# thelondonsmiths/Solex_ser_recon_EN

Hardware: AMD Instinct MI355X
Metric: SER frames/sec end-to-end (decode→clahe) + %HBM roofline, 1/2/4/8 MI355X (higher is better)
Workload: dtype u16

## Files before the change

include/shg_hip.h:

```cpp
#ifndef SHG_HIP_H
#define SHG_HIP_H

#include <stddef.h>
#include <stdint.h>

#ifdef __cplusplus
extern "C" {
#endif

#define SHG_ABI_VERSION 16

#define SHG_E_ARG        (-1)
#define SHG_E_WORKSPACE  (-2)
#define SHG_E_UNSUPPORTED (-3)
#define SHG_E_VALUE      (-4)
#define SHG_E_TYPE       (-5)
#define SHG_E_LINALG     (-6)
#define SHG_E_RUNTIME    (-7)
#define SHG_E_QHULL      (-8)
#define SHG_E_ASSERT     (-9)
#define SHG_E_INDEX      (-10)

typedef void* shg_stream_t;

// ... 199 lines not shown
                             int64_t rank_lo, int64_t rank_hi, uint16_t* out_lo, uint16_t* out_hi,
                             shg_stream_t stream);

int shg_crop_pad_u16(const uint16_t* src, int64_t h, int64_t w, int64_t pitch,
                     uint16_t* dst, int64_t nw, int64_t dst_pitch,
                     int64_t sx0, int64_t dx0, int64_t n, int32_t fill, shg_stream_t stream);

size_t shg_clahe_workspace_bytes(int tiles, int bytes_per_px);
size_t shg_clahe_workspace_bytes_for(int64_t h, int64_t w, int tiles, int bytes_per_px);
int shg_clahe(const void* img, int64_t h, int64_t w, int64_t pitch, int bytes_per_px,
              double clip_limit, int tiles, void* dst, int64_t dst_pitch,
              void* workspace, size_t workspace_bytes, shg_stream_t stream);

int shg_hist(const void* img, int64_t h, int64_t w, int64_t pitch, int bytes_per_px,
             uint32_t* hist, shg_stream_t stream);

size_t shg_select_u16_workspace_bytes(int n_ranks);
int shg_select_u16(const uint16_t* img, int64_t h, int64_t w, int64_t pitch, const int64_t* host_ranks,
                   int n_ranks, double* out, void* workspace, size_t workspace_bytes, shg_stream_t stream);

int shg_rescale_u16(const uint16_t* img, int64_t h, int64_t w, int64_t pitch,
                    double lo, double hi, double alpha, uint16_t* dst, int64_t dst_pitch,
                    shg_stream_t stream);
int shg_rescale_u8(const uint8_t* img, int64_t h, int64_t w, int64_t pitch, double lo, double hi,
                   double alpha, uint8_t* dst, int64_t dst_pitch, shg_stream_t stream);

int shg_fill_disc_u16(uint16_t* img, int64_t h, int64_t w, int64_t pitch,
                      int64_t x0, int64_t y0, int64_t r, uint16_t value, int32_t* scratch,
                      shg_stream_t stream);

int shg_downscale_mean_u16(const uint16_t* img, int64_t h, int64_t w, int64_t pitch, int factor,
                           double* dst, shg_stream_t stream);

int shg_box_blur_f64(const double* src, int64_t h, int64_t w, int k, double* dst, double* tmp,
                     shg_stream_t stream);

int shg_box_blur_key_f64(const double* src, int64_t h, int64_t w, int k, double* dst, uint32_t* keys, double* tmp,
                         shg_stream_t stream);
size_t shg_select_keys_workspace_bytes(int n_pairs);
int shg_select_keys_u32(const uint32_t* const* host_keys, int64_t n, const int64_t* host_ranks, const int* host_k,
                        int n_pairs, double* out, void* workspace, size_t workspace_bytes, shg_stream_t stream);

size_t shg_select_workspace_bytes(int n_ranks);
int shg_select_f64(const double* values, int64_t n, const int64_t* host_ranks, int n_ranks, double* out,
                   void* workspace, size_t workspace_bytes, shg_stream_t stream);
int shg_select_multi_f64(const double* const* host_arrays, int64_t n, const int64_t* host_ranks, int n_ranks,
                         double* out, void* workspace, size_t workspace_bytes, shg_stream_t stream);

int shg_flood_stats_f64(const double* image, const double* blurred, int64_t n, double very_bright,
                        double* stats, uint32_t* counts, void* workspace, shg_stream_t stream);
int shg_flood_stats_lerp_f64(const double* image, const double* blurred, int64_t n,
                             const double* order_stats, double gamma, double* stats, uint32_t* counts,
                             void* workspace, shg_stream_t stream);

size_t shg_canny_workspace_bytes(int64_t h, int64_t w);
int shg_canny_masks_f64(const double* blurred, int64_t h, int64_t w, double flood_thresh,
                        const double* host_gauss_weights, int radius, double low, double high,
                        uint8_t* low_mask, uint8_t* high_mask, void* workspace, size_t workspace_bytes,
                        shg_stream_t stream);

size_t shg_edge_components_workspace_bytes(int64_t h, int64_t w);
int shg_edge_components(const uint8_t* low_mask, const uint8_t* high_mask, int64_t h, int64_t w,
                        int32_t* out_idx, int32_t* out_root, int32_t* out_count,
                        void* workspace, size_t workspace_bytes, shg_stream_t stream);

size_t shg_contrast_stats_workspace_bytes(int tiles);
size_t shg_contrast_stats_workspace_bytes_for(int64_t h, int64_t w, int tiles);
int shg_contrast_stats_u16(const uint16_t* frame, int64_t h, int64_t w, int64_t pitch, double clip_limit,
                           int tiles, uint16_t* cl1, int64_t cl1_pitch, const int64_t* ranks_frame2,
                           const int64_t* ranks_cl13, double* out5, void* workspace, size_t workspace_bytes,
                           shg_stream_t stream);
int shg_contrast_products_u16(const uint16_t* frame, int64_t frame_pitch, const uint16_t* cl1, int64_t cl1_pitch,
                              int64_t h, int64_t w, const double* lo_hi6, uint16_t* high_contrast,
                              uint16_t* protus, uint16_t* cc, int64_t dst_pitch, int64_t disc_x0,
                              int64_t disc_y0, int64_t disc_r, shg_stream_t stream);
int shg_contrast_products_vec_fits(const uint16_t* frame, int64_t frame_pitch, const uint16_t* cl1, int64_t cl1_pitch,
                                   int64_t h, int64_t w, const uint16_t* high_contrast, const uint16_t* protus,
                                   const uint16_t* cc, int64_t dst_pitch);

int shg_limb_fused_fits(int64_t sh, int64_t sw, int k);
size_t shg_limb_prepare_workspace_bytes(int64_t sh, int64_t sw, int k);
int shg_limb_prepare(const uint16_t* img, int64_t h, int64_t w, int64_t pitch, int k, const int64_t* host_ranks4, double gamma99,
                     double* packed, const uint32_t** keys_out, void* workspace, size_t workspace_bytes, shg_stream_t stream);
size_t shg_limb_edges_workspace_bytes(int64_t sh, int64_t sw);
int shg_limb_edges(const uint32_t* keys, int64_t sh, int64_t sw, int k, double flood_thresh, const double* host_gauss_weights,
                   int radius, double low, double high, int32_t* comp, void* workspace, size_t workspace_bytes, shg_stream_t stream);


size_t shg_stage_mean_fit_workspace_bytes(int64_t n_frames, int64_t height, int64_t width, int bytes_per_px);
size_t shg_stage_mean_fit_host_bytes(int64_t height, int64_t width);
int shg_stage_mean_fit(const void* stack, int64_t n_frames, int64_t height, int64_t width, int bytes_per_px,
                       int64_t frame_stride_px, const uint64_t* sum_in, const uint16_t* max_in, int64_t n_total,
                       uint16_t* mean_out, uint16_t* max_out, int64_t* host_y12, double* host_p4, double* host_fit,
                       int32_t* host_trace_sharp, uint8_t* host_mask_good, void* workspace, size_t workspace_bytes,
                       void* host_pinned, size_t host_pinned_bytes, shg_stream_t stream);

size_t shg_stage_extract_workspace_bytes(int64_t height, int64_t width, int n_shifts);
int shg_stage_extract(const void* stack, int64_t n_frames, int64_t height, int64_t width, int bytes_per_px,
                      int64_t frame_stride_px, const double* host_fit, const int32_t* host_shifts, int n_shifts,
                      uint16_t* disks, int64_t row_pitch, int64_t plane_stride, int64_t n_cols, int64_t k_offset,
                      int flip_x, uint32_t* minmax_slots, void* workspace, size_t workspace_bytes, void* host_pinned,
                      size_t host_pinned_bytes, shg_stream_t stream);

size_t shg_stage_limb_points_workspace_bytes(int64_t h, int64_t w);
size_t shg_stage_limb_points_host_bytes(int64_t h, int64_t w);
int shg_stage_limb_points(const uint16_t* disk, int64_t h, int64_t w, int64_t pitch, const double* host_gauss_taps,
                          int32_t* host_points, uint8_t* host_flags, int64_t points_cap, int64_t* host_counts2,
                          void* workspace, size_t workspace_bytes, void* host_pinned, size_t host_pinned_bytes,
                          shg_stream_t stream);

int shg_stage_limb_fit(const uint16_t* disk, int64_t h, int64_t w, int64_t pitch, const double* host_gauss_taps,
                       int32_t* host_points, uint8_t* host_flags, int64_t points_cap, int64_t* host_counts3,
                       double* host_geom16, int64_t* host_dims2, double* host_outline200, void* workspace,
                       size_t workspace_bytes, void* host_pinned, size_t host_pinned_bytes, shg_stream_t stream);

size_t shg_stage_process_workspace_bytes(int64_t k, int64_t h, int64_t w, int64_t crop_w, int tiles);
size_t shg_stage_process_host_bytes(int64_t k, int64_t h);
int shg_stage_process_frames(const uint16_t* const* host_frames, int64_t k, int64_t h, int64_t w, int64_t pitch,
                             int transversalium, const double* host_circle3, const double* host_borders4,
                             const double* host_taps, int64_t window, double* host_factors, int64_t crop_w,
                             int64_t sx0, int64_t dx0, int64_t ncopy, double clip_limit, int tiles, int64_t disc_x0,
                             int64_t disc_y0, int64_t disc_r, uint16_t* const* host_detrans, int64_t detrans_pitch,
                             uint16_t* const* host_final, uint16_t* const* host_cl1, uint16_t* const* host_hc,
                             uint16_t* const* host_protus, uint16_t* const* host_cc, int64_t out_pitch, void* workspace,
                             size_t workspace_bytes, void* host_pinned, size_t host_pinned_bytes, shg_stream_t stream);

typedef struct shg_scan_request {
    uint32_t struct_bytes;
    int32_t  start_phase;
    const void* stack;
    int64_t  n_frames, height, width, frame_stride_px;
    int32_t  bytes_per_px;
    int32_t  flip_x;
    const int32_t* host_shifts;
    const uint8_t* host_requested;
    int32_t  n_shifts;
    int32_t  want_fit_image;
    double   ratio_fixe, slant_fix_deg;
    int32_t  transversalium, keep_detrans;
    int64_t  trans_strength;
    const double* host_taps;
    int64_t  taps_window;
    int32_t  crop_square, has_fixed_width;
    int64_t  fixed_width;
    int32_t  disk_display, tiles;
    int64_t  delta_radius;
    double   clip_limit;
    const double* host_gauss_taps;
    uint16_t* mean_out;
    uint16_t* max_out;
    uint16_t* disks;
    int64_t  disk_pitch, disk_plane_stride;
    uint32_t* minmax_slots;
    void*    arena;
    size_t   arena_bytes;
    void*    results;
    size_t   results_bytes;
    void*    workspace;
    size_t   workspace_bytes;
    void*    host_pinned;
    size_t   host_pinned_bytes;
    double*  host_fit;
    int32_t* host_trace_sharp;
    uint8_t* host_mask_good;
    int32_t* host_points;
    uint8_t* host_flags;
    int64_t  points_cap;
    double*  host_outline200;
    double*  host_factors;
} shg_scan_request;

typedef struct shg_scan_result {
    int32_t phase_done;
    int32_t limb_fitted;
    int64_t y1, y2;
    double  p4[4];
    int64_t counts3[3];
    double  geom16[16];
    double  phi, ratio;
    double  h_first[3], h_rest[3];
    double  theta_first, theta_rest;
    double  circle3[3], borders4[4];
    double  circle_out3[3];
    int64_t out_h, out_w, frame_pitch;
    int64_t n_out, prod_w, prod_pitch;
    int64_t window;
    int64_t crop4[4];
    int64_t disc3[3];
    int64_t fit_image_off;
    int64_t frames_off;
    int64_t detrans_off;
    int64_t products_off;
    int64_t results_off;
    size_t  needed_arena_bytes, needed_results_bytes, needed_workspace_bytes;
} shg_scan_result;

size_t shg_scan_workspace_bytes(const shg_scan_request* req);
size_t shg_scan_host_bytes(const shg_scan_request* req);
int shg_scan_file(const shg_scan_request* req, shg_scan_result* res, shg_stream_t stream);
typedef int (*shg_savgol_taps_fn)(int64_t window, double* out);
int shg_host_set_savgol_taps(shg_savgol_taps_fn fn);

typedef struct shg_pool shg_pool;
int shg_pool_create(const shg_stream_t* streams, int n_workers, const int32_t* host_cpus, int n_cpus, shg_pool** out);
int shg_pool_submit(shg_pool* pool, const shg_scan_request* req, shg_scan_result* res, int64_t* ticket);
int shg_pool_submit_after(shg_pool* pool, const shg_scan_request* req, shg_scan_result* res, shg_stream_t after, int64_t* ticket);
int shg_scan_prelaunch(const shg_scan_request* req, shg_stream_t after, int* launched);
int shg_pass_a_prelaunch(const void* stack, int64_t n_frames, int64_t height, int64_t width, int bytes_per_px,
                         int64_t frame_stride_px, void* workspace, size_t workspace_bytes, shg_stream_t after, int* launched);
int shg_pass_a_forget(const void* workspace);
int shg_lane_packets_probe(const void* stack, int64_t n_frames, int64_t height, int64_t width, int bytes_per_px,
                           int64_t frame_stride_px, void* workspace, size_t workspace_bytes, int mode, int launches,
                           shg_stream_t stream, double* ms_per_launch);
int shg_pool_poll(shg_pool* pool, int64_t ticket);
int shg_pool_wait(shg_pool* pool, int64_t ticket, int* scan_status, char* error_buf, size_t error_cap);
int shg_pool_destroy(shg_pool* pool);

int shg_device_cu_count(int* out);
int shg_stream_create(int priority, const uint32_t* host_cu_mask, int n_mask_words, shg_stream_t* out);
int shg_stream_destroy(shg_stream_t stream);
int shg_frame_pass_lane_set(shg_stream_t lane);
shg_stream_t shg_frame_pass_lane_get(void);

int shg_host_bind_lapack(void* dgelsd_ilp64);
int shg_host_lapack_bound(void);
typedef int64_t (*shg_mode_pick_fn)(const int64_t* neg_counts, int64_t n);
int shg_host_set_mode_pick(shg_mode_pick_fn pick);
int shg_host_polyfit3(const double* host_x, const double* host_y, int64_t n, double* host_coef4);
int shg_host_detect_bord(const double* host_row_means, int64_t n, int64_t* lb, int64_t* ub);
int shg_host_line_fit(const int32_t* host_trace_blur, const int32_t* host_trace_sharp, int64_t ih, int64_t y1,
                      int64_t y2, int32_t blur_offset, double* host_p4, double* host_fit, uint8_t* host_mask_good);
int shg_host_column_plan(const double* host_fit, int64_t ih, int64_t iw, const int32_t* host_shifts, int n_shifts,
                         int32_t* host_ind_l, double* host_lw, double* host_rw);
int shg_host_flood_threshold(double total, int64_t h, int64_t w, double mn, double mx, const int64_t* host_counts20,
                             double* thresh_out);
int shg_host_limb_points(const int32_t* host_idx, const int32_t* host_root, int64_t m, int64_t h, int64_t w,
                         uint8_t* host_out_sel, int64_t* n_selected);
int shg_host_bind_blas(void* cblas_dgemm_ilp64, void* cblas_dsyrk_ilp64, void* cblas_dgemv_ilp64, void* dgesv_ilp64,
                       void* dgeev_ilp64);
int shg_host_blas_bound(void);
int shg_host_fit_ellipse(const double* host_points, int64_t n, double* host_center2, double* width, double* height,
                         double* phi);
int shg_host_correction_matrix(double phi, double r, double* host_inv4, double* theta_out);
int shg_host_two_step(const double* host_points, int64_t n, double* host_center2, double* height_out, double* phi_out,
                      double* ratio_out, uint8_t* host_kept, int64_t* n_kept, double* host_outline200);
int shg_host_warp_geometry(double phi, double ratio, int64_t h, int64_t w, double* host_mat3_9, double* host_inv4,
                           double* host_origin2, double* det_out, double* theta_out, int64_t* out_h, int64_t* out_w);
int shg_host_limb_geometry(const double* host_points, int64_t n, int64_t h, int64_t w, double* host_geom16,
                           int64_t* host_dims2, uint8_t* host_kept, int64_t* n_kept, double* host_outline200);
int shg_host_chord_bounds(double cx, double cy, double r, double b0, double b2, int64_t y1, int64_t y2, int64_t w,
                          int32_t* host_xa, int32_t* host_xb);
int shg_host_transversalium_factors(const double* host_ratios, const double* host_interior, int64_t k, int64_t n,
// ... 9 lines not shown
```

solex_ser_recon_en_amd/Solex_recon.py:

```python
import contextlib
import functools
import math
import os
import queue
import sys
import threading

import numpy as np

from . import dist, ops, outputs, timing
from .device import DeviceImage, bind_thread, cpu_plan, default_device, to_device_u16
from .ellipse_to_circle import correct_image, ellipse_to_circle
from .fits_io import write_fits
from . import stages
from .solex_util import (as_uint16_image, clearlog, compute_mean_return_fit, correct_transversalium2_batch, extract_disks,
                         image_process_batch, logme, make_header, output_path, plots_enabled, removeVignette, savgol_taps,
                         savgol_window, write_complete, write_products)
from .video_reader import video_reader


WORKERS = 4


def _worker_count(workers, n_tasks):
# ... 460 lines not shown


def _scan_pool(scan, n_tasks, n_workers, device):
    import torch
    lock = threading.Lock()
    state = {'next': 0, 'errors': []}

    done = threading.Semaphore(0)

    def run(k):
        try:
            work(k)
        except BaseException as e:
            with lock:
                state['errors'].append((n_tasks, e))
        finally:
            done.release()

    def work(k):
        try:
            torch.cuda.set_device(device)
            bind_thread('scan', device)
            ctx = _worker_context(device, k)
            stages.use_buffers(ctx['buffers'])
            stream = ctx['stream']
        except BaseException as e:
            with lock:
                state['errors'].append((state['next'], e))
            return
        with torch.cuda.stream(stream):
            while True:
                with lock:
                    i = state['next']
                    if i >= n_tasks or state['errors']:
                        break
                    state['next'] = i + 1
                try:
                    scan(i)
                except BaseException as e:
                    with lock:
                        state['errors'].append((i, e))
                    break
            stream.synchronize()

    for k in range(n_workers):
        _Service.named('shg-scan-%s-%d' % (device, k)).jobs.put(functools.partial(run, k))
    for _ in range(n_workers):
        done.acquire()
    if state['errors']:
        raise min(state['errors'], key=lambda ie: ie[0])[1]


def _one_call_ok(rdr, options):
    if os.environ.get('SHG_SCAN_CALL', '1') == '0' or timing.enabled:
        return False
    if options.get('_shard_frames') or dist.is_sharded(rdr):
        return False
    if options['de-vignette'] or (options['transversalium'] and options.get('stubborn_transversalium')):
        return False
    return True


def scan_one_call(rdr, options):
    return _OneCall(rdr, options).run().finish()


class _OneCall:

    def __init__(self, rdr, options, pooled=False):
        self.rdr, self.options = rdr, options
        self.basefich0 = basefich0 = os.path.splitext(str(rdr.file))[0]
        options['basefich0'] = basefich0
        self.log = log = basefich0 + '_log.txt'
        clearlog(log, options)
        logme(log, options, 'Pixel shift : ' + str(options['shift']))
        options['shift_requested'] = options['shift']
        options['shift'] = list(dict.fromkeys([options['ellipse_fit_shift'], 0] + options['shift']))
        self.hdr = make_header(rdr)
        logme(log, options, 'Width, Height : ' + str(rdr.Width) + ' ' + str(rdr.Height))
        logme(log, options, 'Number of frames : ' + str(rdr.FrameCount))
        self.shifts = shifts = options['shift']
        self.requested = [sh in options['shift_requested'] for sh in shifts]
        self.plots = plots = plots_enabled(options)
        self.call = stages.ScanCall(rdr.device_stack(), shifts, self.requested, options, savgol_taps, want_plot_data=plots,
                                    want_fit_image=plots, own_buffers=pooled)

    def run(self):
        self.call.run()
        return self

    def submit(self, pool):
        self.call.submit(pool)
        return self

    def done(self):
        return self.call.done()

    def finish(self):
        from .ellipse_to_circle import _log_geometry, _warp_geometry
        rdr, options, hdr, log, basefich0 = self.rdr, self.options, self.hdr, self.log, self.basefich0
        shifts, requested, plots = self.shifts, self.requested, self.plots
        r, error = self.call.wait().collect()
        self.call = None
        _release_stack(rdr)
        phase = r['phase']
        if phase >= 1:
            mean_img = DeviceImage(r['mean'])
            y1, y2 = r['y1'], r['y2']
            if options['save_fit']:
                outputs.submit(write_fits, output_path(basefich0 + '_mean.fits', options), mean_img, hdr)
            logme(log, options, 'Vertical limits y1, y2 : ' + str(y1) + ' ' + str(y2))
            logme(log, options, lambda: 'Spectral line polynomial fit: ' + str(r['p']))
            if plots:
                rows = np.arange(y1, y2)
                good = r['mask_good']
                outputs.submit(outputs.plot_spectral_line, output_path(basefich0 + '_spectral_line_data.png', options), mean_img,
                               r['sharp'].astype(np.int64)[y1:y2][good], rows[good], r['fit'][:, 3], int(rdr.ih), (y2 - y1) // 20 + 1)
        disk_list = []
        if phase >= 2:
            hdr['NAXIS1'] = rdr.iw
            if options['save_fit'] or plots or (phase >= 3 and not r['limb_fitted'] and requested[0] and '_nolog' not in options):
                disk_list = [DeviceImage(r['disks'][i], minmax=r['extrema'][i]) for i in range(len(shifts))]
            if options.get('_keep_raw'):
                options['_raw_disks'] = [DeviceImage(r['disks'][i]) for i in range(len(shifts))]
            for i, disk in enumerate(disk_list):
                if options['save_fit'] and requested[i]:
                    outputs.submit(write_fits, output_path(basefich0 + '_shift=' + str(shifts[i]) + '_raw.fits', options), disk, hdr)
            if options['transversalium']:
                logme(log, options, 'Transversalium correction : ' + str(options['trans_strength']))
            else:
                logme(log, options, 'Transversalium disabled')
            logme(log, options, 'Mirror X : ' + str(options['flip_x']))
            logme(log, options, 'Post-rotation : ' + str(options['img_rotate']) + ' degrees')
            logme(log, options, f'Protus adjustment : {options["delta_radius"]}')
            logme(log, options, f'de-vignette : {options["de-vignette"]}')
        if phase >= 3:
            if r['limb_fitted']:
                options['ratio_fixe'] = r['ratio']
                _log_geometry(options, r['phi'], r['ratio'], r['theta_first'], np.array(r['circle'][:2]), r['circle'][2])
                print('sun borders found:' + str(r['borders']))
                options['slant_fix'] = math.degrees(r['phi'])
            elif requested[0] and '_nolog' not in options:
                ih_, n_ = disk_list[0].shape
                theta, inv_mat, _, _, _, origin, det = _warp_geometry(float(r['phi']), float(r['ratio']), int(ih_), int(n_))
                _log_geometry(options, r['phi'], r['ratio'], theta, (inv_mat @ np.array([-1.0, -1.0]).T).T - origin,
                              -1.0 * np.sqrt(np.abs(r['ratio'] / det)), known=False)
        if error is not None:
            raise error
        names = [basefich0 + '_shift=' + str(shifts[i]) for i in range(len(shifts)) if requested[i]]
        if plots and r['limb_fitted']:
            fix_img = r['frames'][0] if requested[0] else r['fit_image']
            outputs.submit(outputs.plot_ellipse_fit, output_path(basefich0 + '_shift=' + str(shifts[0]) + '_ellipse_fit.png', options),
                           disk_list[0], DeviceImage(fix_img), r['raw_X'], r['X_f'], r['outline'], r['borders'])
        if options['save_fit']:
            for j, basefich in enumerate(names):
                outputs.submit(write_fits, output_path(basefich + '_circular.fits', options), DeviceImage(r['frames'][j]), hdr)
        if options['transversalium']:
            for i, basefich in enumerate(names):
                c = r['factors'][i]
                options['_transversalium_cache'] = c
                if plots:
                    outputs.submit(outputs.plot_transversalium, output_path(basefich + '_transversalium_correction.png', options), c)
                if options['save_fit']:
                    outputs.submit(write_fits, output_path(basefich + '_detransversaliumed.fits', options), DeviceImage(r['detrans'][i]), hdr)
        if '_nolog' in options and not options['save_fit'] and options['img_rotate'] // 90 % 4 == 0:
            return [(DeviceImage(r['cc'][i]), DeviceImage(r['protus'][i])) for i in range(len(names))]
        results = [write_products(r['final'][i], r['cl1'][i], r['hc'][i], r['protus'][i], r['cc'][i], options, hdr, names[i])
                   for i in range(len(names))]
# ... 213 lines not shown
```

solex_ser_recon_en_amd/_lib.py:

```python
import ctypes
import os
from ctypes import c_double, c_int, c_int32, c_int64, c_size_t, c_uint16, c_uint32, c_void_p

import torch

_HERE = os.path.dirname(os.path.abspath(__file__))
LIB_PATH = os.path.join(_HERE, 'csrc', 'libshg_hip.so')

if not os.path.exists(LIB_PATH):
    raise ImportError(
        'libshg_hip.so is missing (%s). Build it with `python -c "import __graft_entry__ as g; g.build()"` or '
        '`make -C solex_ser_recon_en_amd/csrc`. There is no CPU fallback for the SHG hot path.' % LIB_PATH)

lib = ctypes.CDLL(LIB_PATH)

P = c_void_p
PD = ctypes.POINTER(c_double)
PI64 = ctypes.POINTER(c_int64)


class ScanRequest(ctypes.Structure):
    _fields_ = [('struct_bytes', c_uint32), ('start_phase', c_int32),
                ('stack', P), ('n_frames', c_int64), ('height', c_int64), ('width', c_int64), ('frame_stride_px', c_int64),
                ('bytes_per_px', c_int32), ('flip_x', c_int32),
                ('host_shifts', P), ('host_requested', P), ('n_shifts', c_int32), ('want_fit_image', c_int32),
                ('ratio_fixe', c_double), ('slant_fix_deg', c_double),
                ('transversalium', c_int32), ('keep_detrans', c_int32), ('trans_strength', c_int64),
                ('host_taps', P), ('taps_window', c_int64),
                ('crop_square', c_int32), ('has_fixed_width', c_int32), ('fixed_width', c_int64),
                ('disk_display', c_int32), ('tiles', c_int32), ('delta_radius', c_int64), ('clip_limit', c_double),
                ('host_gauss_taps', P),
                ('mean_out', P), ('max_out', P), ('disks', P), ('disk_pitch', c_int64), ('disk_plane_stride', c_int64),
                ('minmax_slots', P), ('arena', P), ('arena_bytes', c_size_t), ('results', P), ('results_bytes', c_size_t), ('workspace', P), ('workspace_bytes', c_size_t),
                ('host_pinned', P), ('host_pinned_bytes', c_size_t),
                ('host_fit', P), ('host_trace_sharp', P), ('host_mask_good', P), ('host_points', P), ('host_flags', P),
                ('points_cap', c_int64), ('host_outline200', P), ('host_factors', P)]


class ScanResult(ctypes.Structure):
    _fields_ = [('phase_done', c_int32), ('limb_fitted', c_int32), ('y1', c_int64), ('y2', c_int64), ('p4', c_double * 4),
                ('counts3', c_int64 * 3), ('geom16', c_double * 16), ('phi', c_double), ('ratio', c_double),
                ('h_first', c_double * 3), ('h_rest', c_double * 3), ('theta_first', c_double), ('theta_rest', c_double),
                ('circle3', c_double * 3), ('borders4', c_double * 4), ('circle_out3', c_double * 3),
                ('out_h', c_int64), ('out_w', c_int64), ('frame_pitch', c_int64),
                ('n_out', c_int64), ('prod_w', c_int64), ('prod_pitch', c_int64), ('window', c_int64),
                ('crop4', c_int64 * 4), ('disc3', c_int64 * 3),
                ('fit_image_off', c_int64), ('frames_off', c_int64), ('detrans_off', c_int64), ('products_off', c_int64),
                ('results_off', c_int64), ('needed_arena_bytes', c_size_t), ('needed_results_bytes', c_size_t), ('needed_workspace_bytes', c_size_t)]


SIGNATURES = {
    'shg_abi_version': (c_int, []),
    'shg_last_error_string': (ctypes.c_char_p, []),
    'shg_profile_enable': (c_int, [c_int]),
    'shg_profile_select': (c_int, [ctypes.c_char_p]),
    'shg_profile_reset': (c_int, []),
    'shg_profile_get': (c_int, [ctypes.c_char_p, ctypes.POINTER(c_double), ctypes.POINTER(c_int64)]),
    'shg_profile_total': (c_int, [ctypes.POINTER(c_double), ctypes.POINTER(c_int64)]),
    'shg_profile_dump': (c_int, [ctypes.c_char_p]),
    'shg_host_timing_enable': (c_int, [c_int]),
    'shg_host_timing_report': (c_int, [ctypes.c_char_p, c_size_t]),
    'shg_stream_read_probe': (c_int, [P, c_int64, c_int, c_int, c_int, c_int64, P, P]),
    'shg_accumulate_workspace_bytes': (c_size_t, [c_int64, c_int64, c_int64, c_int]),
    'shg_accumulate_sum_max': (c_int, [P, c_int64, c_int64, c_int64, c_int, c_int64, P, P, P, c_size_t, P]),
    'shg_frame_pitch_bytes': (c_int64, [c_int64]),
    'shg_upload_frames': (c_int, [P, c_int64, P, c_int64, c_int64, P]),
    'shg_unpack_dib_frames': (c_int, [P, c_int64, c_int64, c_int64, c_int64, c_int, c_int64, c_int, P, P, c_int64, P]),
    'shg_finalize_mean_max': (c_int, [P, P, c_int64, c_int64, c_int64, c_int, P, P, P]),
    'shg_reduce_frame_stats': (c_int, [P, c_int, c_int64, c_int64, P, P, P]),
    'shg_accumulate_mean_max': (c_int, [P, c_int64, c_int64, c_int64, c_int, c_int64, P, P, P, c_size_t, P]),
    'shg_box_blur_u16': (c_int, [P, c_int64, c_int64, c_int, c_int, P, P, P]),
    'shg_row_argmin_u16': (c_int, [P, c_int64, c_int64, c_int64, c_int64, P, P]),
    'shg_row_mean_u16': (c_int, [P, c_int64, c_int64, P, P]),
    'shg_atlas_correlate': (c_int, [P, c_int64, c_double, c_double, c_double, c_double, P, c_int64, c_int64, c_int64, P, c_int64,
                                    P, P, P, c_int64, P, P]),
    'shg_line_core_shift': (c_int, [P, c_int64, c_int64, c_int64, c_int, c_int64, P, c_int, c_int, P, c_int64, c_int64, c_int64, P]),
    'shg_doppler_finish': (c_int, [P, c_int64, c_int64, c_int64, c_double, c_double, c_double, c_int64, c_int64, P, P, P, c_int64,
                                   P, c_int64, c_double, P]),
    'shg_line_profile': (c_int, [P, c_int64, c_int64, c_int64, c_int, c_int64, P, c_int, c_int, c_int, P, c_int64, c_int64, c_int64,
                                 c_int64, P]),
    'shg_line_profile_finish': (c_int, [P, c_int64, c_int64, c_int64, c_int64, c_double, c_double, c_double, c_int64, c_int64, P, P,
                                        P, c_int64, c_int64, P, c_int64, c_int64, c_int, c_double, P]),
    'shg_line_bisector': (c_int, [P, c_int64, c_int64, c_int64, c_int, c_int64, P, c_int, c_int, P, c_int, c_int, P, c_int64, c_int64,
                                  c_int64, c_int64, P]),
    'shg_line_bisector_finish': (c_int, [P, c_int64, c_int, c_int64, c_int64, c_int64, c_double, c_double, c_double, c_int64, c_int64,
                                         P, P, P, c_int64, c_int64, P, c_int64, c_int64, c_int, c_double, P]),
    'shg_line_emission': (c_int, [P, c_int64, c_int64, c_int64, c_int, c_int64, P, c_int, c_int, c_double, c_int, P, c_int64, c_int64,
                                  c_int64, c_int64, P]),
    'shg_line_emission_finish': (c_int, [P, c_int64, c_int64, c_int64, c_int64, c_double, c_double, c_double, c_int64, c_int64, P, P,
                                         P, c_int64, c_int64, P, c_int64, c_int64, c_int, c_double, P]),
    'shg_map_plane_moments': (c_int, [P, c_int64, c_int64, c_int64, P, P, P, P]),
    'shg_map_detrend': (c_int, [P, c_int64, c_int64, c_int64, P, P, c_int64, P, c_int64, c_double, P]),
    'shg_ring_medians_u16_workspace_bytes': (c_size_t, [c_int64]),
    'shg_ring_medians_u16': (c_int, [P, c_int64, c_int64, c_int64, P, c_int64, P, P, P, P, c_size_t, P]),
    'shg_ring_flatten_u16': (c_int, [P, c_int64, c_int64, c_int64, P, P, c_int64, P, c_int64, P]),
    'shg_stack_combine_u16': (c_int, [P, P, P, c_int, c_int, c_double, c_int, P, c_int64, c_int64, c_int64, P, c_int64, P]),
    'shg_shift_ssd_u16': (c_int, [P, c_int64, P, c_int64, c_int64, c_int64, c_int, P, P, P]),
    'shg_patch_ssd_u16': (c_int, [P, c_int64, P, c_int64, c_int64, c_int64, P, c_int64, c_int, c_int, P, P, P]),
    'shg_stack_combine_field_u16': (c_int, [P, P, P, P, c_int64, c_int64, c_int, c_int, c_int, c_double, c_int, P, c_int64, c_int64, c_int64,
                                            P, c_int64, P]),
    'shg_patch_sharpness_u16': (c_int, [P, c_int64, c_int64, c_int64, P, c_int64, c_int, c_int, P, P, P]),
    'shg_stack_combine_weighted_u16': (c_int, [P, P, P, P, P, c_int64, c_int64, c_int, c_int, c_int, c_double, c_int, P, c_int64, c_int64,
                                               c_int64, P, c_int64, P]),
    'shg_wavelet_workspace_bytes': (c_size_t, [c_int64, c_int64, c_int]),
    'shg_wavelet_sharpen_u16': (c_int, [P, c_int64, c_int64, c_int64, c_int, P, P, P, c_int64, P, P, c_size_t, P]),
    'shg_wavelet_noise_u16': (c_int, [P, c_int64, c_int64, c_int64, P, P, P, c_size_t, P]),
    'shg_rl_workspace_bytes': (c_size_t, [c_int64, c_int64]),
    'shg_rl_deconvolve_u16': (c_int, [P, c_int64, c_int64, c_int64, P, c_int, c_int, P, c_int64, P, P, c_size_t, P]),
    'shg_blur_fits_fused': (c_int, [c_int64, c_int]),
    'shg_blur_row_mean_u16': (c_int, [P, c_int64, c_int64, c_int, c_int, P, P]),
    'shg_blur_argmin_u16': (c_int, [P, c_int64, c_int64, c_int, c_int, c_int64, c_int64, P, P, P]),
    'shg_extract_columns': (c_int, [P, c_int64, c_int64, c_int64, c_int, c_int64, P, P, P, c_int, P, c_int64, c_int64,
                                    c_int64, c_int64, c_int, P]),
    'shg_extract_columns_minmax': (c_int, [P, c_int64, c_int64, c_int64, c_int, c_int64, P, P, P, c_int, P, c_int64, c_int64,
                                           c_int64, c_int64, c_int, P, P]),
    'shg_extract_dense_fits': (c_int, [P, c_int]),
    'shg_extract_columns_dense': (c_int, [P, c_int64, c_int64, c_int64, c_int, c_int64, P, P, P, P, P, c_int, P, c_int64, c_int64, c_int64, c_int64,
                                          c_int, P, P]),
    'shg_warp_rows_minmax_u16': (c_int, [P, c_int64, c_int64, c_int64, c_double, c_double, c_double, P, c_int64, c_int64,
                                         c_int64, P, P]),
    'shg_warp_rows_u16': (c_int, [P, c_int64, c_int64, c_int64, c_double, c_double, c_double, P, c_int64, c_int64,
                                  c_int64, P, P]),
    'shg_warp_rows_wide_fits': (c_int, [P, c_int64, c_int64, c_int64, c_double, c_double, c_double, P, c_int64, c_int64, c_int64]),
    'shg_rowpair_logratio_stats': (c_int, [P, c_int64, c_int64, c_int64, c_int64, c_int64, P, P, P, P, P]),
    'shg_rowpair_logratio_stats_mirrored': (c_int, [P, c_int64, c_int64, c_int64, c_int64, c_int64, P, P, P, P, P, P]),
    'shg_line_order_stats_u16': (c_int, [P, c_int64, c_int64, c_int64, c_int, c_int64, c_int64, P, P, P]),
    'shg_scale_rows_u16': (c_int, [P, c_int64, c_int64, c_int64, P, P, P, c_int64, P]),
    'shg_scale_rows_vec_fits': (c_int, [P, c_int64, c_int64, c_int64, P, c_int64]),
    'shg_correlate1d_rows_f64': (c_int, [P, c_int64, c_int64, P, c_int, c_int, P, P]),
    'shg_lin_filter_row_sums': (c_int, [P, c_int64, c_int64, c_int64, P, P, P, P, P, c_int, P, P, P]),
    'shg_lin_filter_apply': (c_int, [P, c_int64, c_int64, c_int64, P, P, P, c_int, c_int, P, P, P, P, c_int, P, c_int64, P]),
    'shg_crop_pad_u16': (c_int, [P, c_int64, c_int64, c_int64, P, c_int64, c_int64, c_int64, c_int64, c_int64,
                                 c_int, P]),
    'shg_clahe_workspace_bytes': (c_size_t, [c_int, c_int]),
    'shg_clahe_workspace_bytes_for': (c_size_t, [c_int64, c_int64, c_int, c_int]),
    'shg_clahe': (c_int, [P, c_int64, c_int64, c_int64, c_int, c_double, c_int, P, c_int64, P, c_size_t, P]),
    'shg_hist': (c_int, [P, c_int64, c_int64, c_int64, c_int, P, P]),
    'shg_select_u16_workspace_bytes': (c_size_t, [c_int]),
    'shg_select_u16': (c_int, [P, c_int64, c_int64, c_int64, ctypes.POINTER(c_int64), c_int, P, P, c_size_t, P]),
    'shg_rescale_u16': (c_int, [P, c_int64, c_int64, c_int64, c_double, c_double, c_double, P, c_int64, P]),
    'shg_rescale_u8': (c_int, [P, c_int64, c_int64, c_int64, c_double, c_double, c_double, P, c_int64, P]),
    'shg_contrast_stats_workspace_bytes': (c_size_t, [c_int]),
    'shg_contrast_stats_workspace_bytes_for': (c_size_t, [c_int64, c_int64, c_int]),
    'shg_contrast_stats_u16': (c_int, [P, c_int64, c_int64, c_int64, c_double, c_int, P, c_int64, P, P, P, P, c_size_t, P]),
    'shg_contrast_products_u16': (c_int, [P, c_int64, P, c_int64, c_int64, c_int64, P, P, P, P, c_int64, c_int64, c_int64, c_int64, P]),
    'shg_contrast_products_vec_fits': (c_int, [P, c_int64, P, c_int64, c_int64, c_int64, P, P, P, c_int64]),
    'shg_fill_disc_u16': (c_int, [P, c_int64, c_int64, c_int64, c_int64, c_int64, c_int64, c_uint16, P, P]),
    'shg_downscale_mean_u16': (c_int, [P, c_int64, c_int64, c_int64, c_int, P, P]),
    'shg_box_blur_f64': (c_int, [P, c_int64, c_int64, c_int, P, P, P]),
    'shg_box_blur_key_f64': (c_int, [P, c_int64, c_int64, c_int, P, P, P, P]),
    'shg_select_keys_workspace_bytes': (c_size_t, [c_int]),
    'shg_select_keys_u32': (c_int, [ctypes.POINTER(c_void_p), c_int64, ctypes.POINTER(c_int64), ctypes.POINTER(c_int), c_int, P, P, c_size_t, P]),
    'shg_select_workspace_bytes': (c_size_t, [c_int]),
    'shg_select_f64': (c_int, [P, c_int64, ctypes.POINTER(c_int64), c_int, P, P, c_size_t, P]),
    'shg_select_multi_f64': (c_int, [ctypes.POINTER(c_void_p), c_int64, ctypes.POINTER(c_int64), c_int, P, P, c_size_t, P]),
    'shg_flood_stats_f64': (c_int, [P, P, c_int64, c_double, P, P, P, P]),
    'shg_flood_stats_lerp_f64': (c_int, [P, P, c_int64, P, c_double, P, P, P, P]),
    'shg_edge_components_workspace_bytes': (c_size_t, [c_int64, c_int64]),
    'shg_edge_components': (c_int, [P, P, c_int64, c_int64, P, P, P, P, c_size_t, P]),
    'shg_canny_workspace_bytes': (c_size_t, [c_int64, c_int64]),
    'shg_canny_masks_f64': (c_int, [P, c_int64, c_int64, c_double, ctypes.POINTER(c_double), c_int, c_double, c_double, P, P, P,
                                    c_size_t, P]),
    'shg_limb_fused_fits': (c_int, [c_int64, c_int64, c_int]),
    'shg_limb_prepare_workspace_bytes': (c_size_t, [c_int64, c_int64, c_int]),
    'shg_limb_prepare': (c_int, [P, c_int64, c_int64, c_int64, c_int, PI64, c_double, P, ctypes.POINTER(c_void_p), P, c_size_t, P]),
    'shg_limb_edges_workspace_bytes': (c_size_t, [c_int64, c_int64]),
    'shg_limb_edges': (c_int, [P, c_int64, c_int64, c_int, c_double, PD, c_int, c_double, c_double, P, P, c_size_t, P]),
    'shg_stage_mean_fit_workspace_bytes': (c_size_t, [c_int64, c_int64, c_int64, c_int]),
    'shg_stage_mean_fit_host_bytes': (c_size_t, [c_int64, c_int64]),
    'shg_stage_mean_fit': (c_int, [P, c_int64, c_int64, c_int64, c_int, c_int64, P, P, c_int64, P, P, P, P, P, P, P, P, c_size_t, P,
                                   c_size_t, P]),
    'shg_stage_extract_workspace_bytes': (c_size_t, [c_int64, c_int64, c_int]),
    'shg_stage_extract': (c_int, [P, c_int64, c_int64, c_int64, c_int, c_int64, P, P, c_int, P, c_int64, c_int64, c_int64, c_int64, c_int,
                                  P, P, c_size_t, P, c_size_t, P]),
    'shg_stage_limb_points_workspace_bytes': (c_size_t, [c_int64, c_int64]),
    'shg_stage_limb_points_host_bytes': (c_size_t, [c_int64, c_int64]),
    'shg_stage_limb_points': (c_int, [P, c_int64, c_int64, c_int64, P, P, P, c_int64, P, P, c_size_t, P, c_size_t, P]),
    'shg_stage_limb_fit': (c_int, [P, c_int64, c_int64, c_int64, P, P, P, c_int64, P, P, P, P, P, c_size_t, P, c_size_t, P]),
    'shg_stage_process_workspace_bytes': (c_size_t, [c_int64, c_int64, c_int64, c_int64, c_int]),
    'shg_stage_process_host_bytes': (c_size_t, [c_int64, c_int64]),
    'shg_stage_process_frames': (c_int, [P, c_int64, c_int64, c_int64, c_int64, c_int, P, P, P, c_int64, P, c_int64, c_int64, c_int64,
                                         c_int64, c_double, c_int, c_int64, c_int64, c_int64, P, c_int64, P, P, P, P, P, c_int64, P, c_size_t,
                                         P, c_size_t, P]),
    'shg_scan_workspace_bytes': (c_size_t, [ctypes.POINTER(ScanRequest)]),
    'shg_scan_host_bytes': (c_size_t, [ctypes.POINTER(ScanRequest)]),
    'shg_scan_file': (c_int, [ctypes.POINTER(ScanRequest), ctypes.POINTER(ScanResult), P]),
    'shg_host_set_savgol_taps': (c_int, [P]),
    'shg_pool_create': (c_int, [P, c_int, P, c_int, ctypes.POINTER(c_void_p)]),
    'shg_pool_submit': (c_int, [P, ctypes.POINTER(ScanRequest), ctypes.POINTER(ScanResult), ctypes.POINTER(c_int64)]),
    'shg_pool_submit_after': (c_int, [P, ctypes.POINTER(ScanRequest), ctypes.POINTER(ScanResult), P, ctypes.POINTER(c_int64)]),
    'shg_scan_prelaunch': (c_int, [ctypes.POINTER(ScanRequest), P, ctypes.POINTER(c_int)]),
    'shg_pass_a_prelaunch': (c_int, [P, c_int64, c_int64, c_int64, c_int, c_int64, P, c_size_t, P, ctypes.POINTER(c_int)]),
    'shg_pass_a_forget': (c_int, [P]),
    'shg_lane_packets_probe': (c_int, [P, c_int64, c_int64, c_int64, c_int, c_int64, P, c_size_t, c_int, c_int, P, ctypes.POINTER(c_double)]),
    'shg_pool_poll': (c_int, [P, c_int64]),
    'shg_pool_wait': (c_int, [P, c_int64, ctypes.POINTER(c_int), ctypes.c_char_p, c_size_t]),
    'shg_pool_destroy': (c_int, [P]),
    'shg_device_cu_count': (c_int, [ctypes.POINTER(c_int)]),
    'shg_stream_create': (c_int, [c_int, P, c_int, ctypes.POINTER(c_void_p)]),
    'shg_stream_destroy': (c_int, [P]),
    'shg_frame_pass_lane_set': (c_int, [P]),
    'shg_frame_pass_lane_get': (c_void_p, []),
    'shg_host_bind_lapack': (c_int, [P]),
    'shg_host_lapack_bound': (c_int, []),
    'shg_host_set_mode_pick': (c_int, [P]),
    'shg_host_polyfit3': (c_int, [P, P, c_int64, P]),
    'shg_host_detect_bord': (c_int, [P, c_int64, PI64, PI64]),
    'shg_host_line_fit': (c_int, [P, P, c_int64, c_int64, c_int64, ctypes.c_int32, P, P, P]),
    'shg_host_column_plan': (c_int, [P, c_int64, c_int64, P, c_int, P, P, P]),
    'shg_host_flood_threshold': (c_int, [c_double, c_int64, c_int64, c_double, c_double, P, PD]),
    'shg_host_limb_points': (c_int, [P, P, c_int64, c_int64, c_int64, P, PI64]),
    'shg_host_bind_blas': (c_int, [P, P, P, P, P]),
    'shg_host_blas_bound': (c_int, []),
    'shg_host_fit_ellipse': (c_int, [P, c_int64, P, PD, PD, PD]),
    'shg_host_correction_matrix': (c_int, [c_double, c_double, P, PD]),
    'shg_host_two_step': (c_int, [P, c_int64, P, PD, PD, PD, P, PI64, P]),
    'shg_host_warp_geometry': (c_int, [c_double, c_double, c_int64, c_int64, P, P, P, PD, PD, PI64, PI64]),
    'shg_host_limb_geometry': (c_int, [P, c_int64, c_int64, c_int64, P, P, P, PI64, P]),
    'shg_host_chord_bounds': (c_int, [c_double, c_double, c_double, c_double, c_double, c_int64, c_int64, c_int64, P, P]),
    'shg_host_transversalium_factors': (c_int, [P, P, c_int64, c_int64, P, c_int64, c_int, P]),
    'shg_host_percentile_plan': (c_int, [c_int64, c_double, PI64, PI64, PD]),
    'shg_host_lerp': (c_double, [c_double, c_double, c_double]),
}

for _name, (_res, _args) in SIGNATURES.items():
    _fn = getattr(lib, _name)
    _fn.restype = _res
    _fn.argtypes = _args

ABI_VERSION = 16
if lib.shg_abi_version() != ABI_VERSION:
    raise ImportError('libshg_hip.so ABI %d != expected %d: rebuild it' % (lib.shg_abi_version(), ABI_VERSION))


def last_error():
    return lib.shg_last_error_string().decode('utf-8', 'replace')


def _host_error(status, what, message=None):
    msg = last_error() if message is None else message
    if status == -4:
        return ValueError(msg)
    if status == -5:
        return TypeError(msg)
    if status == -6:
        import numpy
        return numpy.linalg.LinAlgError(msg)
    if status == -10:
        return IndexError(msg)
    if status == -9:
        return AssertionError(msg)
    if status == -8:
        try:
            from scipy.spatial import QhullError
            return QhullError(msg)
        except ImportError:
            pass
    return RuntimeError('%s: %s' % (what, msg) if status != -7 else msg)


def check(status, what, message=None):
# ... 106 lines not shown
```

solex_ser_recon_en_amd/csrc/extract.hip:

```cpp
#include <stdlib.h>
#include <algorithm>
#include <type_traits>
#include "shg_common.h"

namespace shg {
thread_local bool t_minmax_slots_zeroed = false;
thread_local void* t_zero_with_fold = nullptr;
thread_local size_t t_zero_with_fold_words = 0;
thread_local void* t_prezeroed = nullptr;
}

namespace {

constexpr int TY = 64;
constexpr int TK = 64;
constexpr int TKP = TK + 2;
constexpr int SC_MAX = 4;

struct ExtractArgs {
    const void* stack;
    int n_frames;
    int64_t height, width, fstride;
    const int32_t* ind_l;
    const double *lw, *rw;
    int n_shifts;
    uint16_t* disks;
    int64_t row_pitch, plane_stride, n_cols, k_offset;
    int flip_x, vec_store;
    uint32_t* mm;
};

template <typename T, bool ROT, int BATCH, int SC> __global__ __launch_bounds__(256) void k_extract(const ExtractArgs kargs) {
    const T* __restrict__ stack = static_cast<const T*>(kargs.stack);
    const int n_frames = kargs.n_frames, n_shifts = kargs.n_shifts, flip_x = kargs.flip_x, vec_store = kargs.vec_store;
    const int64_t height = kargs.height, width = kargs.width, fstride = kargs.fstride, row_pitch = kargs.row_pitch, plane_stride = kargs.plane_stride,
                  n_cols = kargs.n_cols, k_offset = kargs.k_offset;
    const int32_t* __restrict__ ind_l = kargs.ind_l;
    const double* __restrict__ lw = kargs.lw;
    const double* __restrict__ rw = kargs.rw;
    uint16_t* __restrict__ disks = kargs.disks;
    uint32_t* __restrict__ mm = kargs.mm;
    __shared__ uint16_t tile[SC][TY][TKP];
    const int64_t ih = ROT ? width : height;
    const int lane = threadIdx.x & 63;
    const int wave = __builtin_amdgcn_readfirstlane(threadIdx.x >> 6);
    const int64_t c0 = (int64_t)blockIdx.x * TK;
    const int64_t y = (int64_t)blockIdx.y * TY + lane;
    const int s0 = blockIdx.z * SC;
    const int ns = min(SC, n_shifts - s0);
    const bool y_ok = y < ih;
    constexpr int scale = sizeof(T) == 1 ? 256 : 1;

    const int64_t yc = y_ok ? y : ih - 1;
    int il[SC];
    const double wl = lw[yc], wr = rw[yc];
    const double kl = wl * 0x1p+52, kr = wr * 0x1p+52;
    const bool fast = __all(fabs(wl) < 0x1p+900 && fabs(wr) < 0x1p+900) != 0;
#pragma unroll
    for (int s = 0; s < SC; ++s) il[s] = ind_l[(int64_t)(s0 + min(s, ns - 1)) * ih + yc];

    uint32_t off[SC], offr[SC];
    const int64_t step = ROT ? width : 1;
#pragma unroll
    for (int s = 0; s < SC; ++s) {
        off[s] = (uint32_t)((ROT ? (int64_t)il[s] * width + (width - 1 - yc) : yc * width + il[s]) * (int64_t)sizeof(T));
        offr[s] = off[s] + (uint32_t)(step * (int64_t)sizeof(T));
    }

    __shared__ uint32_t wred[4][SC][2];
    uint32_t vlo[SC], vhi[SC];
#pragma unroll
    for (int s = 0; s < SC; ++s) { vlo[s] = 0xffffu; vhi[s] = 0u; }

    for (int cb = wave; cb < TK; cb += 4 * BATCH) {
        T lv[BATCH][SC], rv[BATCH][SC];
        bool ok[BATCH];
#pragma unroll
        for (int i = 0; i < BATCH; ++i) {
            const int cc = cb + 4 * i;
            const int64_t col = c0 + cc;
            const int64_t k = (flip_x ? (n_cols - 1 - col) : col) - k_offset;
            ok[i] = cc < TK && col < n_cols && k >= 0 && k < n_frames;
            const char* f = reinterpret_cast<const char*>(stack + (ok[i] ? k : 0) * fstride);
#pragma unroll
            for (int s = 0; s < SC; ++s) {
                lv[i][s] = *reinterpret_cast<const T*>(f + off[s]);
                rv[i][s] = *reinterpret_cast<const T*>(f + offr[s]);
            }
        }
        auto blend = [&](auto fast_form) {
#pragma unroll
            for (int i = 0; i < BATCH; ++i) {
// ... 153 lines not shown
            const T* f = stack + k * fstride;
            for (int d = 0; d < S; ++d) {
                const int il = ind_l[(int64_t)plane_of.v[d] * ih + yc];
                const int64_t off = ROT ? (int64_t)il * width + (width - 1 - yc) : yc * width + il;
                const double l = (double)((int)f[off] * scale);
                const double r = (double)((int)f[off + step] * scale);
                const double val = l * wl + r * wr;
                const uint32_t q = (uint32_t)(uint16_t)(int)val;
                dtile[((size_t)d * TY + lane) * DKP + cc] = (uint16_t)q;
                vlo[d] = q < vlo[d] ? q : vlo[d];
                vhi[d] = q > vhi[d] ? q : vhi[d];
            }
        }
    }
    if (mm) {
#pragma unroll
        for (int d = 0; d < DS_MAX; ++d) {
            if (d < S) {
                uint32_t lo = vlo[d], hi = vhi[d];
#pragma unroll
                for (int e = 32; e >= 1; e >>= 1) {
                    const uint32_t ol = __shfl_xor(lo, e), oh = __shfl_xor(hi, e);
                    lo = ol < lo ? ol : lo;
                    hi = oh > hi ? oh : hi;
                }
                if (lane == 0) { wred[wave][d][0] = lo; wred[wave][d][1] = hi; }
            }
        }
    }
    __syncthreads();
    if (mm && threadIdx.x < S) {
        const int d = threadIdx.x;
        uint32_t lo = wred[0][d][0], hi = wred[0][d][1];
        for (int wv = 1; wv < NW; ++wv) { lo = wred[wv][d][0] < lo ? wred[wv][d][0] : lo; hi = wred[wv][d][1] > hi ? wred[wv][d][1] : hi; }
        if (hi >= lo) {
            const int slot = (int)((blockIdx.x * 5u + blockIdx.y * 3u) & 63u);
            uint32_t* m = mm + ((int64_t)plane_of.v[d] * 64 + slot) * 2;
            atomicMax(&m[0], 0xffffu - lo);
            atomicMax(&m[1], hi);
        }
    }
    constexpr int SEGS = DK / 8, ROWS = 64 * NW / SEGS;
    const int seg = threadIdx.x % SEGS;
    const int64_t col = c0 + seg * 8;
    for (int pr = threadIdx.x / SEGS; pr < S * TY; pr += ROWS) {
        const int d = pr / TY, r = pr % TY;
        const int64_t yy = (int64_t)blockIdx.y * TY + r;
        if (yy >= ih) continue;
        uint16_t* dst = disks + (int64_t)plane_of.v[d] * plane_stride + yy * row_pitch + col;
        const uint16_t* src = &dtile[((size_t)d * TY + r) * DKP + seg * 8];
        if (vec_store && col + 8 <= n_cols) {
            const int64_t ka = (flip_x ? (n_cols - 1 - col) : col) - k_offset;
            const int64_t kb = (flip_x ? (n_cols - 1 - (col + 7)) : (col + 7)) - k_offset;
            if (ka >= 0 && ka < n_frames && kb >= 0 && kb < n_frames) {
                const uint32_t* s32 = reinterpret_cast<const uint32_t*>(src);
                *reinterpret_cast<uint4*>(dst) = make_uint4(s32[0], s32[1], s32[2], s32[3]);
                continue;
            }
        }
        for (int j = 0; j < 8; ++j) {
            const int64_t cj = col + j;
            const int64_t kj = (flip_x ? (n_cols - 1 - cj) : cj) - k_offset;
            if (cj < n_cols && kj >= 0 && kj < n_frames) dst[j] = src[j];
        }
    }
}

constexpr int BAND_MAX_S = DS_MAX;
constexpr int BAND_NW = 8;
struct BandArgs {
    const void* stack;
    int n_frames;
    int64_t height, width, fstride;
    const int32_t* ind_l;
    const int32_t* base_col;
    const double *lw, *rw;
    int S;
    uint16_t* disks;
    int64_t row_pitch, plane_stride, n_cols, k_offset;
    int flip_x, vec_store;
    uint32_t* mm;
    int nx;
    uint8_t plane_of[BAND_MAX_S];
};
typedef unsigned short __attribute__((ext_vector_type(2))) ushort2_t;
typedef unsigned int __attribute__((ext_vector_type(4))) u32x4_t;
__device__ __forceinline__ uint32_t pk_min_u16(uint32_t a, uint32_t b) {
    return __builtin_bit_cast(uint32_t, __builtin_elementwise_min(__builtin_bit_cast(ushort2_t, a), __builtin_bit_cast(ushort2_t, b)));
}
__device__ __forceinline__ uint32_t pk_max_u16(uint32_t a, uint32_t b) {
    return __builtin_bit_cast(uint32_t, __builtin_elementwise_max(__builtin_bit_cast(ushort2_t, a), __builtin_bit_cast(ushort2_t, b)));
}

template <typename T, int G, bool CONSEC>
__global__ __launch_bounds__(64 * BAND_NW) void k_extract_band(const BandArgs a) {
    constexpr int NW = BAND_NW;
    constexpr int DKW = TK / 2 + 1;
    constexpr int FPW = TK / NW;
    constexpr int PAIRS = FPW / 2;
    constexpr int R = CONSEC ? G + 1 : 2 * G;
    static_assert(FPW % 2 == 0 && FPW * R <= 64, "pairs of frames; a wave has at most 64 loads in flight");
    extern __shared__ uint32_t btile[];
    const int g = (int)(blockIdx.x >> 3);
    const int bx = (int)(blockIdx.y * 8u + (blockIdx.x & 7u)), by = (int)blockIdx.z;
    if (bx >= a.nx) return;
    const T* __restrict__ stack = static_cast<const T*>(a.stack);
    const int n_frames = a.n_frames, flip_x = a.flip_x, S = a.S;
    const int64_t width = a.width, ih = a.width, iw = a.height, fstride = a.fstride, n_cols = a.n_cols, k_offset = a.k_offset;
    const int lane = threadIdx.x & 63;
    const int wave = __builtin_amdgcn_readfirstlane(threadIdx.x >> 6);
    const int64_t c0 = (int64_t)bx * TK;
    const int64_t y = (int64_t)by * TY + lane;
    const bool y_ok = y < ih;
    const int64_t yc = y_ok ? y : ih - 1;
    const int g0 = g * G, ns = min(G, S - g0);
    constexpr int scale = sizeof(T) == 1 ? 256 : 1;
    const double wl = a.lw[yc], wr = a.rw[yc];
    constexpr int HI = sizeof(T) == 1 ? 0x43B00000 : 0x43300000;
    const double kl = wl * (sizeof(T) == 1 ? 0x1p+60 : 0x1p+52), kr = wr * (sizeof(T) == 1 ? 0x1p+60 : 0x1p+52);
    const bool fast = __all(fabs(wl) < 0x1p+900 && fabs(wr) < 0x1p+900) != 0;
    const uint32_t rowb = (uint32_t)(width * (int64_t)sizeof(T));
    const uint32_t colb = (uint32_t)((width - 1 - yc) * (int64_t)sizeof(T));
    uint32_t voff[R];
    bool plain = true;
    if (CONSEC) {
        const int base = a.base_col[yc];
        plain = base >= 0 && (int64_t)base + S <= iw - 1;
        voff[0] = (uint32_t)((plain ? base : 0) + g0) * rowb + colb;
#pragma unroll
        for (int d = 1; d < R; ++d) voff[d] = voff[0] + (uint32_t)min(d, ns) * rowb;
    } else {
#pragma unroll
        for (int d = 0; d < G; ++d) {
            voff[2 * d] = (uint32_t)a.ind_l[(int64_t)(g0 + min(d, ns - 1)) * ih + yc] * rowb + colb;
            voff[2 * d + 1] = voff[2 * d] + rowb;
        }
    }

    const int ncols32 = (int)n_cols;
    uint32_t f_lo, f_hi;
    {
        const int i = lane < FPW ? lane : 0;
        const int col = (int)c0 + 2 * (wave + NW * (i >> 1)) + (i & 1);
        const int k = (flip_x ? (ncols32 - 1 - col) : col) - (int)k_offset;
        const bool ok = col < ncols32 && (unsigned)k < (unsigned)n_frames;
        const uint64_t f = (uint64_t)(uint32_t)(ok ? k : 0) * (uint64_t)(fstride * (int64_t)sizeof(T));
        f_lo = (uint32_t)f;
        f_hi = (uint32_t)(f >> 32);
    }
    uint32_t v[FPW][R];
#pragma unroll
    for (int i = 0; i < FPW; ++i) {
        const char* f = reinterpret_cast<const char*>(stack) + (((uint64_t)(uint32_t)__builtin_amdgcn_readlane((int)f_hi, i) << 32) |
                                                                (uint32_t)__builtin_amdgcn_readlane((int)f_lo, i));
#pragma unroll
        for (int d = 0; d < R; ++d) v[i][d] = (uint32_t)*reinterpret_cast<const T*>(f + voff[d]);
    }

    uint32_t* const my = btile + lane * DKW + wave;
    auto blend = [&](auto fast_form) {
#pragma unroll
        for (int p = 0; p < PAIRS; ++p) {
            uint32_t qv[2][G];
#pragma unroll
            for (int h = 0; h < 2; ++h) {
                const int i = 2 * p + h;
#pragma unroll
                for (int d = 0; d < G; ++d) {
                    const uint32_t xl = v[i][CONSEC ? d : 2 * d], xr = v[i][CONSEC ? d + 1 : 2 * d + 1];
                    double val;
                    if (decltype(fast_form)::value)
                        val = __builtin_fma(__hiloint2double(HI, (int)xl), wl, -kl) + __builtin_fma(__hiloint2double(HI, (int)xr), wr, -kr);
                    else
                        val = (double)(int)(xl * scale) * wl + (double)(int)(xr * scale) * wr;
                    qv[h][d] = (uint32_t)(int)val;
                }
            }
#pragma unroll
            for (int d = 0; d < G; ++d) my[d * TY * DKW + NW * p] = __builtin_amdgcn_perm(qv[1][d], qv[0][d], 0x05040100u);
        }
    };
    if (fast) blend(std::true_type{});
    else blend(std::false_type{});

    if (CONSEC && y_ok && !plain) {
        uint16_t* t16 = reinterpret_cast<uint16_t*>(btile);
        for (int i = 0; i < FPW; ++i) {
            const int cc = 2 * (wave + NW * (i >> 1)) + (i & 1);
            const int64_t col = c0 + cc;
            const int64_t k = (flip_x ? (n_cols - 1 - col) : col) - k_offset;
            if (!(col < n_cols && k >= 0 && k < n_frames)) continue;
            const T* f = stack + k * fstride;
            for (int d = 0; d < ns; ++d) {
                const int il = a.ind_l[(int64_t)a.plane_of[g0 + d] * ih + yc];
                const int64_t off = (int64_t)il * width + (width - 1 - yc);
                const double l = (double)((int)f[off] * scale);
                const double r = (double)((int)f[off + width] * scale);
                t16[((size_t)(d * TY + lane) * DKW) * 2 + cc] = (uint16_t)(uint32_t)(int)(l * wl + r * wr);
            }
        }
    }
    __syncthreads();

    constexpr int SEGS = TK / 8;
    const int seg = lane % SEGS;
    const int64_t col = c0 + seg * 8;
    const int64_t ka = (flip_x ? (n_cols - 1 - col) : col) - k_offset;
    const int64_t kb = (flip_x ? (n_cols - 1 - (col + 7)) : (col + 7)) - k_offset;
    const bool whole = a.vec_store && col + 8 <= n_cols && ka >= 0 && ka < n_frames && kb >= 0 && kb < n_frames;
    const int rows_here = (int)min((int64_t)TY, ih - (int64_t)by * TY);
    for (int d = wave; d < ns; d += NW) {
        const int plane = CONSEC ? a.plane_of[g0 + d] : g0 + d;
        uint16_t* dst0 = a.disks + (int64_t)plane * a.plane_stride + ((int64_t)by * TY) * a.row_pitch + col;
        uint32_t lo = 0xffffffffu, hi = 0u;
        if (whole) {
#pragma unroll 4
            for (int r = lane / SEGS; r < rows_here; r += 64 / SEGS) {
                const uint32_t* s32 = &btile[(d * TY + r) * DKW + seg * 4];
                const u32x4_t o = {s32[0], s32[1], s32[2], s32[3]};
                __builtin_nontemporal_store(o, reinterpret_cast<u32x4_t*>(dst0 + r * a.row_pitch));
                lo = pk_min_u16(pk_min_u16(lo, o.x), pk_min_u16(pk_min_u16(o.y, o.z), o.w));
                hi = pk_max_u16(pk_max_u16(hi, o.x), pk_max_u16(pk_max_u16(o.y, o.z), o.w));
            }
        } else {
            for (int r = lane / SEGS; r < rows_here; r += 64 / SEGS) {
                const uint16_t* src = reinterpret_cast<const uint16_t*>(&btile[(d * TY + r) * DKW + seg * 4]);
                uint16_t* dst = dst0 + r * a.row_pitch;
                for (int j = 0; j < 8; ++j) {
                    const int64_t cj = col + j;
                    const int64_t kj = (flip_x ? (n_cols - 1 - cj) : cj) - k_offset;
                    if (cj < n_cols && kj >= 0 && kj < n_frames) {
                        dst[j] = src[j];
                        lo = pk_min_u16(lo, src[j] * 0x10001u);
                        hi = pk_max_u16(hi, src[j] * 0x10001u);
                    }
                }
            }
        }
        if (a.mm) {
            lo = shg::wave_fold_u32(lo, [](uint32_t x, uint32_t y) { return pk_min_u16(x, y); });
            hi = shg::wave_fold_u32(hi, [](uint32_t x, uint32_t y) { return pk_max_u16(x, y); });
            const uint32_t l16 = min(lo & 0xffffu, lo >> 16), h16 = max(hi & 0xffffu, hi >> 16);
            if (lane == 0 && h16 >= l16) {
                const int slot = (int)((bx * 5u + by * 3u) & 63u);
                uint32_t* m = a.mm + ((int64_t)plane * 64 + slot) * 2;
                atomicMax(&m[0], 0xffffu - l16);
                atomicMax(&m[1], h16);
            }
        }
    }
}

template <bool CONSEC>
int launch_band(const BandArgs& ba, int bytes_per_px, int64_t ih, hipStream_t st) {
    const int S = ba.S;
    int G;
    if (CONSEC) {
        const int ng7 = (S + 6) / 7;
        G = std::max(4, (S + ng7 - 1) / ng7);
    } else {
        G = S <= 2 ? 2 : 4;
    }
    const int ng = (S + G - 1) / G;
    const dim3 grid(8u * (unsigned)ng, ((unsigned)ba.nx + 7u) / 8u, (unsigned)((ih + TY - 1) / TY));
    int status = SHG_E_UNSUPPORTED;
#define SHG_BAND(T, GV)                                                                                                                   \
    if (G == GV && bytes_per_px == (int)sizeof(T)) {                                                                                      \
        constexpr size_t lds = (size_t)GV * TY * (TK / 2 + 1) * 4;                                                                        \
        static const bool ok_ = lds <= 64 * 1024 || hipFuncSetAttribute(reinterpret_cast<const void*>(k_extract_band<T, GV, CONSEC>),    \
                                                                        hipFuncAttributeMaxDynamicSharedMemorySize, (int)lds) == hipSuccess; \
        if (!ok_) (void)hipGetLastError();                                                                                                \
        status = shg::launch_timed("extract", k_extract_band<T, GV, CONSEC>, grid, dim3(64 * BAND_NW), lds, st, nullptr, "k_extract_band", ba); \
    }
    if constexpr (CONSEC) {
        SHG_BAND(uint16_t, 4) SHG_BAND(uint16_t, 5) SHG_BAND(uint16_t, 6) SHG_BAND(uint16_t, 7)
        SHG_BAND(uint8_t, 4) SHG_BAND(uint8_t, 5) SHG_BAND(uint8_t, 6) SHG_BAND(uint8_t, 7)
    } else {
        SHG_BAND(uint16_t, 2) SHG_BAND(uint16_t, 4) SHG_BAND(uint8_t, 2) SHG_BAND(uint8_t, 4)
    }
#undef SHG_BAND
    return status;
}

struct FoldMinmaxArgs {
    const uint32_t* slots;
    uint32_t* out;
    int n_planes;
    uint32_t* zero;
    size_t zero_words;
};

__global__ __launch_bounds__(64) void k_fold_minmax(const FoldMinmaxArgs kargs) {
    const uint32_t* __restrict__ slots = kargs.slots;
    uint32_t* __restrict__ out = kargs.out;
    if ((int)blockIdx.x >= kargs.n_planes) {
        uint32_t* __restrict__ z = kargs.zero;
        const size_t stride = (size_t)(gridDim.x - kargs.n_planes) * 64;
        for (size_t i = (size_t)(blockIdx.x - kargs.n_planes) * 64 + threadIdx.x; i < kargs.zero_words; i += stride) z[i] = 0;
        return;
    }
    uint32_t a = slots[((int64_t)blockIdx.x * 64 + threadIdx.x) * 2], b = slots[((int64_t)blockIdx.x * 64 + threadIdx.x) * 2 + 1];
    a = shg::wave_fold_u32(a, [](uint32_t x, uint32_t y) { return x > y ? x : y; });
    b = shg::wave_fold_u32(b, [](uint32_t x, uint32_t y) { return x > y ? x : y; });
    if (threadIdx.x == 0) { out[blockIdx.x * 2] = 0xffffu - a; out[blockIdx.x * 2 + 1] = b; }
}

int launch_fold(uint32_t* minmax_slots, int n_shifts, hipStream_t st) {
    FoldMinmaxArgs fa{minmax_slots, minmax_slots + (int64_t)n_shifts * 64 * 2, n_shifts, nullptr, 0};
    unsigned extra = 0;
    if (shg::t_zero_with_fold && shg::t_zero_with_fold_words > 0) {
        fa.zero = static_cast<uint32_t*>(shg::t_zero_with_fold);
        fa.zero_words = shg::t_zero_with_fold_words;
        extra = (unsigned)std::min<size_t>((fa.zero_words + 1023) / 1024, 64);
    }
    const int e = shg::launch(k_fold_minmax, dim3((unsigned)n_shifts + extra), dim3(64), 0, st, fa, "k_fold_minmax");
    if (e == 0 && extra) shg::t_prezeroed = shg::t_zero_with_fold;
    shg::t_zero_with_fold = nullptr;
    shg::t_zero_with_fold_words = 0;
    return e;
}

}

extern "C" int shg_extract_columns(const void* stack, int64_t n_frames, int64_t height, int64_t width,
                                   int bytes_per_px, int64_t frame_stride_px, const int32_t* ind_l, const double* lw, const double* rw,
                                   int n_shifts, uint16_t* disks, int64_t row_pitch, int64_t plane_stride,
                                   int64_t n_cols, int64_t k_offset, int flip_x, shg_stream_t stream) {
    return shg_extract_columns_minmax(stack, n_frames, height, width, bytes_per_px, frame_stride_px, ind_l, lw, rw, n_shifts, disks,
                                      row_pitch, plane_stride, n_cols, k_offset, flip_x, nullptr, stream);
}

extern "C" int shg_extract_columns_minmax(const void* stack, int64_t n_frames, int64_t height, int64_t width,
                                          int bytes_per_px, int64_t frame_stride_px, const int32_t* ind_l, const double* lw, const double* rw,
                                          int n_shifts, uint16_t* disks, int64_t row_pitch, int64_t plane_stride,
                                          int64_t n_cols, int64_t k_offset, int flip_x, uint32_t* minmax_slots, shg_stream_t stream) {
    const bool slots_zeroed = shg::t_minmax_slots_zeroed;
    shg::t_minmax_slots_zeroed = false;
    SHG_REQUIRE(stack && ind_l && lw && rw && disks, SHG_E_ARG, "shg_extract_columns: null pointer");
    SHG_REQUIRE(n_frames > 0 && height > 0 && width > 0 && n_shifts > 0, SHG_E_ARG, "shg_extract_columns: empty input");
    SHG_REQUIRE(bytes_per_px == 1 || bytes_per_px == 2, SHG_E_ARG, "shg_extract_columns: bytes_per_px must be 1 or 2");
    SHG_REQUIRE(n_frames < (1ll << 31), SHG_E_UNSUPPORTED, "shg_extract_columns: too many frames");
    SHG_REQUIRE(n_cols >= n_frames && k_offset >= 0 && k_offset + n_frames <= n_cols, SHG_E_ARG,
                "shg_extract_columns: frames [%lld, %lld) do not fit %lld columns", (long long)k_offset,
                (long long)(k_offset + n_frames), (long long)n_cols);
    SHG_REQUIRE(row_pitch >= n_cols, SHG_E_ARG, "shg_extract_columns: row_pitch < n_cols");
    SHG_REQUIRE((height < width ? height : width) >= 2, SHG_E_ARG, "shg_extract_columns: spectral axis needs >= 2 pixels");
    SHG_REQUIRE(frame_stride_px == 0 || frame_stride_px >= height * width, SHG_E_ARG, "shg_extract_columns: frame stride smaller than a frame");
    SHG_REQUIRE(height * width * bytes_per_px < (1ll << 32), SHG_E_UNSUPPORTED, "shg_extract_columns: a frame of %lld x %lld samples is larger than 4 GiB",
                (long long)height, (long long)width);
    const int64_t fstride = frame_stride_px > 0 ? frame_stride_px : height * width;
    const bool rot = width > height;
    const int64_t ih = rot ? width : height;
    const int vec_store = ((reinterpret_cast<uintptr_t>(disks) & 15) == 0) && (row_pitch % 8 == 0) && (plane_stride % 8 == 0);
    static const int sc_env = [] { const char* e = getenv("SHG_EXT_SC"); return e ? atoi(e) : 0; }();
    const int sc = n_shifts <= 2 ? 2 : (sc_env == 2 ? 2 : SC_MAX);
    dim3 grid((unsigned)((n_cols + TK - 1) / TK), (unsigned)((ih + TY - 1) / TY), (unsigned)((n_shifts + sc - 1) / sc));
    hipStream_t st = shg::as_stream(stream);
    const int n = (int)n_frames;
    const ExtractArgs xa{stack, n, height, width, fstride, ind_l, lw, rw, n_shifts, disks, row_pitch, plane_stride, n_cols, k_offset, flip_x, vec_store, minmax_slots};
    int launch_status = 0;
#define EXT_LAUNCH_BS(T, ROT, B, SCV) launch_status = shg::launch_timed("extract", k_extract<T, ROT, B, SCV>, grid, dim3(256), 0, st, nullptr, "k_extract", xa)
#define EXT_LAUNCH_B(T, ROT, B) do { if (sc == 2) EXT_LAUNCH_BS(T, ROT, B, 2); else EXT_LAUNCH_BS(T, ROT, B, 4); } while (0)
#define EXT_LAUNCH(T, ROT)                                                 \
    switch (batch) {                                                       \
        case 1: EXT_LAUNCH_B(T, ROT, 1); break;                            \
        case 2: EXT_LAUNCH_B(T, ROT, 2); break;                            \
        case 8: EXT_LAUNCH_B(T, ROT, 8); break;                            \
        case 16: EXT_LAUNCH_B(T, ROT, 16); break;                          \
        default: EXT_LAUNCH_B(T, ROT, 4); break;                           \
    }
    static const int batch_env = [] { const char* e = getenv("SHG_EXT_BATCH"); return e ? atoi(e) : 0; }();
    const int batch2 = 4;
    const int batch = batch_env > 0 ? batch_env : (n_shifts > SC_MAX ? 8 : (n_shifts <= 2 ? batch2 : 4));
    if (minmax_slots && !slots_zeroed) {
        if (hipError_t e = hipMemsetAsync(minmax_slots, 0, (size_t)n_shifts * 64 * 2 * sizeof(uint32_t), st)) {
            shg::set_error("shg_extract_columns: memset: %s", hipGetErrorString(e));
            return (int)e;
        }
    }
    const bool general_only = [] { const char* e = getenv("SHG_EXT_GENERAL"); return e && atoi(e) != 0; }();
    if (rot && !general_only) {
        BandArgs ba{stack, n, height, width, fstride, ind_l, nullptr, lw, rw, n_shifts, disks, row_pitch, plane_stride, n_cols, k_offset, flip_x, vec_store,
                    minmax_slots, (int)((n_cols + TK - 1) / TK), {}};
        launch_status = launch_band<false>(ba, bytes_per_px, ih, st);
        if (launch_status) return launch_status;
        if (minmax_slots) return launch_fold(minmax_slots, n_shifts, st);
        return 0;
    }
    if (bytes_per_px == 2) {
        if (rot) EXT_LAUNCH(uint16_t, true) else EXT_LAUNCH(uint16_t, false)
    } else {
        if (rot) EXT_LAUNCH(uint8_t, true) else EXT_LAUNCH(uint8_t, false)
    }
#undef EXT_LAUNCH_B
#undef EXT_LAUNCH_BS
#undef EXT_LAUNCH
    if (launch_status) return launch_status;
    if (minmax_slots) return launch_fold(minmax_slots, n_shifts, st);
    return 0;
}

extern "C" int shg_extract_dense_fits(const int32_t* host_shifts, int n_shifts) {
    if (!host_shifts || n_shifts < 3 || n_shifts > DS_MAX) return 0;
    int lo = host_shifts[0], hi = host_shifts[0];
    for (int i = 1; i < n_shifts; ++i) { lo = host_shifts[i] < lo ? host_shifts[i] : lo; hi = host_shifts[i] > hi ? host_shifts[i] : hi; }
    if ((int64_t)hi - lo != n_shifts - 1) return 0;
    bool seen[DS_MAX] = {};
    for (int i = 0; i < n_shifts; ++i) {
        if (seen[host_shifts[i] - lo]) return 0;
        seen[host_shifts[i] - lo] = true;
    }
    return 1;
}

extern "C" int shg_extract_columns_dense(const void* stack, int64_t n_frames, int64_t height, int64_t width, int bytes_per_px,
                                         int64_t frame_stride_px, const int32_t* ind_l, const int32_t* base_col, const double* lw,
                                         const double* rw, const int32_t* host_shifts, int n_shifts, uint16_t* disks, int64_t row_pitch,
                                         int64_t plane_stride, int64_t n_cols, int64_t k_offset, int flip_x, uint32_t* minmax_slots,
                                         shg_stream_t stream) {
    const bool slots_zeroed = shg::t_minmax_slots_zeroed;
    shg::t_minmax_slots_zeroed = false;
    SHG_REQUIRE(stack && ind_l && base_col && lw && rw && host_shifts && disks, SHG_E_ARG, "shg_extract_columns_dense: null pointer");
    SHG_REQUIRE(n_frames > 0 && height > 0 && width > 0, SHG_E_ARG, "shg_extract_columns_dense: empty input");
    SHG_REQUIRE(shg_extract_dense_fits(host_shifts, n_shifts), SHG_E_UNSUPPORTED, "shg_extract_columns_dense: the shifts are not 3..%d consecutive integers", DS_MAX);
    SHG_REQUIRE(bytes_per_px == 1 || bytes_per_px == 2, SHG_E_ARG, "shg_extract_columns_dense: bytes_per_px must be 1 or 2");
    SHG_REQUIRE(n_frames < (1ll << 31), SHG_E_UNSUPPORTED, "shg_extract_columns_dense: too many frames");
    SHG_REQUIRE(n_cols >= n_frames && k_offset >= 0 && k_offset + n_frames <= n_cols, SHG_E_ARG, "shg_extract_columns_dense: frames do not fit the columns");
    SHG_REQUIRE(row_pitch >= n_cols, SHG_E_ARG, "shg_extract_columns_dense: row_pitch < n_cols");
    SHG_REQUIRE((height < width ? height : width) > n_shifts, SHG_E_UNSUPPORTED, "shg_extract_columns_dense: the spectral axis must be wider than the shift range");
    SHG_REQUIRE(frame_stride_px == 0 || frame_stride_px >= height * width, SHG_E_ARG, "shg_extract_columns_dense: frame stride smaller than a frame");
    const int64_t fstride = frame_stride_px > 0 ? frame_stride_px : height * width;
    const bool rot = width > height;
    const int64_t ih = rot ? width : height;
    const int vec_store = ((reinterpret_cast<uintptr_t>(disks) & 15) == 0) && (row_pitch % 8 == 0) && (plane_stride % 8 == 0);
    int lo = host_shifts[0];
    for (int i = 1; i < n_shifts; ++i) lo = host_shifts[i] < lo ? host_shifts[i] : lo;
    PlaneOfOffset po = {};
    for (int i = 0; i < n_shifts; ++i) po.v[host_shifts[i] - lo] = i;
    hipStream_t st = shg::as_stream(stream);
    if (minmax_slots && !slots_zeroed) {
        if (hipError_t e = hipMemsetAsync(minmax_slots, 0, (size_t)n_shifts * 64 * 2 * sizeof(uint32_t), st)) {
            shg::set_error("shg_extract_columns_dense: memset: %s", hipGetErrorString(e));
            return (int)e;
        }
    }
    const int n = (int)n_frames;
    if (rot) {
        BandArgs ba{stack, n, height, width, fstride, ind_l, base_col, lw, rw, n_shifts, disks, row_pitch, plane_stride, n_cols, k_offset, flip_x, vec_store,
                    minmax_slots, (int)((n_cols + TK - 1) / TK), {}};
        for (int i = 0; i < n_shifts; ++i) ba.plane_of[host_shifts[i] - lo] = (uint8_t)i;
        const int launch_status = launch_band<true>(ba, bytes_per_px, ih, st);
        if (launch_status) return launch_status;
        if (minmax_slots) return launch_fold(minmax_slots, n_shifts, st);
        return 0;
    }
    static const int shape = [] { const char* e = getenv("SHG_EXT_DENSE_SHAPE"); return e ? atoi(e) : 0; }();
#define SHG_DENSE(T, ROT, B, NW, DKV)                                                                                                               \
    do {                                                                                                                                            \
        static const bool ok_ = hipFuncSetAttribute(reinterpret_cast<const void*>(k_extract_dense<T, ROT, B, NW, DKV>),                            \
                                                    hipFuncAttributeMaxDynamicSharedMemorySize, 160 * 1024) == hipSuccess;                         \
        if (!ok_) (void)hipGetLastError();                                                                                                          \
        const size_t lds = (size_t)n_shifts * TY * (DKV + 2) * sizeof(uint16_t);                                                                    \
        dim3 grid((unsigned)((n_cols + DKV - 1) / DKV), (unsigned)((ih + TY - 1) / TY));                                                            \
        launch_status = shg::launch_timed("extract", k_extract_dense<T, ROT, B, NW, DKV>, grid, dim3(64 * NW), lds, st, nullptr, "k_extract_dense",      \
                                          static_cast<const T*>(stack), n, height, width, fstride, ind_l, base_col, lw, rw,                       \
                                          n_shifts, po, disks, row_pitch, plane_stride, n_cols, k_offset, flip_x, vec_store, minmax_slots);       \
    } while (0)
#define SHG_DENSE_S(T, ROT)                                                                  \
    do {                                                                                     \
        switch (shape) {                                                                     \
            case 1: SHG_DENSE(T, ROT, 4, 8, 32); break;                                      \
            case 2: SHG_DENSE(T, ROT, 2, 16, 32); break;                                     \
            case 3: SHG_DENSE(T, ROT, 4, 4, 16); break;                                      \
            case 4: SHG_DENSE(T, ROT, 2, 8, 16); break;                                      \
            case 5: SHG_DENSE(T, ROT, 2, 4, 8); break;                                       \
            case 6: SHG_DENSE(T, ROT, 4, 4, 32); break;                                      \
            default: SHG_DENSE(T, ROT, 4, 4, 16); break;                                     \
        }                                                                                    \
    } while (0)
    int launch_status = 0;
    if (bytes_per_px == 2) { if (rot) SHG_DENSE_S(uint16_t, true); else SHG_DENSE_S(uint16_t, false); }
    else { if (rot) SHG_DENSE_S(uint8_t, true); else SHG_DENSE_S(uint8_t, false); }
#undef SHG_DENSE_S
#undef SHG_DENSE
    if (launch_status) return launch_status;
    if (minmax_slots) return launch_fold(minmax_slots, n_shifts, st);
    return 0;
}
```

solex_ser_recon_en_amd/csrc/limb_fused.hip:

```cpp
#include <math.h>
#include <stdlib.h>
#include <algorithm>
#include "shg_common.h"
#include "limb_math.h"

namespace {

using namespace shg::limb;
using shg::f64_key;
using shg::key_f64;

#if defined(__HIP_DEVICE_COMPILE__) && !defined(__gfx950__)
#error "limb_fused.hip: published() relies on how gfx950 performs agent-scope atomics; use an acq_rel agent-scope fetch_add elsewhere"
#endif
__device__ __forceinline__ void published() {
    asm volatile("s_waitcnt vmcnt(0)" ::: "memory");
    __syncthreads();
}
__device__ __forceinline__ bool count_done(uint32_t* done, uint32_t total, int fence) {
    const uint32_t before = fence ? __hip_atomic_fetch_add(done, 1u, __ATOMIC_ACQ_REL, __HIP_MEMORY_SCOPE_AGENT)
                                  : __hip_atomic_fetch_add(done, 1u, __ATOMIC_RELAXED, __HIP_MEMORY_SCOPE_AGENT);
    return before == total - 1;
}
inline int limb_fence() {
// ... 1 lines not shown
    return v && v[0] == '1';
}


constexpr int TH = 16, TW = 64;
constexpr int KMAX = 16;

struct PrepLayout {
    int bits0, bits1;
    size_t hist0, hist1, coarse0, coarse1, acc, counts, done, zero_words;
    size_t keys5, keysk, total_words;
};

__host__ __device__ inline int bit_length(uint64_t v) {
    int b = 0;
    while (v) { ++b; v >>= 1; }
    return b;
}

PrepLayout prep_layout(int64_t sh, int64_t sw, int k) {
    PrepLayout L;
    const int kk = k > 5 ? k : 5;
    const int total_bits = bit_length((uint64_t)kk * kk * 16ull * 65535ull);
    L.bits1 = total_bits / 2;
    L.bits0 = total_bits - L.bits1;
    size_t off = 0;
    L.hist0 = off; off += (size_t)2 << L.bits0;
    L.hist1 = off; off += (size_t)4 << L.bits1;
    L.coarse0 = off; off += 2 * 256;
    L.coarse1 = off; off += 4 * 256;
    L.acc = off; off += 2 * ACC_WORDS;
    L.counts = off; off += HIST_BINS;
    L.done = off; off += 4;
    L.zero_words = off;
    off = (off + 63) / 64 * 64;
    const size_t n = (size_t)sh * (size_t)sw;
    L.keysk = off; off += (n + 63) / 64 * 64;
    L.keys5 = off; off += (n + 63) / 64 * 64;
    L.total_words = off;
    return L;
}

__device__ __forceinline__ void flush_hist(const uint32_t* lh, int bits, uint32_t* coarse_lds, uint32_t* __restrict__ fine,
                                           uint32_t* __restrict__ coarse, int tid, int nthreads) {
    for (int e = tid; e < 256; e += nthreads) coarse_lds[e] = 0;
    __syncthreads();
    const int shift = bits - 8;
    for (int e = tid; e < (1 << bits); e += nthreads) {
        const uint32_t c = lh[e];
        if (c) {
            atomicAdd(&fine[e], c);
            atomicAdd(&coarse_lds[e >> shift], c);
        }
    }
    __syncthreads();
    for (int e = tid; e < 256; e += nthreads)
        if (coarse_lds[e]) atomicAdd(&coarse[e], coarse_lds[e]);
}

__device__ __forceinline__ int refl101(int i, int n) {
    if (i < 0) i = -i;
    if (i >= n) i = 2 * n - 2 - i;
    return (i >= 0 && i < n) ? i : (int)shg::reflect101(i, n);
}

constexpr int BT = 16;
constexpr int NT1 = 1024;
struct ZeroWordsArgs {
    uint32_t* dst;
    size_t n_words;
};
__global__ __launch_bounds__(256) void k_zero_words(const ZeroWordsArgs kargs) {
    uint32_t* __restrict__ dst = kargs.dst;
    for (size_t i = (size_t)blockIdx.x * 256 + threadIdx.x; i < kargs.n_words; i += (size_t)gridDim.x * 256) dst[i] = 0;
}

struct LimbBlurArgs {
    const uint16_t* img;
    int h, w;
    int64_t pitch;
    int sh, sw, k, vec4;
    uint32_t *keysk, *keys5;
    unsigned long long* acc;
};
__global__ __launch_bounds__(256) void k_limb_blur(const LimbBlurArgs kargs) {
    const uint16_t* __restrict__ img = kargs.img;
    const int h = kargs.h, w = kargs.w, sh = kargs.sh, sw = kargs.sw, k = kargs.k, vec4 = kargs.vec4;
    const int64_t pitch = kargs.pitch;
    uint32_t* __restrict__ keysk = kargs.keysk;
    uint32_t* __restrict__ keys5 = kargs.keys5;
    unsigned long long* __restrict__ acc = kargs.acc;
    __shared__ uint32_t S[(BT + KMAX) * (BT + KMAX)];
    __shared__ uint32_t H[(BT + KMAX) * BT];
    __shared__ unsigned long long wsum[4];
    __shared__ uint32_t wmin[4];
    const int hl = max(k / 2, 2), hr = max(k - 1 - k / 2, 2);
    const int RH = BT + hl + hr, RW = RH;
    const int x0 = blockIdx.x * BT, y0 = blockIdx.y * BT;
    const int tid = threadIdx.x;
    uint32_t my_min = 0xffffffffu;
    unsigned long long own = 0;
    for (int e = tid; e < RH * RW; e += 256) {
        const int r = e / RW, c = e - r * RW;
        const int sy = refl101(y0 - hl + r, sh), sx = refl101(x0 - hl + c, sw);
        uint32_t s = 0;
        if (vec4 && sx * 4 + 4 <= w && sy * 4 + 4 <= h) {
            uint2 q[4];
#pragma unroll
            for (int j = 0; j < 4; ++j) q[j] = *reinterpret_cast<const uint2*>(img + (int64_t)(sy * 4 + j) * pitch + sx * 4);
#pragma unroll
            for (int j = 0; j < 4; ++j) s += (q[j].x & 0xffffu) + (q[j].x >> 16) + (q[j].y & 0xffffu) + (q[j].y >> 16);
        } else {
            for (int j = 0; j < 4; ++j) {
                const int y = sy * 4 + j;
                if (y >= h) break;
                for (int i = 0; i < 4; ++i) {
                    const int x = sx * 4 + i;
                    if (x < w) s += img[(int64_t)y * pitch + x];
                }
            }
        }
        S[e] = s;
        const int oy = y0 - hl + r, ox = x0 - hl + c;
        if (r >= hl && r < hl + BT && c >= hl && c < hl + BT && oy < sh && ox < sw) own += s;
    }
    own = shg::wave_sum((uint64_t)own);
    if ((tid & 63) == 0) wsum[tid >> 6] = own;
    const int n_arrays = k == 5 ? 1 : 2;
    for (int a = 0; a < n_arrays; ++a) {
        const int kw = a == 0 ? k : 5;
        uint32_t* keys = a == 0 ? keysk : keys5;
        __syncthreads();
        const int c_off = hl - kw / 2, r_lo = hl - kw / 2, r_n = BT + kw - 1;
        for (int e = tid; e < r_n * BT; e += 256) {
            const int r = r_lo + e / BT, x = e % BT;
            uint32_t s = 0;
            for (int j = 0; j < kw; ++j) s += S[r * RW + x + c_off + j];
            H[r * BT + x] = s;
        }
        __syncthreads();
        const int y = tid / BT, x = tid % BT;
        if (y0 + y < sh && x0 + x < sw) {
            uint32_t s = 0;
            for (int j = 0; j < kw; ++j) s += H[(r_lo + y + j) * BT + x];
            keys[(int64_t)(y0 + y) * sw + x0 + x] = s;
            if (a == 0) my_min = s;
        }
    }
    my_min = shg::wave_fold_u32(my_min, [](uint32_t x, uint32_t y) { return x < y ? x : y; });
    if ((tid & 63) == 0) wmin[tid >> 6] = my_min;
    __syncthreads();
    if (tid == 0) {
        const int slot = (blockIdx.y * gridDim.x + blockIdx.x) % FLOOD_SLOTS;
        const unsigned long long t = wsum[0] + wsum[1] + wsum[2] + wsum[3];
        if (t) atomicAdd(&acc[acc_sum(slot)], t);
        const uint32_t m = min(min(wmin[0], wmin[1]), min(wmin[2], wmin[3]));
        if (m != 0xffffffffu) atomicMax(&acc[ACC_SMALLEST + slot], ~f64_key(((double)m * kUnit) * (1.0 / ((double)k * (double)k))));
    }
}

__device__ __forceinline__ void wave_pick(const uint32_t* __restrict__ fine, const uint32_t* __restrict__ coarse, int bits, int64_t rank,
                                          int& digit, int64_t& below) {
    const int lane = threadIdx.x & 63;
    const int per = 1 << (bits - 8);
    int64_t c[4], local = 0;
#pragma unroll
    for (int j = 0; j < 4; ++j) {
        c[j] = __hip_atomic_load(&coarse[lane * 4 + j], __ATOMIC_RELAXED, __HIP_MEMORY_SCOPE_AGENT);
        local += c[j];
    }
    int64_t incl = shg::wave_scan((int64_t)local);
    int64_t excl = incl - local;
    int chunk = -1;
    int64_t base = 0;
    if (excl <= rank && rank < incl) {
#pragma unroll
        for (int j = 0; j < 4; ++j) {
            if (chunk < 0 && rank < excl + c[j]) { chunk = lane * 4 + j; base = excl; }
            excl += c[j];
        }
    }
    const unsigned long long owner = __ballot(chunk >= 0);
    const int src = owner ? __ffsll((long long)owner) - 1 : 0;
    chunk = __shfl(chunk, src);
    base = __shfl(base, src);
    const int64_t f = lane < per ? (int64_t)__hip_atomic_load(&fine[chunk * per + lane], __ATOMIC_RELAXED, __HIP_MEMORY_SCOPE_AGENT) : 0;
    int64_t fi = shg::wave_scan((int64_t)f);
    const int64_t fe = base + fi - f;
    const bool mine = lane < per && fe <= rank && rank < fe + f;
    const unsigned long long who = __ballot(mine);
    const int src2 = who ? __ffsll((long long)who) - 1 : 0;
    digit = chunk * per + src2;
    below = __shfl(fe, src2);
}

struct Ranks4 { int64_t rank[4]; int array[4]; double scale[4]; };

struct LimbSelect0Args {
    const uint32_t *keysk, *keys5;
    int64_t n;
    int bits0, bits1;
    uint32_t *hist0, *coarse0;
};
__global__ __launch_bounds__(256) void k_limb_select0(const LimbSelect0Args kargs) {
    const uint32_t* __restrict__ keysk = kargs.keysk;
    const uint32_t* __restrict__ keys5 = kargs.keys5;
    const int64_t n = kargs.n;
    const int bits0 = kargs.bits0, bits1 = kargs.bits1;
    uint32_t* __restrict__ hist0 = kargs.hist0;
    uint32_t* __restrict__ coarse0 = kargs.coarse0;
    extern __shared__ uint32_t lds[];
    __shared__ uint32_t lc[256];
    const int a = blockIdx.y;
    const uint32_t* __restrict__ v = a ? keys5 : keysk;
    for (int e = threadIdx.x; e < (1 << bits0); e += 256) lds[e] = 0;
    __syncthreads();
    const int64_t stride = (int64_t)gridDim.x * 256;
    for (int64_t base = (int64_t)blockIdx.x * 256 + threadIdx.x; base < n; base += 4 * stride) {
        uint32_t kk[4];
        bool ok[4];
#pragma unroll
        for (int u = 0; u < 4; ++u) { const int64_t i = base + u * stride; ok[u] = i < n; kk[u] = v[ok[u] ? i : 0]; }
#pragma unroll
        for (int u = 0; u < 4; ++u)
            if (ok[u]) atomicAdd(&lds[kk[u] >> bits1], 1u);
    }
    __syncthreads();
    flush_hist(lds, bits0, lc, hist0 + ((size_t)a << bits0), coarse0 + a * 256, threadIdx.x, 256);
}

struct LimbSelect1Args {
    const uint32_t *keysk, *keys5;
    int64_t n;
    Ranks4 p;
    int bits0, bits1;
    const uint32_t *hist0, *coarse0;
    uint32_t *hist1, *coarse1;
    double gamma;
    uint32_t* done;
// ... 292 lines not shown
        if ((top || left) && x > 0 && (mask[up - 1] & 1)) uf_union<AgentLoad>(L, i, up - 1);
        if (top && (mask[up] & 1)) uf_union<AgentLoad>(L, i, up);
        if ((top || right) && x < w - 1 && (mask[up + 1] & 1)) uf_union<AgentLoad>(L, i, up + 1);
    }
}

struct LimbEmitArgs {
    const uint8_t* mask;
    const int* L;
    int h, w;
    const int* row_counts;
    int tiles_x, n;
    int* comp;
};
__global__ __launch_bounds__(256) void k_limb_emit(const LimbEmitArgs kargs) {
    const uint8_t* __restrict__ mask = kargs.mask;
    const int* __restrict__ L = kargs.L;
    const int h = kargs.h, w = kargs.w, tiles_x = kargs.tiles_x, n = kargs.n;
    const int* __restrict__ row_counts = kargs.row_counts;
    int* __restrict__ comp = kargs.comp;
    __shared__ int wave_cnt[4];
    __shared__ int base;
    __shared__ int part[4];
    const int y = blockIdx.x;
    const int lane = threadIdx.x & 63, wave = threadIdx.x >> 6;
    int before = 0;
    for (int e = threadIdx.x; e < y * tiles_x; e += 256) before += row_counts[e];
    before = shg::wave_sum(before);
    if (lane == 0) part[wave] = before;
    __syncthreads();
    if (threadIdx.x == 0) base = part[0] + part[1] + part[2] + part[3];
    __syncthreads();
    for (int xb = 0; xb < w; xb += 256) {
        const int x = xb + threadIdx.x;
        int root = -1, hi = 0;
        if (x < w) {
            const int i = y * w + x;
            const int l = L[i];
            if (l >= 0) {
                root = uf_find<AgentLoad>(L, l);
                hi = (mask[i] >> 1) & 1;
            }
        }
        const unsigned long long m = __ballot(root >= 0);
        if (lane == 0) wave_cnt[wave] = __popcll(m);
        __syncthreads();
        int off = base;
        for (int i = 0; i < wave; ++i) off += wave_cnt[i];
        if (root >= 0) {
            const int pos = off + __popcll(m & ((1ull << lane) - 1ull));
            comp[1 + pos] = y * w + x;
            comp[1 + n + pos] = root | (hi << 30);
        }
        __syncthreads();
        if (threadIdx.x == 0) base += wave_cnt[0] + wave_cnt[1] + wave_cnt[2] + wave_cnt[3];
        __syncthreads();
    }
    if (y == h - 1 && threadIdx.x == 0) comp[0] = base;
}

size_t canny_tile_lds(int R) {
    const int FW = TW + 4 + 2 * R, FH = TH + 4 + 2 * R, VW = FW, VH = TH + 4, SW = TW + 4, MW = TW + 2, MH = TH + 2;
    return (size_t)(((VH + 7) & ~7) + VH * VW + VH * SW + 3 * MH * MW) * 8 + (size_t)TH * TW * 4 + (size_t)FH * FW;
}

}

extern "C" int shg_limb_fused_fits(int64_t sh, int64_t sw, int k) {
    return sh > 2 && sw > 2 && sh * sw < (1ll << 30) && k >= 1 && k <= KMAX;
}

size_t shg::limb_prepare_zero_words(int64_t h, int64_t w) {
    const int64_t sh = (h + 3) / 4, sw = (w + 3) / 4;
    const int k = (int)((double)sh * 0.01);
    if (!shg_limb_fused_fits(sh, sw, k)) return 0;
    return prep_layout(sh, sw, k).zero_words;
}

extern "C" size_t shg_limb_prepare_workspace_bytes(int64_t sh, int64_t sw, int k) {
    if (!shg_limb_fused_fits(sh, sw, k)) return 0;
    return prep_layout(sh, sw, k).total_words * 4;
}

extern "C" int shg_limb_prepare(const uint16_t* img, int64_t h, int64_t w, int64_t pitch, int k, const int64_t* host_ranks4, double gamma99,
                                double* packed, const uint32_t** keys_out, void* workspace, size_t workspace_bytes, shg_stream_t stream) {
    SHG_REQUIRE(img && host_ranks4 && packed && keys_out && workspace, SHG_E_ARG, "shg_limb_prepare: null pointer");
    SHG_REQUIRE(h > 0 && w > 0 && pitch >= w, SHG_E_ARG, "shg_limb_prepare: bad image size");
    const int64_t sh = (h + 3) / 4, sw = (w + 3) / 4, n = sh * sw;
    SHG_REQUIRE(shg_limb_fused_fits(sh, sw, k), SHG_E_UNSUPPORTED, "shg_limb_prepare: a %d x %d window on %lld x %lld is outside the fused path", k, k,
                (long long)sh, (long long)sw);
    SHG_REQUIRE(gamma99 >= 0.0 && gamma99 <= 1.0, SHG_E_ARG, "shg_limb_prepare: gamma %g outside [0, 1]", gamma99);
    const PrepLayout lay = prep_layout(sh, sw, k);
    SHG_REQUIRE(workspace_bytes >= lay.total_words * 4, SHG_E_WORKSPACE, "shg_limb_prepare: workspace too small");
    SHG_REQUIRE((reinterpret_cast<uintptr_t>(workspace) & 7) == 0, SHG_E_ARG, "shg_limb_prepare: workspace not 8-byte aligned");
    for (int i = 0; i < 4; ++i) SHG_REQUIRE(host_ranks4[i] >= 0 && host_ranks4[i] < n, SHG_E_ARG, "shg_limb_prepare: rank outside the image");
    hipStream_t st = shg::as_stream(stream);
    uint32_t* ws = static_cast<uint32_t*>(workspace);
    uint32_t *hist0 = ws + lay.hist0, *hist1 = ws + lay.hist1, *coarse0 = ws + lay.coarse0, *coarse1 = ws + lay.coarse1;
    uint32_t *counts = ws + lay.counts, *done = ws + lay.done;
    unsigned long long* acc = reinterpret_cast<unsigned long long*>(ws + lay.acc);
    uint32_t *keysk = ws + lay.keysk, *keys5 = k == 5 ? keysk : ws + lay.keys5;
    double* out4 = reinterpret_cast<double*>(acc + ACC_ORDER_STATS);
    SHG_PROF("limb_prepare", st);
    if (shg::t_prezeroed == workspace) {
        shg::t_prezeroed = nullptr;
    } else if (int e = shg::launch(k_zero_words, dim3((unsigned)std::min<size_t>((lay.zero_words + 255) / 256, 64)), dim3(256), 0, st, ZeroWordsArgs{ws, lay.zero_words}, "k_zero_words")) {
        return e;
    }
    Ranks4 p;
    const double scale_k = 1.0 / ((double)k * (double)k), scale_5 = 1.0 / 25.0;
    for (int i = 0; i < 4; ++i) { p.rank[i] = host_ranks4[i]; p.array[i] = (i < 2 && k != 5) ? 1 : 0; p.scale[i] = (i < 2) ? scale_5 : scale_k; }
    dim3 grid1((unsigned)((sw + BT - 1) / BT), (unsigned)((sh + BT - 1) / BT));
    const int vec4 = (reinterpret_cast<uintptr_t>(img) & 7) == 0 && pitch % 4 == 0;
    if (int e = shg::launch(k_limb_blur, grid1, dim3(256), 0, st, LimbBlurArgs{img, (int)h, (int)w, pitch, (int)sh, (int)sw, k, vec4, keysk, keys5, acc}, "k_limb_blur")) return e;
    static const bool lds_ok = [] {
        return hipFuncSetAttribute(reinterpret_cast<const void*>(k_limb_select0), hipFuncAttributeMaxDynamicSharedMemorySize, 128 * 1024) == hipSuccess &&
               hipFuncSetAttribute(reinterpret_cast<const void*>(k_limb_select1), hipFuncAttributeMaxDynamicSharedMemorySize, 128 * 1024) == hipSuccess;
    }();
    if (!lds_ok) (void)hipGetLastError();
    int64_t blocks = (n + 2047) / 2048;
    if (blocks > 256) blocks = 256;
    if (int e = shg::launch(k_limb_select0, dim3((unsigned)blocks, k == 5 ? 1u : 2u), dim3(256), ((size_t)1 << lay.bits0) * 4, st,
                           LimbSelect0Args{keysk, keys5, n, lay.bits0, lay.bits1, hist0, coarse0}, "k_limb_select0"))
        return e;
    if (int e = shg::launch(k_limb_select1, dim3((unsigned)blocks, 4u), dim3(256), ((size_t)1 << lay.bits1) * 4, st,
                           LimbSelect1Args{keysk, keys5, n, p, lay.bits0, lay.bits1, hist0, coarse0, hist1, coarse1, gamma99, done, acc, out4, limb_fence()}, "k_limb_select1"))
        return e;
    *keys_out = keysk;
    return shg::launch(k_limb_flood_hist, dim3((unsigned)blocks), dim3(256), 0, st, LimbFloodHistArgs{keysk, n, scale_k, acc, out4, counts, done + 1, packed, limb_fence()}, "k_limb_flood_hist");
}

extern "C" size_t shg_limb_edges_workspace_bytes(int64_t sh, int64_t sw) {
    if (sh <= 0 || sw <= 0) return 0;
    const size_t n = (size_t)sh * (size_t)sw, tiles_x = (size_t)((sw + TW - 1) / TW);
    return ((n + 255) / 256 * 256) + n * 4 + (size_t)sh * tiles_x * 4 + 256;
}

extern "C" int shg_limb_edges(const uint32_t* keys, int64_t sh, int64_t sw, int k, double flood_thresh, const double* host_gauss_weights,
                              int radius, double low, double high, int32_t* comp, void* workspace, size_t workspace_bytes, shg_stream_t stream) {
    SHG_REQUIRE(keys && host_gauss_weights && comp && workspace, SHG_E_ARG, "shg_limb_edges: null pointer");
    SHG_REQUIRE(sh > 2 && sw > 2 && sh * sw < (1ll << 30) && k >= 1, SHG_E_ARG, "shg_limb_edges: bad image size");
    SHG_REQUIRE(radius >= 0 && radius <= MAXR, SHG_E_UNSUPPORTED, "shg_limb_edges: Gaussian radius %d > %d", radius, MAXR);
    SHG_REQUIRE(workspace_bytes >= shg_limb_edges_workspace_bytes(sh, sw), SHG_E_WORKSPACE, "shg_limb_edges: workspace too small");
    GaussW g;
    g.radius = radius;
    for (int i = 0; i < 2 * radius + 1; ++i) g.w[i] = host_gauss_weights[i];
    const size_t n = (size_t)sh * (size_t)sw;
    const int tiles_x = (int)((sw + TW - 1) / TW);
    uint8_t* mask = static_cast<uint8_t*>(workspace);
    int* L = reinterpret_cast<int*>(mask + (n + 255) / 256 * 256);
    int* row_counts = L + n;
    hipStream_t st = shg::as_stream(stream);
    SHG_PROF("limb_edges", st);
    dim3 grid((unsigned)tiles_x, (unsigned)((sh + TH - 1) / TH));
    static const bool lds_ok = hipFuncSetAttribute(reinterpret_cast<const void*>(k_limb_canny_tile), hipFuncAttributeMaxDynamicSharedMemorySize, 160 * 1024) == hipSuccess;
    if (!lds_ok) (void)hipGetLastError();
    if (int e = shg::launch(k_limb_canny_tile, grid, dim3(NT1), canny_tile_lds(radius), st,
                           LimbCannyArgs{keys, (int)sh, (int)sw, 1.0 / ((double)k * (double)k), flood_thresh, g, low, high, mask, L, row_counts, tiles_x}, "k_limb_canny_tile"))
        return e;
    {
        const int64_t tops = ((sh + TH - 1) / TH) * sw, sides = 2 * (int64_t)tiles_x * sh;
        if (int e = shg::launch(k_limb_border_merge, dim3((unsigned)((std::max(tops, sides) + 255) / 256), 2u), dim3(256), 0, st, LimbBorderArgs{mask, (int)sh, (int)sw, L}, "k_limb_border_merge"))
            return e;
    }
    return shg::launch(k_limb_emit, dim3((unsigned)sh), dim3(256), 0, st, LimbEmitArgs{mask, L, (int)sh, (int)sw, row_counts, tiles_x, (int)n, comp}, "k_limb_emit");
}
```

solex_ser_recon_en_amd/csrc/scan.hip:

```cpp
#include <math.h>
#include <string.h>
#include <atomic>
#include <vector>
#include "shg_common.h"

namespace {

constexpr size_t kAlign = 256;
inline size_t up(size_t b) { return (b + kAlign - 1) / kAlign * kAlign; }
inline int64_t round64(int64_t v) { return (v + 63) / 64 * 64; }
inline int64_t floor_div(int64_t a, int64_t b) { int64_t q = a / b; return (a % b != 0 && ((a < 0) != (b < 0))) ? q - 1 : q; }

const double kRadToDeg = 180.0 / 3.141592653589793238462643383279502884;
const double kDegToRad = 3.141592653589793238462643383279502884 / 180.0;

std::atomic<shg_savgol_taps_fn> g_taps_fn{nullptr};

#define SCAN_TRY(expr)                  \
    do {                                \
        if (int e_ = (expr)) return e_; \
    } while (0)

struct Regions {
    size_t mean_ws, extract_ws, limb_ws, mean_pin, extract_pin, limb_pin, process_pin;
// ... 93 lines not shown
    }
    memcpy(rs->disc3, pl->disc, sizeof(rs->disc3));
    return 0;
}

}

extern "C" int shg_host_set_savgol_taps(shg_savgol_taps_fn fn) {
    g_taps_fn.store(fn);
    return 0;
}

extern "C" size_t shg_scan_workspace_bytes(const shg_scan_request* rq) {
    if (!rq || rq->height <= 0 || rq->width <= 0 || rq->n_frames <= 0 || rq->n_shifts <= 0 || !rq->host_requested) return 0;
    const Regions r = regions(rq);
    return r.mean_ws + r.extract_ws + r.limb_ws + kAlign;
}

extern "C" size_t shg_scan_host_bytes(const shg_scan_request* rq) {
    if (!rq || rq->height <= 0 || rq->width <= 0 || rq->n_frames <= 0 || rq->n_shifts <= 0 || !rq->host_requested) return 0;
    const Regions r = regions(rq);
    return r.mean_pin + r.extract_pin + r.limb_pin + r.process_pin + kAlign;
}

extern "C" int shg_scan_prelaunch(const shg_scan_request* rq, shg_stream_t after, int* launched) {
    SHG_REQUIRE(rq && launched, SHG_E_ARG, "shg_scan_prelaunch: null pointer");
    *launched = 0;
    if (rq->struct_bytes != sizeof(shg_scan_request) || rq->start_phase != 0 || !rq->stack || !rq->workspace || rq->n_frames <= 0 ||
        rq->height <= 0 || rq->width <= 0 || rq->n_shifts <= 0 || (rq->bytes_per_px != 1 && rq->bytes_per_px != 2))
        return 0;
    const Regions rg = regions(rq);
    const size_t acc = shg_accumulate_workspace_bytes(rq->n_frames, rq->height, rq->width, rq->bytes_per_px);
    if (rq->workspace_bytes < rg.mean_ws || acc == 0 || acc > rg.mean_ws) return 0;
    return shg_pass_a_prelaunch(rq->stack, rq->n_frames, rq->height, rq->width, rq->bytes_per_px, rq->frame_stride_px, rq->workspace, acc, after,
                                launched);
}

extern "C" int shg_scan_file(const shg_scan_request* rq, shg_scan_result* rs, shg_stream_t stream) {
    SHG_HOST_TIME("scan_file");
    SHG_REQUIRE(rq && rs, SHG_E_ARG, "shg_scan_file: null pointer");
    SHG_REQUIRE(rq->struct_bytes == sizeof(shg_scan_request), SHG_E_ARG, "shg_scan_file: the caller's shg_scan_request has %u bytes, the library's %zu",
                rq->struct_bytes, sizeof(shg_scan_request));
    SHG_REQUIRE(rq->stack && rq->host_shifts && rq->host_requested && rq->mean_out && rq->max_out && rq->disks && rq->minmax_slots &&
                rq->workspace && rq->host_pinned && rq->host_fit, SHG_E_ARG, "shg_scan_file: null pointer in the request");
    SHG_REQUIRE(rq->n_frames > 0 && rq->height > 0 && rq->width > 0 && rq->n_shifts > 0, SHG_E_ARG, "shg_scan_file: empty input");
    SHG_REQUIRE(rq->disk_pitch >= rq->n_frames && rq->disk_plane_stride > 0, SHG_E_ARG, "shg_scan_file: bad disk layout");
    SHG_REQUIRE(rq->start_phase == 0 || rq->start_phase == 3, SHG_E_ARG, "shg_scan_file: start_phase must be 0 or 3");
    const int64_t ih = slit_rows(rq), n_cols = rq->n_frames;
    const int S = rq->n_shifts;
    const int64_t k = n_requested(rq);
    const bool limb = fits_limb(rq);
    SHG_REQUIRE(!limb || (rq->host_gauss_taps && rq->host_points && rq->host_flags && rq->points_cap > 0), SHG_E_ARG,
                "shg_scan_file: the limb fit needs host_gauss_taps, host_points, host_flags");
    const Regions rg = regions(rq);
    char* ws = static_cast<char*>(rq->workspace);
    char* pin = static_cast<char*>(rq->host_pinned);
    const size_t ws_fixed = rg.mean_ws + rg.extract_ws + rg.limb_ws;
    SHG_REQUIRE(rq->workspace_bytes >= ws_fixed, SHG_E_WORKSPACE, "shg_scan_file: workspace %zu < %zu bytes", rq->workspace_bytes, ws_fixed);
    SHG_REQUIRE(rq->host_pinned_bytes >= rg.mean_pin + rg.extract_pin + rg.limb_pin + rg.process_pin, SHG_E_WORKSPACE,
                "shg_scan_file: pinned staging area %zu < %zu bytes", rq->host_pinned_bytes, rg.mean_pin + rg.extract_pin + rg.limb_pin + rg.process_pin);
    char* mean_ws = ws;
    char* extract_ws = mean_ws + rg.mean_ws;
    char* limb_ws = extract_ws + rg.extract_ws;
    char* process_ws = limb_ws + rg.limb_ws;
    char* mean_pin = pin;
    char* extract_pin = mean_pin + rg.mean_pin;
    char* limb_pin = extract_pin + rg.extract_pin;
    char* process_pin = limb_pin + rg.limb_pin;

    if (rq->start_phase == 0) {
        memset(rs, 0, sizeof(*rs));
        rs->fit_image_off = rs->frames_off = rs->detrans_off = rs->products_off = rs->results_off = -1;
        int64_t y12[2];
        SCAN_TRY(shg_stage_mean_fit(rq->stack, rq->n_frames, rq->height, rq->width, rq->bytes_per_px, rq->frame_stride_px, nullptr, nullptr,
                                    rq->n_frames, rq->mean_out, rq->max_out, y12, rs->p4, rq->host_fit, rq->host_trace_sharp, rq->host_mask_good,
                                    mean_ws, rg.mean_ws, mean_pin, rg.mean_pin, stream));
        rs->y1 = y12[0];
        rs->y2 = y12[1];
        rs->phase_done = 1;
        if (limb) {
            shg::t_zero_with_fold = limb_ws;
            shg::t_zero_with_fold_words = shg::limb_prepare_zero_words(ih, n_cols);
        }
        const int extract_status = shg_stage_extract(rq->stack, rq->n_frames, rq->height, rq->width, rq->bytes_per_px, rq->frame_stride_px, rq->host_fit,
                                                     rq->host_shifts, S, rq->disks, rq->disk_pitch, rq->disk_plane_stride, n_cols, 0, rq->flip_x,
                                                     rq->minmax_slots, extract_ws, rg.extract_ws, extract_pin, rg.extract_pin, stream);
        shg::t_zero_with_fold = nullptr;
        shg::t_zero_with_fold_words = 0;
        if (extract_status) { shg::t_prezeroed = nullptr; return extract_status; }
        rs->phase_done = 2;
        bool later_disks = false;
        for (int i = 1; i < S; ++i) later_disks = later_disks || rq->host_requested[i];
        double mat3[9], inv[4], origin[2], det;
        if (limb) {
            int64_t dims[2];
            const int limb_status = shg_stage_limb_fit(rq->disks, ih, n_cols, rq->disk_pitch, rq->host_gauss_taps, rq->host_points, rq->host_flags, rq->points_cap,
                                                       rs->counts3, rs->geom16, dims, rq->host_outline200, limb_ws, rg.limb_ws, limb_pin, rg.limb_pin, stream);
            shg::t_prezeroed = nullptr;
            if (limb_status) return limb_status;
            const double* g = rs->geom16;
            rs->limb_fitted = 1;
            rs->phi = g[3];
            rs->ratio = g[4];
            memcpy(rs->circle3, g + 5, 3 * sizeof(double));
            memcpy(rs->borders4, g + 8, 4 * sizeof(double));
            memcpy(rs->h_first, g + 12, 3 * sizeof(double));
            rs->theta_first = g[15];
            rs->out_h = dims[0];
            rs->out_w = dims[1];
            memcpy(rs->h_rest, rs->h_first, sizeof(rs->h_rest));
            rs->theta_rest = rs->theta_first;
            if (later_disks) {
                const double phi_again = (rs->phi * kRadToDeg) * kDegToRad;
                int64_t oh, ow;
                SCAN_TRY(shg_host_warp_geometry(phi_again, rs->ratio, ih, n_cols, mat3, inv, origin, &det, &rs->theta_rest, &oh, &ow));
                SHG_REQUIRE(oh == rs->out_h && ow == rs->out_w, SHG_E_VALUE, "process_frames: the frames must share one shape and row pitch");
                memcpy(rs->h_rest, mat3, 3 * sizeof(double));
            }
        } else {
            rs->ratio = isnan(rq->ratio_fixe) ? 1.0 : rq->ratio_fixe;
            rs->phi = isnan(rq->slant_fix_deg) ? 0.0 : rq->slant_fix_deg * kDegToRad;
            SCAN_TRY(shg_host_warp_geometry(rs->phi, rs->ratio, ih, n_cols, mat3, inv, origin, &det, &rs->theta_first, &rs->out_h, &rs->out_w));
            memcpy(rs->h_first, mat3, 3 * sizeof(double));
            memcpy(rs->h_rest, mat3, 3 * sizeof(double));
            rs->theta_rest = rs->theta_first;
            rs->circle3[0] = rs->circle3[1] = rs->circle3[2] = -1;
            shg::t_prezeroed = nullptr;
        }
        rs->phase_done = 3;
    } else {
        SHG_REQUIRE(rs->phase_done == 3, SHG_E_ARG, "shg_scan_file: nothing to resume (phase_done = %d)", rs->phase_done);
    }

    Plan pl;
    SCAN_TRY(make_plan(rq, rs, &pl));
    const int64_t out_h = rs->out_h, out_w = rs->out_w;
    SHG_REQUIRE(out_h > 0 && out_w > 0, SHG_E_VALUE, "correct_image: empty output (%lld x %lld)", (long long)out_h, (long long)out_w);
    const int64_t frame_pitch = round64(out_w);
    const int64_t prod_w = pl.crop_w > 0 ? pl.crop_w : out_w, prod_pitch = round64(prod_w);
    const bool fit_image = rq->want_fit_image && !rq->host_requested[0];
    const bool detrans = rq->transversalium && rq->keep_detrans && k > 0;
    const size_t frame_bytes = up((size_t)out_h * frame_pitch * 2), prod_bytes = up((size_t)out_h * prod_pitch * 2);
    size_t off = 0;
    rs->fit_image_off = fit_image ? (int64_t)off : -1;
    off += fit_image ? frame_bytes : 0;
    rs->frames_off = k > 0 ? (int64_t)off : -1;
    off += (size_t)k * frame_bytes;
    rs->detrans_off = detrans ? (int64_t)off : -1;
    off += detrans ? (size_t)k * frame_bytes : 0;
    rs->products_off = k > 0 ? (int64_t)off : -1;
    off += (size_t)k * 3 * prod_bytes;
    rs->results_off = k > 0 ? 0 : -1;
    rs->needed_results_bytes = (size_t)k * 2 * prod_bytes;
    rs->frame_pitch = frame_pitch;
    rs->n_out = k;
    rs->prod_w = prod_w;
    rs->prod_pitch = prod_pitch;
    rs->needed_arena_bytes = off;
    const size_t process_ws_bytes = k > 0 ? up(shg_stage_process_workspace_bytes(k, out_h, out_w, pl.crop_w, rq->tiles)) : 0;
    rs->needed_workspace_bytes = ws_fixed + process_ws_bytes;
    if (rq->arena_bytes < rs->needed_arena_bytes || (off > 0 && !rq->arena) || rq->results_bytes < rs->needed_results_bytes ||
        (k > 0 && !rq->results) || rq->workspace_bytes < rs->needed_workspace_bytes) {
        shg::set_error("shg_scan_file: the corrected images are %lld x %lld: arena %zu of %zu bytes, results %zu of %zu bytes, workspace %zu of "
                       "%zu bytes -- grow them and call again with start_phase = 3", (long long)out_h, (long long)out_w, rq->arena_bytes,
                       rs->needed_arena_bytes, rq->results_bytes, rs->needed_results_bytes, rq->workspace_bytes, rs->needed_workspace_bytes);
        return SHG_E_WORKSPACE;
    }
    SHG_REQUIRE(((reinterpret_cast<uintptr_t>(rq->arena) | reinterpret_cast<uintptr_t>(rq->results)) & 255) == 0, SHG_E_ARG,
                "shg_scan_file: arenas not 256-byte aligned");
    char* arena = static_cast<char*>(rq->arena);
    char* results = static_cast<char*>(rq->results);
    const uint32_t* extrema = rq->minmax_slots + (size_t)S * 128;
    std::vector<const uint16_t*> w_src;
    std::vector<uint16_t*> w_dst;
    std::vector<const uint32_t*> w_mm;
    std::vector<double> w_h;
    auto add_warp = [&](int i, uint16_t* dst) {
        const double* hr = i == 0 ? rs->h_first : rs->h_rest;
        w_src.push_back(rq->disks + (size_t)i * rq->disk_plane_stride);
        w_dst.push_back(dst);
// ... 32 lines not shown
```

solex_ser_recon_en_amd/csrc/shg_common.h:

```cpp
#pragma once
#if defined(__HIPCC__)
#include <hip/hip_runtime.h>
#include <hip/hip_ext.h>
#endif
#include <stdint.h>
#include <stdio.h>
#include <string.h>
#include <type_traits>

#if defined(__HIPCC__)
#define SHG_HD __host__ __device__ __forceinline__
#else
#define SHG_HD inline
#endif

namespace shg {

SHG_HD uint64_t f64_key(double v) {
#if defined(__HIP_DEVICE_COMPILE__)
    const uint64_t b = (uint64_t)__double_as_longlong(v);
#else
    uint64_t b;
    memcpy(&b, &v, sizeof b);
#endif
    return (b >> 63) ? ~b : (b | 0x8000000000000000ull);
}
SHG_HD double key_f64(uint64_t k) {
    const uint64_t b = (k >> 63) ? (k & 0x7fffffffffffffffull) : ~k;
#if defined(__HIP_DEVICE_COMPILE__)
    return __longlong_as_double((long long)b);
#else
    double v;
    memcpy(&v, &b, sizeof v);
    return v;
#endif
}

SHG_HD double np_lerp(double a, double b, double gamma) {
    const double diff = b - a;
    return gamma >= 0.5 ? b - diff * (1 - gamma) : a + diff * gamma;
}

}

#if defined(__HIPCC__)
#include "../../include/shg_hip.h"

namespace shg {

void set_error(const char* fmt, ...);

inline int check_launch(const char* what) {
    hipError_t e = hipGetLastError();
    if (e != hipSuccess) {
        set_error("%s: %s", what, hipGetErrorString(e));
        return (int)e;
    }
    return 0;
}


template <typename A>
struct same_type { using type = A; };
template <typename A>
inline int launch(void (*k)(A), dim3 grid, dim3 block, size_t lds, hipStream_t st, const typename same_type<A>::type& a, const char* what) {
    hipLaunchKernelGGL(k, grid, block, lds, st, a);
    return check_launch(what);
}

struct TimedEvents { hipEvent_t start = nullptr, stop = nullptr; bool sampled = false; };
int timed_begin(const char* tag, bool want_done, TimedEvents* ev);
void timed_end(const char* tag, hipStream_t st, const TimedEvents& ev, bool launched, hipEvent_t* done);
void event_release(hipEvent_t e);
template <typename... P>
inline int launch_timed(const char* tag, void (*k)(P...), dim3 grid, dim3 block, size_t lds, hipStream_t st, hipEvent_t* done, const char* what,
                        typename same_type<P>::type... a) {
    TimedEvents ev;
    if (int e = timed_begin(tag, done != nullptr, &ev)) return e;
    int r;
    if (ev.start || ev.stop) {
        void* args[] = {static_cast<void*>(&a)...};
        const hipError_t le = hipExtLaunchKernel(reinterpret_cast<const void*>(k), grid, block, args, lds, st, ev.start, ev.stop, 0);
        r = check_launch(what);
        if (r == 0 && le != hipSuccess) { set_error("%s: %s", what, hipGetErrorString(le)); r = (int)le; }
    } else {
        hipLaunchKernelGGL(k, grid, block, lds, st, a...);
        r = check_launch(what);
    }
    timed_end(tag, st, ev, r == 0, done);
    return r;
}

#define SHG_REQUIRE(cond, code, ...)            \
    do {                                        \
        if (!(cond)) {                          \
            shg::set_error(__VA_ARGS__);        \
            return (code);                      \
        }                                       \
    } while (0)

inline hipStream_t as_stream(shg_stream_t s) { return reinterpret_cast<hipStream_t>(s); }

typedef int (*lane_launch_fn)(hipStream_t st, void* arg, hipEvent_t* done);
int on_frame_pass_lane(hipStream_t st, lane_launch_fn launch, void* arg);

extern thread_local bool t_minmax_slots_zeroed;
extern thread_local void* t_zero_with_fold;
extern thread_local size_t t_zero_with_fold_words;
extern thread_local void* t_prezeroed;
size_t limb_prepare_zero_words(int64_t h, int64_t w);
int prelaunch_on_lane(hipStream_t after, lane_launch_fn launch, void* arg, hipEvent_t* done);

struct ProfScope {
    ProfScope(const char* tag, hipStream_t st);
    ~ProfScope();
    int slot;
    hipStream_t stream;
    unsigned generation;
};
#define SHG_PROF(tag, st) shg::ProfScope shg_prof_scope_(tag, st)

struct HostScope {
    explicit HostScope(const char* tag);
    ~HostScope();
    const char* tag;
    double t0;
};
#define SHG_HOST_CAT2(a, b) a##b
#define SHG_HOST_CAT(a, b) SHG_HOST_CAT2(a, b)
#define SHG_HOST_TIME(tag) shg::HostScope SHG_HOST_CAT(shg_host_scope_, __LINE__)(tag)

constexpr int kMaxBatch = 32;
template <int N>
struct PtrBatchN {
    const void* p[N];
    template <typename T>
    __device__ __forceinline__ T* at(int i) const { return static_cast<T*>(const_cast<void*>(p[i])); }
};
using PtrBatch = PtrBatchN<kMaxBatch>;
template <int N, typename T>
inline PtrBatchN<N> make_batch_n(T* const* host_ptrs, int first, int count) {
    PtrBatchN<N> b = {};
    for (int i = 0; i < count && i < N; ++i) b.p[i] = host_ptrs[first + i];
    return b;
}
template <typename T>
inline PtrBatch make_batch(T* const* host_ptrs, int first, int count) { return make_batch_n<kMaxBatch>(host_ptrs, first, count); }

int rowpair_stats_batch(const uint16_t* const* host_imgs, int64_t k, int64_t h, int64_t w, int64_t pitch, int64_t y1, int64_t y2,
                        const int32_t* xa, const int32_t* xb, const double* row_factor, double* out, double* out_mirror, shg_stream_t stream);
int scale_rows_batch(const uint16_t* const* host_imgs, int64_t k, int64_t h, int64_t w, int64_t pitch, const double* c,
                     const double* row_factor, uint16_t* const* host_dsts, int64_t dst_pitch, shg_stream_t stream);
int crop_pad_batch(const uint16_t* const* host_srcs, int64_t k, int64_t h, int64_t w, int64_t pitch, uint16_t* const* host_dsts, int64_t nw,
                   int64_t dst_pitch, int64_t sx0, int64_t dx0, int64_t n, int32_t fill, shg_stream_t stream);
int contrast_products_batch(const uint16_t* const* host_frames, int64_t frame_pitch, const uint16_t* const* host_cl1, int64_t cl1_pitch,
                            int64_t k, int64_t h, int64_t w, const double* host_lo_hi6, uint16_t* const* host_hc, uint16_t* const* host_protus,
                            uint16_t* const* host_cc, int64_t dst_pitch, int64_t disc_x0, int64_t disc_y0, int64_t disc_r, shg_stream_t stream,
                            const double* stats5 = nullptr, double g_bright = 0.0, double g_dark = 0.0, double* mirror5 = nullptr);
int warp_rows_batch(const uint16_t* const* host_srcs, int64_t k, int64_t h, int64_t w, int64_t src_pitch, const double* host_h3,
                    uint16_t* const* host_dsts, int64_t out_h, int64_t out_w, int64_t dst_pitch, const uint32_t* const* host_minmax2,
                    shg_stream_t stream);
struct FrameSource {
    const uint16_t* const* host_raw;
    int64_t raw_pitch;
    const double* factors;
    int64_t sx0, dx0, ncopy;
};
bool contrast_stats_batches(int64_t h, int64_t w, int tiles, double clip_limit);
int contrast_stats_batch(const uint16_t* const* host_frames, int64_t k, int64_t h, int64_t w, int64_t pitch, double clip_limit, int tiles,
                         uint16_t* const* host_cl1, int64_t cl1_pitch, const int64_t* ranks_frame2, const int64_t* ranks_cl13, double* out5,
                         void* workspace, size_t workspace_bytes, shg_stream_t stream, const FrameSource* from = nullptr);

constexpr int kWave = 64;
constexpr int kCUs = 256;

__device__ __forceinline__ int lane_id() { return threadIdx.x & (kWave - 1); }

template <typename Op>
__device__ __forceinline__ uint32_t wave_fold_u32(uint32_t v, Op op) {
    v = op(v, (uint32_t)__builtin_amdgcn_update_dpp((int)v, (int)v, 0xB1, 0xf, 0xf, false));
    v = op(v, (uint32_t)__builtin_amdgcn_update_dpp((int)v, (int)v, 0x4E, 0xf, 0xf, false));
    v = op(v, (uint32_t)__builtin_amdgcn_update_dpp((int)v, (int)v, 0x141, 0xf, 0xf, false));
    v = op(v, (uint32_t)__builtin_amdgcn_update_dpp((int)v, (int)v, 0x140, 0xf, 0xf, false));
    const uint32_t r0 = (uint32_t)__builtin_amdgcn_readlane((int)v, 0), r1 = (uint32_t)__builtin_amdgcn_readlane((int)v, 16),
                   r2 = (uint32_t)__builtin_amdgcn_readlane((int)v, 32), r3 = (uint32_t)__builtin_amdgcn_readlane((int)v, 48);
    return op(op(r0, r1), op(r2, r3));
}

template <typename Op>
__device__ __forceinline__ uint64_t wave_fold_u64(uint64_t v, Op op) {
    auto step = [&](auto ctrl) {
        const int lo = __builtin_amdgcn_update_dpp((int)(uint32_t)v, (int)(uint32_t)v, decltype(ctrl)::value, 0xf, 0xf, false);
// ... 81 lines not shown
```

solex_ser_recon_en_amd/csrc/stages.hip:

```cpp
#include <math.h>
#include <stdlib.h>
#include <string.h>
#include <algorithm>
#include <vector>
#include "shg_common.h"

namespace {

constexpr size_t kAlign = 256;
inline size_t up(size_t b) { return (b + kAlign - 1) / kAlign * kAlign; }

struct Arena {
    char* base;
    size_t cap, off;
    Arena(void* p, size_t bytes) : base(static_cast<char*>(p)), cap(bytes), off(0) {}
    template <typename T>
    T* take(size_t count) {
        const size_t b = up(count * sizeof(T));
        if (!base || off + b > cap) return nullptr;
        T* p = reinterpret_cast<T*>(base + off);
        off += b;
        return p;
    }
};
// ... 87 lines not shown
extern "C" size_t shg_stage_mean_fit_host_bytes(int64_t height, int64_t width) {
    if (height <= 0 || width <= 0) return 0;
    const size_t ih = (size_t)slit_rows(height, width);
    return up(ih * 8) + up(2 * ih * 4);
}

extern "C" int shg_stage_mean_fit(const void* stack, int64_t n_frames, int64_t height, int64_t width, int bytes_per_px,
                                  int64_t frame_stride_px, const uint64_t* sum_in, const uint16_t* max_in, int64_t n_total,
                                  uint16_t* mean_out, uint16_t* max_out, int64_t* host_y12, double* host_p4, double* host_fit,
                                  int32_t* host_trace_sharp, uint8_t* host_mask_good, void* workspace, size_t workspace_bytes,
                                  void* host_pinned, size_t host_pinned_bytes, shg_stream_t stream) {
    SHG_HOST_TIME("stage mean_fit");
    SHG_REQUIRE(mean_out && max_out && host_y12 && host_p4 && host_fit && workspace && host_pinned, SHG_E_ARG,
                "shg_stage_mean_fit: null pointer");
    SHG_REQUIRE((sum_in == nullptr) == (max_in == nullptr), SHG_E_ARG, "shg_stage_mean_fit: sum_in and max_in go together");
    SHG_REQUIRE(sum_in || stack, SHG_E_ARG, "shg_stage_mean_fit: neither a stack nor its sums");
    SHG_REQUIRE(height > 0 && width > 0 && n_total > 0, SHG_E_ARG, "shg_stage_mean_fit: empty input");
    const int64_t ih = slit_rows(height, width), iw = spectral_cols(height, width);
    const size_t hw = (size_t)height * (size_t)width;
    hipStream_t st = shg::as_stream(stream);
    Arena dev(workspace, workspace_bytes), pin(host_pinned, host_pinned_bytes);
    const size_t acc_bytes = sum_in ? 0 : shg_accumulate_workspace_bytes(n_frames, height, width, bytes_per_px);
    char* acc_ws = dev.take<char>(acc_bytes ? acc_bytes : 1);
    uint64_t* sum = dev.take<uint64_t>(hw);
    uint16_t* mx = dev.take<uint16_t>(hw);
    uint16_t* blur = dev.take<uint16_t>(hw);
    uint32_t* tmp = dev.take<uint32_t>(hw);
    double* row_means = dev.take<double>((size_t)ih);
    int32_t* traces = dev.take<int32_t>(2 * (size_t)ih);
    double* h_means = pin.take<double>((size_t)ih);
    int32_t* h_traces = pin.take<int32_t>(2 * (size_t)ih);
    SHG_REQUIRE(acc_ws && sum && mx && blur && tmp && row_means && traces, SHG_E_WORKSPACE, "shg_stage_mean_fit: workspace too small");
    SHG_REQUIRE(h_means && h_traces, SHG_E_WORKSPACE, "shg_stage_mean_fit: pinned staging area too small");
    Staging stg;
    STAGE_TRY(map_staging(host_pinned, &stg, "shg_stage_mean_fit"));
    row_means = stg.on_device(h_means);
    traces = stg.on_device(h_traces);

    if (!sum_in) {
        SHG_REQUIRE(n_total == n_frames, SHG_E_ARG, "shg_stage_mean_fit: n_total %lld != %lld frames of the stack", (long long)n_total, (long long)n_frames);
        STAGE_TRY(shg_accumulate_mean_max(stack, n_frames, height, width, bytes_per_px, frame_stride_px, mean_out, max_out, acc_ws, acc_bytes, stream));
    } else {
        STAGE_TRY(shg_finalize_mean_max(sum_in, max_in, n_total, height, width, bytes_per_px, mean_out, max_out, stream));
    }
    if (shg_blur_fits_fused(iw, 5)) {
        STAGE_TRY(shg_blur_row_mean_u16(max_out, ih, iw, 5, 5, row_means, stream));
    } else {
        STAGE_TRY(shg_box_blur_u16(max_out, ih, iw, 5, 5, blur, tmp, stream));
        STAGE_TRY(shg_row_mean_u16(blur, ih, iw, row_means, stream));
    }
    STAGE_SYNC(st, "shg_stage_mean_fit");
    int64_t y1, y2;
    STAGE_TRY(shg_host_detect_bord(h_means, ih, &y1, &y2));
    const int64_t clip = (int64_t)((double)(y2 - y1) * 0.05);
    y1 = std::min(ih - 1, y1 + clip);
    y2 = std::max<int64_t>(0, y2 - clip);
    host_y12[0] = y1;
    host_y12[1] = y2;
    const int blur_w = 25, blur_h = (int)((double)(y2 - y1) * 0.01);
    const int64_t lo = blur_w / 2, hi = iw + (-(blur_w + 1) / 2);
    if (blur_h > 0 && shg_blur_fits_fused(iw, blur_h)) {
        STAGE_TRY(shg_blur_argmin_u16(mean_out, ih, iw, blur_w, blur_h, lo, hi, traces, traces + ih, stream));
    } else {
        STAGE_TRY(shg_box_blur_u16(mean_out, ih, iw, blur_w, blur_h, blur, tmp, stream));
        STAGE_TRY(shg_row_argmin_u16(blur, ih, iw, lo, hi, traces, stream));
        STAGE_TRY(shg_row_argmin_u16(mean_out, ih, iw, 0, iw, traces + ih, stream));
    }
    STAGE_SYNC(st, "shg_stage_mean_fit");
    if (host_trace_sharp) memcpy(host_trace_sharp, h_traces + ih, (size_t)ih * 4);
    return shg_host_line_fit(h_traces, h_traces + ih, ih, y1, y2, (int32_t)lo, host_p4, host_fit, host_mask_good);
}

extern "C" size_t shg_stage_extract_workspace_bytes(int64_t height, int64_t width, int n_shifts) {
    if (height <= 0 || width <= 0 || n_shifts <= 0) return 0;
    const size_t ih = (size_t)slit_rows(height, width);
    return up((size_t)n_shifts * ih * 4) + up(2 * ih * 8) + up(ih * 4);
}

extern "C" int shg_stage_extract(const void* stack, int64_t n_frames, int64_t height, int64_t width, int bytes_per_px,
                                 int64_t frame_stride_px, const double* host_fit, const int32_t* host_shifts, int n_shifts,
                                 uint16_t* disks, int64_t row_pitch, int64_t plane_stride, int64_t n_cols, int64_t k_offset,
                                 int flip_x, uint32_t* minmax_slots, void* workspace, size_t workspace_bytes, void* host_pinned,
                                 size_t host_pinned_bytes, shg_stream_t stream) {
    SHG_HOST_TIME("stage extract");
    SHG_REQUIRE(stack && host_fit && host_shifts && disks && workspace && host_pinned, SHG_E_ARG, "shg_stage_extract: null pointer");
    SHG_REQUIRE(height > 0 && width > 0 && n_shifts > 0, SHG_E_ARG, "shg_stage_extract: empty input");
    const int64_t ih = slit_rows(height, width), iw = spectral_cols(height, width);
    Arena dev(workspace, workspace_bytes), pin(host_pinned, host_pinned_bytes);
    int32_t* ind_l = dev.take<int32_t>((size_t)n_shifts * ih);
    double* w2 = dev.take<double>(2 * (size_t)ih);
    int32_t* base = dev.take<int32_t>((size_t)ih);
    int32_t* h_ind = pin.take<int32_t>((size_t)n_shifts * ih);
    double* h_w2 = pin.take<double>(2 * (size_t)ih);
    int32_t* h_base = pin.take<int32_t>((size_t)ih);
    SHG_REQUIRE(ind_l && w2 && base, SHG_E_WORKSPACE, "shg_stage_extract: workspace too small");
    SHG_REQUIRE(h_ind && h_w2 && h_base, SHG_E_WORKSPACE, "shg_stage_extract: pinned staging area too small");
    STAGE_TRY(shg_host_column_plan(host_fit, ih, iw, host_shifts, n_shifts, h_ind, h_w2, h_w2 + ih));
    const int dense_mode = [] { const char* v = getenv("SHG_EXT_DENSE"); return v ? atoi(v) : 1; }();
    const bool dense = dense_mode > 0 && iw > n_shifts && shg_extract_dense_fits(host_shifts, n_shifts);
    if (dense) {
        int lo = host_shifts[0];
        for (int i = 1; i < n_shifts; ++i) lo = std::min(lo, (int)host_shifts[i]);
        for (int64_t y = 0; y < ih; ++y) {
            const double v = host_fit[y * 4] + 1.0 * (double)lo;
            h_base[y] = (v == v && v > -1e9 && v < 1e9) ? (int32_t)(int64_t)v : INT32_MIN;
        }
    }
    hipStream_t st = shg::as_stream(stream);
    Staging stg;
    STAGE_TRY(map_staging(host_pinned, &stg, "shg_stage_extract"));
    const char* end = dense ? reinterpret_cast<const char*>(h_base + ih) : reinterpret_cast<const char*>(h_w2 + 2 * ih);
    if (minmax_slots) {
        const size_t n_words = ((size_t)(end - reinterpret_cast<const char*>(h_ind)) + 3) / 4, zero_words = (size_t)n_shifts * 130;
        const unsigned blocks = (unsigned)std::min<size_t>((std::max(n_words, zero_words) + 255) / 256, 64);
        STAGE_TRY(shg::launch(k_words_zero, dim3(blocks), dim3(256), 0, st,
                             WordsArgs{reinterpret_cast<uint32_t*>(ind_l), reinterpret_cast<const uint32_t*>(stg.on_device(h_ind)), n_words, minmax_slots, zero_words}, "k_words_zero"));
        shg::t_minmax_slots_zeroed = true;
    } else {
        STAGE_TRY(move_words(ind_l, stg.on_device(h_ind), (size_t)(end - reinterpret_cast<const char*>(h_ind)), st));
    }
    if (dense)
        return shg_extract_columns_dense(stack, n_frames, height, width, bytes_per_px, frame_stride_px, ind_l, base, w2, w2 + ih, host_shifts, n_shifts,
                                         disks, row_pitch, plane_stride, n_cols, k_offset, flip_x, minmax_slots, stream);
    return shg_extract_columns_minmax(stack, n_frames, height, width, bytes_per_px, frame_stride_px, ind_l, w2, w2 + ih, n_shifts, disks,
                                      row_pitch, plane_stride, n_cols, k_offset, flip_x, minmax_slots, stream);
}

namespace {
constexpr int kFactor = 4;
inline int64_t small_dim(int64_t v) { return (v + kFactor - 1) / kFactor; }

inline bool limb_fused(int64_t sh, int64_t sw, int k) {
    const char* v = getenv("SHG_LIMB_FUSED");
    return !(v && v[0] == '0') && k > 0 && shg_limb_fused_fits(sh, sw, k);
}

int64_t keep_strong_components(int32_t* idx, int32_t* root, int64_t m, int64_t n) {
    thread_local std::vector<uint8_t> strong;
    if ((int64_t)strong.size() < n) strong.assign((size_t)n, 0);
    for (int64_t i = 0; i < m; ++i)
        if (root[i] & (1 << 30)) strong[(size_t)(root[i] & 0x3fffffff)] = 1;
    int64_t kept = 0;
    for (int64_t i = 0; i < m; ++i) {
        const int32_t r = root[i] & 0x3fffffff;
        if (strong[(size_t)r]) { idx[kept] = idx[i]; root[kept] = r; ++kept; }
    }
    for (int64_t i = 0; i < kept; ++i) strong[(size_t)root[i]] = 0;
    return kept;
}
struct LimbImage { const uint16_t* disk; int64_t h, w, pitch, sh, sw, n; int k; };

struct FusedLimb {
    size_t prep_bytes, edge_bytes;
    char *prep_ws = nullptr, *edge_ws = nullptr;
    const uint32_t* keys = nullptr;
    FusedLimb(const LimbImage& im) : prep_bytes(shg_limb_prepare_workspace_bytes(im.sh, im.sw, im.k)), edge_bytes(shg_limb_edges_workspace_bytes(im.sh, im.sw)) {}
    size_t bytes() const { return up(prep_bytes) + up(edge_bytes) + kAlign; }
    bool carve(Arena& dev) {
        prep_ws = dev.take<char>(prep_bytes);
        edge_ws = dev.take<char>(edge_bytes);
        return prep_ws && edge_ws;
    }
    int prepare(const LimbImage& im, const int64_t* ranks, double gamma99, double* packed_dev, shg_stream_t stream) {
        return shg_limb_prepare(im.disk, im.h, im.w, im.pitch, im.k, ranks, gamma99, packed_dev, &keys, prep_ws, prep_bytes, stream);
    }
    int edges(const LimbImage& im, double thresh3, const double* taps, int radius, double low, double high, int32_t* comp_dev, shg_stream_t stream) {
        return shg_limb_edges(keys, im.sh, im.sw, im.k, thresh3, taps, radius, low, high, comp_dev, edge_ws, edge_bytes, stream);
    }
    int64_t kept(int32_t* h_comp, int64_t n) const { return keep_strong_components(h_comp + 1, h_comp + 1 + n, h_comp[0], n); }
};

struct SeparateLimb {
    size_t n, sel_bytes, canny_bytes, cc_bytes;
    double *small = nullptr, *blurred = nullptr, *blur5 = nullptr, *tmp = nullptr, *packed = nullptr;
    char *sel_ws = nullptr, *flood_ws = nullptr, *canny_ws = nullptr, *cc_ws = nullptr;
    uint32_t *keys_k = nullptr, *keys_5 = nullptr;
    uint8_t *low_mask = nullptr, *high_mask = nullptr;
    int32_t* comp = nullptr;
    SeparateLimb(const LimbImage& im)
        : n((size_t)im.n), sel_bytes(std::max(shg_select_workspace_bytes(4), shg_select_keys_workspace_bytes(4))),
          canny_bytes(shg_canny_workspace_bytes(im.sh, im.sw)), cc_bytes(shg_edge_components_workspace_bytes(im.sh, im.sw)) {}
    template <typename Take>
    void layout(Take take) {
        take(small, n); take(blurred, n); take(blur5, n); take(tmp, n);
        take(sel_ws, sel_bytes);
        take(keys_k, n); take(keys_5, n);
        take(packed, 32);
        take(flood_ws, 256);
        take(low_mask, n); take(high_mask, n);
        take(canny_ws, canny_bytes); take(cc_ws, cc_bytes);
        take(comp, 2 * n + 1);
    }
    size_t bytes() {
        size_t total = 0;
        layout([&](auto*& p, size_t count) { total += up(count * sizeof(*p)); });
        return total + 3 * kAlign + kAlign;
    }
    bool carve(Arena& dev) {
        bool ok = true;
        layout([&](auto*& p, size_t count) { p = dev.take<std::remove_reference_t<decltype(*p)>>(count); ok = ok && p; });
        return ok;
    }
    int prepare(const LimbImage& im, const int64_t* ranks, double gamma99, double* packed_dev, shg_stream_t stream) {
        const int64_t sh = im.sh, sw = im.sw;
        const int k = im.k;
        STAGE_TRY(shg_downscale_mean_u16(im.disk, im.h, im.w, im.pitch, kFactor, small, stream));
        if (k <= 63) {
            STAGE_TRY(shg_box_blur_key_f64(small, sh, sw, k, blurred, keys_k, tmp, stream));
            if (k == 5) {
                blur5 = blurred;
                keys_5 = keys_k;
            } else {
                STAGE_TRY(shg_box_blur_key_f64(small, sh, sw, 5, blur5, keys_5, tmp, stream));
            }
            const uint32_t* karr[4] = {keys_5, keys_5, keys_k, keys_k};
            const int kk[4] = {5, 5, k, k};
            STAGE_TRY(shg_select_keys_u32(karr, im.n, ranks, kk, 4, packed, sel_ws, sel_bytes, stream));
        } else {
            STAGE_TRY(shg_box_blur_f64(small, sh, sw, k, blurred, tmp, stream));
            STAGE_TRY(shg_box_blur_f64(small, sh, sw, 5, blur5, tmp, stream));
            const double* arrays[4] = {blur5, blur5, blurred, blurred};
            STAGE_TRY(shg_select_multi_f64(arrays, im.n, ranks, 4, packed, sel_ws, sel_bytes, stream));
        }
        STAGE_TRY(shg_flood_stats_lerp_f64(small, blurred, im.n, packed + 2, gamma99, packed + 4, reinterpret_cast<uint32_t*>(packed + 8), flood_ws, stream));
        return move_words(packed_dev, packed, 8 * 8 + 20 * 4, shg::as_stream(stream));
    }
    int edges(const LimbImage& im, double thresh3, const double* taps, int radius, double low, double high, int32_t* comp_dev, shg_stream_t stream) {
        STAGE_TRY(shg_canny_masks_f64(blurred, im.sh, im.sw, thresh3, taps, radius, low, high, low_mask, high_mask, canny_ws, canny_bytes, stream));
        STAGE_TRY(shg_edge_components(low_mask, high_mask, im.sh, im.sw, comp + 1, comp + 1 + im.n, comp, cc_ws, cc_bytes, stream));
        k_edge_list<<<16, 256, 0, shg::as_stream(stream)>>>(comp, im.n, comp_dev);
        return shg::check_launch("k_edge_list");
    }
    int64_t kept(int32_t* h_comp, int64_t) const { return h_comp[0]; }
};

inline LimbImage limb_image(const uint16_t* disk, int64_t h, int64_t w, int64_t pitch) {
    const int64_t sh = small_dim(h), sw = small_dim(w);
    return LimbImage{disk, h, w, pitch, sh, sw, sh * sw, (int)((double)sh * 0.01)};
}

template <typename Chain>
int limb_points_with(Chain chain, const LimbImage& im, const double* host_gauss_taps, int32_t* host_points, uint8_t* host_flags, int64_t points_cap,
                     int64_t* host_counts2, void* workspace, size_t workspace_bytes, void* host_pinned, size_t host_pinned_bytes, shg_stream_t stream) {
    const int64_t sh = im.sh, sw = im.sw, n = im.n;
    hipStream_t st = shg::as_stream(stream);
    Arena dev(workspace, workspace_bytes), pin(host_pinned, host_pinned_bytes);
    const bool carved = chain.carve(dev);
    double* h_packed = pin.take<double>(32);
    int32_t* h_comp = pin.take<int32_t>(2 * (size_t)n + 1);
    SHG_REQUIRE(carved, SHG_E_WORKSPACE, "shg_stage_limb_points: workspace too small");
    SHG_REQUIRE(h_packed && h_comp, SHG_E_WORKSPACE, "shg_stage_limb_points: pinned staging area too small");
    Staging stg;
    STAGE_TRY(map_staging(host_pinned, &stg, "shg_stage_limb_points"));
    int64_t ranks[4];
    double gamma99;
    ranks[0] = (n & 1) ? n / 2 : n / 2 - 1;
    ranks[1] = n / 2;
    STAGE_TRY(shg_host_percentile_plan(n, 99.0, &ranks[2], &ranks[3], &gamma99));
    STAGE_TRY(chain.prepare(im, ranks, gamma99, stg.on_device(h_packed), stream));
    STAGE_SYNC(st, "shg_stage_limb_points");
    const double median5 = (n & 1) ? h_packed[0] : (h_packed[0] + h_packed[1]) / 2;
    const double low = median5 / 10, high = low * 1.5;
    int64_t counts64[20];
    const uint32_t* hc = reinterpret_cast<const uint32_t*>(h_packed + 8);
    for (int i = 0; i < 20; ++i) counts64[i] = hc[i];
    double thresh3;
    STAGE_TRY(shg_host_flood_threshold(h_packed[4], sh, sw, h_packed[5], h_packed[6], counts64, &thresh3));

    int64_t m = 0;
    const double* taps = host_gauss_taps;
    for (int rung = 0;; ++rung) {
        if (rung == 4) { shg::set_error("ellipse fit: could not find any edges of the solar disk"); return SHG_E_RUNTIME; }
        const double sigma = 2.0 - 0.5 * rung;
        const int radius = (int)(4.0 * sigma + 0.5);
        STAGE_TRY(chain.edges(im, thresh3, taps, radius, low, high, stg.on_device(h_comp), stream));
        STAGE_SYNC(st, "shg_stage_limb_points");
        SHG_REQUIRE(h_comp[0] >= 0 && h_comp[0] <= n, SHG_E_RUNTIME, "shg_stage_limb_points: %lld edge pixels in an image of %lld", (long long)h_comp[0], (long long)n);
        m = chain.kept(h_comp, n);
        if (m > 0) break;
        taps += 2 * radius + 1;
    }
    const int32_t* idx = h_comp + 1;
    const int32_t* root = h_comp + 1 + n;
    SHG_REQUIRE(points_cap >= m, SHG_E_WORKSPACE, "shg_stage_limb_points: %lld edge pixels, room for %lld", (long long)m, (long long)points_cap);
    int64_t n_sel = 0;
    STAGE_TRY(shg_host_limb_points(idx, root, m, sh, sw, host_flags, &n_sel));
    for (int64_t i = 0; i < m; ++i) {
        host_points[2 * i] = idx[i] / (int32_t)sw;
        host_points[2 * i + 1] = idx[i] % (int32_t)sw;
    }
    host_counts2[0] = m;
    host_counts2[1] = n_sel;
    return 0;
}
}

extern "C" size_t shg_stage_limb_points_workspace_bytes(int64_t h, int64_t w) {
    if (h <= 0 || w <= 0) return 0;
    const LimbImage im = limb_image(nullptr, h, w, w);
    return limb_fused(im.sh, im.sw, im.k) ? FusedLimb(im).bytes() : SeparateLimb(im).bytes();
}

extern "C" size_t shg_stage_limb_points_host_bytes(int64_t h, int64_t w) {
    if (h <= 0 || w <= 0) return 0;
    const size_t n = (size_t)small_dim(h) * (size_t)small_dim(w);
    return up(32 * 8) + up((2 * n + 1) * 4);
}

extern "C" int shg_stage_limb_points(const uint16_t* disk, int64_t h, int64_t w, int64_t pitch, const double* host_gauss_taps,
                                     int32_t* host_points, uint8_t* host_flags, int64_t points_cap, int64_t* host_counts2,
                                     void* workspace, size_t workspace_bytes, void* host_pinned, size_t host_pinned_bytes,
                                     shg_stream_t stream) {
    SHG_REQUIRE(disk && host_gauss_taps && host_points && host_flags && host_counts2 && workspace && host_pinned, SHG_E_ARG,
                "shg_stage_limb_points: null pointer");
    SHG_REQUIRE(h > 0 && w > 0 && pitch >= w, SHG_E_ARG, "shg_stage_limb_points: bad image size");
    const LimbImage im = limb_image(disk, h, w, pitch);
    if (im.k <= 0) {
        shg::set_error("ellipse fit: the scan needs at least 400 slit rows (cv2.blur kernel int(0.01 * h/4) = 0)");
        return SHG_E_RUNTIME;
    }
    if (limb_fused(im.sh, im.sw, im.k))
        return limb_points_with(FusedLimb(im), im, host_gauss_taps, host_points, host_flags, points_cap, host_counts2, workspace, workspace_bytes,
                                host_pinned, host_pinned_bytes, stream);
    return limb_points_with(SeparateLimb(im), im, host_gauss_taps, host_points, host_flags, points_cap, host_counts2, workspace, workspace_bytes,
                            host_pinned, host_pinned_bytes, stream);
}

extern "C" int shg_stage_limb_fit(const uint16_t* disk, int64_t h, int64_t w, int64_t pitch, const double* host_gauss_taps,
                                  int32_t* host_points, uint8_t* host_flags, int64_t points_cap, int64_t* host_counts3,
                                  double* host_geom16, int64_t* host_dims2, double* host_outline200, void* workspace,
                                  size_t workspace_bytes, void* host_pinned, size_t host_pinned_bytes, shg_stream_t stream) {
    SHG_HOST_TIME("stage limb_fit");
    SHG_REQUIRE(host_counts3 && host_geom16 && host_dims2, SHG_E_ARG, "shg_stage_limb_fit: null pointer");
    STAGE_TRY(shg_stage_limb_points(disk, h, w, pitch, host_gauss_taps, host_points, host_flags, points_cap, host_counts3, workspace,
                                    workspace_bytes, host_pinned, host_pinned_bytes, stream));
    const int64_t m = host_counts3[0], n_sel = host_counts3[1];
    std::vector<double> X((size_t)std::max<int64_t>(n_sel, 1) * 2);
    std::vector<uint8_t> kept((size_t)std::max<int64_t>(n_sel, 1));
    for (int64_t i = 0, j = 0; i < m; ++i)
        if (host_flags[i]) {
            X[2 * j] = (double)host_points[2 * i] * kFactor;
            X[2 * j + 1] = (double)host_points[2 * i + 1] * kFactor;
            ++j;
        }
    STAGE_TRY(shg_host_limb_geometry(X.data(), n_sel, h, w, host_geom16, host_dims2, kept.data(), &host_counts3[2], host_outline200));
    for (int64_t i = 0, j = 0; i < m; ++i)
        if (host_flags[i]) { if (kept[j]) host_flags[i] |= 2; ++j; }
    return 0;
}

extern "C" size_t shg_stage_process_workspace_bytes(int64_t k, int64_t h, int64_t w, int64_t crop_w, int tiles) {
    if (k <= 0 || h <= 0 || w <= 0) return 0;
    const size_t pitch = ((size_t)std::max(w, crop_w) + 63) / 64 * 64;
    return 2 * up((size_t)h * 4) + 2 * up((size_t)k * h * 8) + up((size_t)k * h * 8) + up(4096 * 8) +
           (size_t)k * up((size_t)h * pitch * 2) + (size_t)k * up(shg_contrast_stats_workspace_bytes_for(h, crop_w > 0 ? crop_w : w, tiles)) + up((size_t)k * 5 * 8) + kAlign;
}

extern "C" size_t shg_stage_process_host_bytes(int64_t k, int64_t h) {
    if (k <= 0 || h <= 0) return 0;
    return 2 * up((size_t)h * 4) + 2 * up((size_t)k * h * 8) + up((size_t)k * h * 8) + up((size_t)k * 5 * 8) + up(4096 * 8);
}

extern "C" int shg_stage_process_frames(const uint16_t* const* host_frames, int64_t k, int64_t h, int64_t w, int64_t pitch,
                                        int transversalium, const double* host_circle3, const double* host_borders4,
                                        const double* host_taps, int64_t window, double* host_factors,
                                        int64_t crop_w, int64_t sx0, int64_t dx0, int64_t ncopy,
                                        double clip_limit, int tiles, int64_t disc_x0, int64_t disc_y0, int64_t disc_r,
                                        uint16_t* const* host_detrans, int64_t detrans_pitch,
                                        uint16_t* const* host_final, uint16_t* const* host_cl1, uint16_t* const* host_hc,
                                        uint16_t* const* host_protus, uint16_t* const* host_cc, int64_t out_pitch,
                                        void* workspace, size_t workspace_bytes, void* host_pinned, size_t host_pinned_bytes,
                                        shg_stream_t stream) {
    SHG_HOST_TIME("stage process_frames");
    SHG_REQUIRE(host_frames && host_final && host_cl1 && host_hc && host_protus && host_cc && workspace && host_pinned, SHG_E_ARG,
                "shg_stage_process_frames: null pointer");
    SHG_REQUIRE(k > 0 && h > 0 && w > 0 && pitch >= w, SHG_E_ARG, "shg_stage_process_frames: bad image size");
    const int64_t out_w = crop_w > 0 ? crop_w : w;
    SHG_REQUIRE(out_pitch >= out_w, SHG_E_ARG, "shg_stage_process_frames: out_pitch < output width");
    hipStream_t st = shg::as_stream(stream);
    Arena dev(workspace, workspace_bytes), pin(host_pinned, host_pinned_bytes);
    int32_t* xa = dev.take<int32_t>((size_t)h);
    int32_t* xb = dev.take<int32_t>((size_t)h);
    double* taps_d = dev.take<double>(4096);
    double* stats = dev.take<double>((size_t)k * h);
    double* interior = dev.take<double>((size_t)k * h);
    double* factors = dev.take<double>((size_t)k * h);
    const size_t tpitch = ((size_t)w + 63) / 64 * 64;
    std::vector<uint16_t*> scaled((size_t)k, nullptr);
    const char* fuse_env = getenv("SHG_FUSE_SCALE");
    const bool fuse_on = !(fuse_env && fuse_env[0] == '0');
    const bool fuse = fuse_on && !host_detrans && shg::contrast_stats_batches(h, crop_w > 0 ? crop_w : w, tiles, clip_limit) && pitch >= w;
    const bool need_tmp = transversalium && crop_w > 0 && !host_detrans && !fuse;
    if (need_tmp)
        for (int64_t i = 0; i < k; ++i) scaled[i] = dev.take<uint16_t>((size_t)h * tpitch);
    const size_t cs_each = up(shg_contrast_stats_workspace_bytes_for(h, out_w, tiles));
    SHG_REQUIRE(cs_each != 0, SHG_E_ARG, "shg_stage_process_frames: unsupported tile count %d", tiles);
    const size_t cs_bytes = (size_t)k * cs_each;
    char* cs_ws = dev.take<char>(cs_bytes);
    double* out5 = dev.take<double>((size_t)k * 5);
    int32_t* h_xa = pin.take<int32_t>((size_t)h);
    int32_t* h_xb = pin.take<int32_t>((size_t)h);
    double* h_taps = pin.take<double>(4096);
    double* h_stats = pin.take<double>((size_t)k * h);
    double* h_interior = pin.take<double>((size_t)k * h);
    double* h_factors = pin.take<double>((size_t)k * h);
    double* h_out5 = pin.take<double>((size_t)k * 5);
    SHG_REQUIRE(xa && xb && stats && interior && factors && taps_d && cs_ws && out5 && (!need_tmp || scaled[k - 1]), SHG_E_WORKSPACE,
                "shg_stage_process_frames: workspace too small");
    SHG_REQUIRE(h_xa && h_xb && h_stats && h_interior && h_factors && h_out5 && h_taps, SHG_E_WORKSPACE, "shg_stage_process_frames: pinned staging area too small");
    Staging stg;
    STAGE_TRY(map_staging(host_pinned, &stg, "shg_stage_process_frames"));

    std::vector<const uint16_t*> cur((size_t)k);
    int64_t cur_pitch = pitch;
    for (int64_t i = 0; i < k; ++i) cur[i] = host_frames[i];
    if (transversalium) {
        SHG_REQUIRE(host_circle3 && host_borders4 && host_taps, SHG_E_ARG, "shg_stage_process_frames: transversalium needs circle, borders, taps");
        const double cx = host_circle3[0], cy = host_circle3[1], r = host_circle3[2];
// ... 98 lines not shown
```

solex_ser_recon_en_amd/stages.py:

```python
import ctypes
import os
import threading

import numpy as np
import torch

from . import _lib, ops
from ._lib import lib

_local = threading.local()


def use_buffers(store):
    _local.buffers = store


def _scratch(name, nbytes, device=None, pinned=False):
    store = _local.__dict__.setdefault('buffers', {})
    key = (name, str(device), pinned)
    buf = store.get(key)
    if buf is None or buf.numel() < nbytes:
        size = max(int(nbytes), 1)
        if pinned:
            buf = torch.empty(size, dtype=torch.uint8).pin_memory()
# ... 217 lines not shown
    def __init__(self, buf):
        self.words = buf.view(torch.uint16)

    def plane(self, off, h, pitch, w):
        return torch.as_strided(self.words, (h, w), (pitch, 1), off // 2)


class _LazyImages:
    __slots__ = ('planes', 'off', 'step', 'count', 'geom')

    def __init__(self, planes, off, step, count, h, pitch, w):
        self.planes, self.off, self.step, self.count, self.geom = planes, off, step, count, (h, pitch, w)

    def __len__(self):
        return self.count

    def __getitem__(self, j):
        if not 0 <= j < self.count:
            raise IndexError(j)
        return self.planes.plane(self.off + j * self.step, *self.geom)


def _host_buffers(name, specs):
    store = _local.__dict__.setdefault('host', {})
    out = []
    for tag, shape, dtype in specs:
        key = (name, tag)
        buf = store.get(key)
        if buf is None or buf.shape != tuple(shape) or buf.dtype != np.dtype(dtype):
            buf = store[key] = np.empty(shape, dtype=dtype)
        out.append(buf)
    return out


_pinned_free = []
_pinned_lock = threading.Lock()


PINNED_SLAB = 12


def _lease_pinned(nbytes):
    with _pinned_lock:
        for i, buf in enumerate(_pinned_free):
            if buf.numel() >= nbytes:
                return _pinned_free.pop(i)
        each = (max(int(nbytes), 1) + 4095) // 4096 * 4096
        slab = torch.empty(each * PINNED_SLAB, dtype=torch.uint8).pin_memory()
        parts = [slab[i * each:(i + 1) * each] for i in range(PINNED_SLAB)]
        _pinned_free.extend(parts[1:])
        return parts[0]


def _return_pinned(buf):
    with _pinned_lock:
        if len(_pinned_free) < 64:
            _pinned_free.append(buf)


_host_free = {}


def _lease_host(specs):
    with _pinned_lock:
        free = _host_free.get(specs)
        if free:
            return free.pop()
    return [np.empty(shape, dtype=dt) for _, shape, dt in specs]


def _return_host(specs, bufs):
    with _pinned_lock:
        free = _host_free.setdefault(specs, [])
        if len(free) < 32:
            free.append(bufs)


def _even256(nbytes):
    return (max(int(nbytes), 256) + 255) // 256 * 256


class ScanCall:

    def __init__(self, stack, shifts, requested, options, taps_for, want_plot_data=False, want_fit_image=False, own_buffers=False):
        n, h, w, bpp = ops.stack_geometry(stack)
        dev = stack.device
        ih, iw = (w, h) if w > h else (h, w)
        self.stack, self.dev, self.n, self.ih, self.plot = stack, dev, n, ih, want_plot_data
        self.sh = sh = np.ascontiguousarray(shifts, dtype=np.int32)
        self.rqd = rqd = np.ascontiguousarray(requested, dtype=np.uint8)
        self.s, self.k = s, k = int(sh.size), int(rqd.sum())
        ratio_fixe, slant_fix = options['ratio_fixe'], options['slant_fix']
        self.limb = limb = ratio_fixe is None and slant_fix is None
        self.trans = trans = bool(options['transversalium'])
        keep_detrans = bool(options['save_fit'] and trans)
        fit_image = bool(want_fit_image and not rqd[0])
        self.own = own_buffers

        self.pitch = pitch = (n + 63) // 64 * 64
        self.images = images = torch.empty((2, ih, iw), dtype=torch.uint16, device=dev)
        self.disks = disks = torch.empty((s, ih, pitch), dtype=torch.uint16, device=dev)
        self.mm_store = mm_store = torch.empty(s * 130, dtype=torch.int32, device=dev)
        self.cap = cap = (-(-ih // 4)) * (-(-n // 4)) if limb else 1
        self.specs = specs = (('fit', (ih, 4), 'f8'), ('sharp', (ih,), 'i4'), ('mask', (ih,), 'u1'), ('points', (cap, 2), 'i4'),
                              ('flags', (cap,), 'u1'), ('outline', (100, 2), 'f8'), ('factors', (max(k, 1), ih), 'f8'))
        self.bufs = bufs = _lease_host(specs) if own_buffers else _host_buffers('scan', specs)
        self.fit, self.sharp, self.mask, self.points, self.flags, self.outline, self.factors = bufs
        self.gauss = gauss = _canny_ladder_taps()
        ts = int(options['trans_strength'])
        self.taps = taps = taps_for(ts) if trans and ts > 3 and ts % 2 == 1 else None

        self.rq = rq = _lib.ScanRequest()
        rq.struct_bytes = ctypes.sizeof(_lib.ScanRequest)
        rq.stack, rq.n_frames, rq.height, rq.width, rq.frame_stride_px, rq.bytes_per_px = stack.data_ptr(), n, h, w, ops.frame_stride(stack), bpp
        rq.flip_x = int(bool(options['flip_x']))
        rq.host_shifts, rq.host_requested, rq.n_shifts, rq.want_fit_image = _p(sh), _p(rqd), s, int(fit_image)
        rq.ratio_fixe = _NAN if ratio_fixe is None else float(ratio_fixe)
        rq.slant_fix_deg = _NAN if slant_fix is None else float(slant_fix)
        rq.transversalium, rq.keep_detrans, rq.trans_strength = int(trans), int(keep_detrans), ts
        rq.host_taps, rq.taps_window = (None, 0) if taps is None else (_p(taps), ts)
        rq.crop_square = int(bool(options['crop_width_square']))
        rq.has_fixed_width = int(options['fixed_width'] is not None)
        rq.fixed_width = 0 if options['fixed_width'] is None else int(options['fixed_width'])
        rq.disk_display, rq.tiles, rq.delta_radius, rq.clip_limit = int(bool(options['disk_display'])), 2, int(options['delta_radius']), 0.8
        rq.host_gauss_taps = _p(gauss)
        rq.mean_out, rq.max_out = images[0].data_ptr(), images[1].data_ptr()
        rq.disks, rq.disk_pitch, rq.disk_plane_stride, rq.minmax_slots = disks.data_ptr(), pitch, ih * pitch, mm_store.data_ptr()
        rq.host_fit = _p(self.fit)
        rq.host_trace_sharp, rq.host_mask_good = (_p(self.sharp), _p(self.mask)) if want_plot_data else (None, None)
        rq.host_points, rq.host_flags, rq.points_cap = (_p(self.points), _p(self.flags), cap) if limb else (None, None, 0)
        rq.host_outline200 = _p(self.outline) if (limb and want_plot_data) else None
        rq.host_factors = _p(self.factors) if (trans and k) else None

        self.key = key = (s, k, ih, n, bpp, bool(options['crop_width_square']), options['fixed_width'], keep_detrans, fit_image, limb)
        hint = _arena_hint.get(key)
        if hint is None:
            guess_w = (int(n * FIRST_GUESS_SCALE) + 127) // 64 * 64
            prod_w = max(guess_w, ih if options['crop_width_square'] else 0, rq.fixed_width)
            hint = ((k * (1 + keep_detrans) + fit_image) * ih * guess_w * 2 + k * 3 * ih * prod_w * 2 + (1 << 16), k * 2 * ih * prod_w * 2 + 4096,
                    lib.shg_scan_workspace_bytes(ctypes.byref(rq)) + (lib.shg_stage_process_workspace_bytes(k, ih, guess_w, prod_w, 2) if k else 0) + 4096)
        self.hint = hint
        pin_bytes = _sizes('scan_pin', lambda *a: lib.shg_scan_host_bytes(ctypes.byref(rq)), s, k, n, h, w, bpp, limb)
        self.pin = _lease_pinned(pin_bytes) if own_buffers else _scratch('scan', pin_bytes, pinned=True)
        self.rs = _lib.ScanResult()
        self.status = None
        self.message = None
        self.pool = self.ticket = None
        self._buffers()

    def _buffers(self):
        rq, hint, dev = self.rq, self.hint, self.dev
        self.arena = arena = torch.empty(_even256(hint[0]), dtype=torch.uint8, device=dev)
        self.results = results = torch.empty(_even256(hint[1]), dtype=torch.uint8, device=dev)
        self.ws = ws = torch.empty(_even256(hint[2]), dtype=torch.uint8, device=dev) if self.own else _scratch('scan', hint[2], dev)
        rq.arena, rq.arena_bytes, rq.results, rq.results_bytes = arena.data_ptr(), arena.numel(), results.data_ptr(), results.numel()
        rq.workspace, rq.workspace_bytes = ws.data_ptr(), ws.numel()
        rq.host_pinned, rq.host_pinned_bytes = self.pin.data_ptr(), self.pin.numel()

    def _needs_resume(self):
        rs = self.rs
        if self.status == -2 and rs.phase_done == 3 and self.rq.start_phase == 0:
            self.hint = (rs.needed_arena_bytes + 4096, rs.needed_results_bytes + 4096, rs.needed_workspace_bytes + 4096)
            self.rq.start_phase = 3
            self._buffers()
            return True
        return False

    def run(self):
        stream = ops._stream()
        while True:
            self.status = lib.shg_scan_file(ctypes.byref(self.rq), ctypes.byref(self.rs), stream)
            self.message = _lib.last_error() if self.status else None
            if not self._needs_resume():
                return self

    def submit(self, pool):
        self.pool = pool
        ticket = ctypes.c_int64()
        after = torch.cuda.current_stream(self.stack.device).cuda_stream
        _lib.check(lib.shg_pool_submit_after(pool, ctypes.byref(self.rq), ctypes.byref(self.rs), after, ctypes.byref(ticket)),
                   'shg_pool_submit')
        self.ticket = ticket.value
        return self

    def done(self):
        return self.ticket is None or lib.shg_pool_poll(self.pool, self.ticket) != 0

    def wait(self):
        while self.ticket is not None:
            status = ctypes.c_int()
            buf = ctypes.create_string_buffer(512)
            _lib.check(lib.shg_pool_wait(self.pool, self.ticket, ctypes.byref(status), buf, len(buf)), 'shg_pool_wait')
            self.ticket = None
            self.status = status.value
            self.message = buf.value.decode('utf-8', 'replace') if self.status else None
            if self._needs_resume():
                self.submit(self.pool)
        return self

    def collect(self):
        rs, rq = self.rs, self.rq
        s, k, n = self.s, self.k, self.n
        phase = int(rs.phase_done)
        if (phase >= 3 and _arena_hint.get(self.key) is None) or rq.start_phase == 3:
            _arena_hint[self.key] = (int(rs.needed_arena_bytes * 1.03) + 4096, int(rs.needed_results_bytes * 1.03) + 4096,
                                     int(rs.needed_workspace_bytes * 1.03) + 4096)
        error = None
        if self.status != 0:
            error = _lib.take_callback_error(rs.window)
            if error is None:
                try:
                    _lib.check(self.status, 'shg_scan_file', self.message)
                except Exception as e:
                    error = e
        out = {'phase': phase, 'mean': self.images[0], 'max': self.images[1], 'limb_fitted': bool(rs.limb_fitted)}
# ... 42 lines not shown
```

Measured before the change: 6.053 million.

## Produce limb-fit 4x4 block sums inside extract kernel and skip unread fit-plane store

The band extraction kernel now uses spare waves to compute 4x4 block sums of the fit plane from its shared tile and writes them into a limb workspace area. The limb blur kernel gains a sums-based variant that reads these precomputed sums instead of re-reading the full disk image. When the raw fit plane is not needed for saving or plots, its store to global memory is skipped entirely. This removes a full-resolution reread and, in some cases, a write, at the cost of extra thread-local hint plumbing and a new ABI field.

Result: no change. 6.042 million (-0.2%).

```diff
diff --git a/include/shg_hip.h b/include/shg_hip.h
--- a/include/shg_hip.h
+++ b/include/shg_hip.h
@@ -305,6 +305,9 @@
 size_t shg_limb_prepare_workspace_bytes(int64_t sh, int64_t sw, int k);
 int shg_limb_prepare(const uint16_t* img, int64_t h, int64_t w, int64_t pitch, int k, const int64_t* host_ranks4, double gamma99,
                      double* packed, const uint32_t** keys_out, void* workspace, size_t workspace_bytes, shg_stream_t stream);
+int shg_limb_prepare_sums(const uint32_t* sums, int64_t sh, int64_t sw, int64_t sums_pitch, int k, const int64_t* host_ranks4,
+                          double gamma99, double* packed, const uint32_t** keys_out, void* workspace, size_t workspace_bytes,
+                          shg_stream_t stream);
 size_t shg_limb_edges_workspace_bytes(int64_t sh, int64_t sw);
 int shg_limb_edges(const uint32_t* keys, int64_t sh, int64_t sw, int k, double flood_thresh, const double* host_gauss_weights,
                    int radius, double low, double high, int32_t* comp, void* workspace, size_t workspace_bytes, shg_stream_t stream);
@@ -324,6 +327,12 @@
                       uint16_t* disks, int64_t row_pitch, int64_t plane_stride, int64_t n_cols, int64_t k_offset,
                       int flip_x, uint32_t* minmax_slots, void* workspace, size_t workspace_bytes, void* host_pinned,
                       size_t host_pinned_bytes, shg_stream_t stream);
+int shg_stage_extract_sums(const void* stack, int64_t n_frames, int64_t height, int64_t width, int bytes_per_px,
+                           int64_t frame_stride_px, const double* host_fit, const int32_t* host_shifts, int n_shifts,
+                           uint16_t* disks, int64_t row_pitch, int64_t plane_stride, int64_t n_cols, int64_t k_offset,
+                           int flip_x, uint32_t* minmax_slots, uint32_t* block_sums, int64_t sums_pitch, int sums_plane,
+                           int skip_plane_store, int* sums_written, void* workspace, size_t workspace_bytes, void* host_pinned,
+                           size_t host_pinned_bytes, shg_stream_t stream);
 
 size_t shg_stage_limb_points_workspace_bytes(int64_t h, int64_t w);
 size_t shg_stage_limb_points_host_bytes(int64_t h, int64_t w);
@@ -336,6 +345,11 @@
                        int32_t* host_points, uint8_t* host_flags, int64_t points_cap, int64_t* host_counts3,
                        double* host_geom16, int64_t* host_dims2, double* host_outline200, void* workspace,
                        size_t workspace_bytes, void* host_pinned, size_t host_pinned_bytes, shg_stream_t stream);
+int shg_stage_limb_fit_sums(const uint16_t* disk, int64_t h, int64_t w, int64_t pitch, const uint32_t* block_sums,
+                            int64_t sums_pitch, const double* host_gauss_taps, int32_t* host_points, uint8_t* host_flags,
+                            int64_t points_cap, int64_t* host_counts3, double* host_geom16, int64_t* host_dims2,
+                            double* host_outline200, void* workspace, size_t workspace_bytes, void* host_pinned,
+                            size_t host_pinned_bytes, shg_stream_t stream);
 
 size_t shg_stage_process_workspace_bytes(int64_t k, int64_t h, int64_t w, int64_t crop_w, int tiles);
 size_t shg_stage_process_host_bytes(int64_t k, int64_t h);
@@ -391,6 +405,7 @@
     int64_t  points_cap;
     double*  host_outline200;
     double*  host_factors;
+    int32_t  fit_disk_unread;
 } shg_scan_request;
 
 typedef struct shg_scan_result {
diff --git a/solex_ser_recon_en_amd/Solex_recon.py b/solex_ser_recon_en_amd/Solex_recon.py
--- a/solex_ser_recon_en_amd/Solex_recon.py
+++ b/solex_ser_recon_en_amd/Solex_recon.py
@@ -566,8 +566,9 @@
         self.shifts = shifts = options['shift']
         self.requested = [sh in options['shift_requested'] for sh in shifts]
         self.plots = plots = plots_enabled(options)
+        self.raw_read = raw_read = bool(options['save_fit'] or plots or options.get('_keep_raw'))
         self.call = stages.ScanCall(rdr.device_stack(), shifts, self.requested, options, savgol_taps, want_plot_data=plots,
-                                    want_fit_image=plots, own_buffers=pooled)
+                                    want_fit_image=plots, own_buffers=pooled, fit_disk_unread=not raw_read)
 
     def run(self):
         self.call.run()
diff --git a/solex_ser_recon_en_amd/_lib.py b/solex_ser_recon_en_amd/_lib.py
--- a/solex_ser_recon_en_amd/_lib.py
+++ b/solex_ser_recon_en_amd/_lib.py
@@ -34,7 +34,7 @@
                 ('minmax_slots', P), ('arena', P), ('arena_bytes', c_size_t), ('results', P), ('results_bytes', c_size_t), ('workspace', P), ('workspace_bytes', c_size_t),
                 ('host_pinned', P), ('host_pinned_bytes', c_size_t),
                 ('host_fit', P), ('host_trace_sharp', P), ('host_mask_good', P), ('host_points', P), ('host_flags', P),
-                ('points_cap', c_int64), ('host_outline200', P), ('host_factors', P)]
+                ('points_cap', c_int64), ('host_outline200', P), ('host_factors', P), ('fit_disk_unread', c_int32)]
 
 
 class ScanResult(ctypes.Structure):
@@ -164,6 +164,7 @@
     'shg_limb_fused_fits': (c_int, [c_int64, c_int64, c_int]),
     'shg_limb_prepare_workspace_bytes': (c_size_t, [c_int64, c_int64, c_int]),
     'shg_limb_prepare': (c_int, [P, c_int64, c_int64, c_int64, c_int, PI64, c_double, P, ctypes.POINTER(c_void_p), P, c_size_t, P]),
+    'shg_limb_prepare_sums': (c_int, [P, c_int64, c_int64, c_int64, c_int, PI64, c_double, P, ctypes.POINTER(c_void_p), P, c_size_t, P]),
     'shg_limb_edges_workspace_bytes': (c_size_t, [c_int64, c_int64]),
     'shg_limb_edges': (c_int, [P, c_int64, c_int64, c_int, c_double, PD, c_int, c_double, c_double, P, P, c_size_t, P]),
     'shg_stage_mean_fit_workspace_bytes': (c_size_t, [c_int64, c_int64, c_int64, c_int]),
@@ -173,10 +174,13 @@
     'shg_stage_extract_workspace_bytes': (c_size_t, [c_int64, c_int64, c_int]),
     'shg_stage_extract': (c_int, [P, c_int64, c_int64, c_int64, c_int, c_int64, P, P, c_int, P, c_int64, c_int64, c_int64, c_int64, c_int,
                                   P, P, c_size_t, P, c_size_t, P]),
+    'shg_stage_extract_sums': (c_int, [P, c_int64, c_int64, c_int64, c_int, c_int64, P, P, c_int, P, c_int64, c_int64, c_int64, c_int64, c_int,
+                                       P, P, c_int64, c_int, c_int, ctypes.POINTER(c_int), P, c_size_t, P, c_size_t, P]),
     'shg_stage_limb_points_workspace_bytes': (c_size_t, [c_int64, c_int64]),
     'shg_stage_limb_points_host_bytes': (c_size_t, [c_int64, c_int64]),
     'shg_stage_limb_points': (c_int, [P, c_int64, c_int64, c_int64, P, P, P, c_int64, P, P, c_size_t, P, c_size_t, P]),
     'shg_stage_limb_fit': (c_int, [P, c_int64, c_int64, c_int64, P, P, P, c_int64, P, P, P, P, P, c_size_t, P, c_size_t, P]),
+    'shg_stage_limb_fit_sums': (c_int, [P, c_int64, c_int64, c_int64, P, c_int64, P, P, P, c_int64, P, P, P, P, P, c_size_t, P, c_size_t, P]),
     'shg_stage_process_workspace_bytes': (c_size_t, [c_int64, c_int64, c_int64, c_int64, c_int]),
     'shg_stage_process_host_bytes': (c_size_t, [c_int64, c_int64]),
     'shg_stage_process_frames': (c_int, [P, c_int64, c_int64, c_int64, c_int64, c_int, P, P, P, c_int64, P, c_int64, c_int64, c_int64,
diff --git a/solex_ser_recon_en_amd/csrc/extract.hip b/solex_ser_recon_en_amd/csrc/extract.hip
--- a/solex_ser_recon_en_amd/csrc/extract.hip
+++ b/solex_ser_recon_en_amd/csrc/extract.hip
@@ -8,6 +8,7 @@
 thread_local void* t_zero_with_fold = nullptr;
 thread_local size_t t_zero_with_fold_words = 0;
 thread_local void* t_prezeroed = nullptr;
+thread_local BlockSumsHint t_block_sums;
 }
 
 namespace {
@@ -327,6 +328,10 @@
     uint32_t* mm;
     int nx;
     uint8_t plane_of[BAND_MAX_S];
+    uint32_t* block_sums;
+    int64_t sums_pitch;
+    int sums_d;
+    uint32_t no_store;
 };
 typedef unsigned short __attribute__((ext_vector_type(2))) ushort2_t;
 typedef unsigned int __attribute__((ext_vector_type(4))) u32x4_t;
@@ -454,8 +459,33 @@
     const int64_t kb = (flip_x ? (n_cols - 1 - (col + 7)) : (col + 7)) - k_offset;
     const bool whole = a.vec_store && col + 8 <= n_cols && ka >= 0 && ka < n_frames && kb >= 0 && kb < n_frames;
     const int rows_here = (int)min((int64_t)TY, ih - (int64_t)by * TY);
+    if (a.block_sums && wave >= ns) {
+        const int ds = a.sums_d - g0;
+        if (ds >= 0 && ds < ns) {
+            const int sh = (int)((ih + 3) >> 2), sw = (ncols32 + 3) >> 2;
+            const int cols_here = min(TK, ncols32 - (int)c0);
+            for (int e = (wave - ns) * 64 + lane; e < (TY / 4) * (TK / 4); e += (NW - ns) * 64) {
+                const int by4 = e / (TK / 4), bx4 = e % (TK / 4);
+                const int sy = by * (TY / 4) + by4, sx = bx * (TK / 4) + bx4;
+                if (sy >= sh || sx >= sw) continue;
+                uint32_t s = 0;
+#pragma unroll
+                for (int j = 0; j < 4; ++j) {
+                    const int r = 4 * by4 + j;
+                    const uint32_t* s32 = &btile[(ds * TY + r) * DKW + 2 * bx4];
+                    const uint32_t p0 = s32[0], p1 = s32[1];
+                    const int c = 4 * bx4;
+                    uint32_t t = (c < cols_here ? p0 & 0xffffu : 0u) + (c + 1 < cols_here ? p0 >> 16 : 0u) +
+                                 (c + 2 < cols_here ? p1 & 0xffffu : 0u) + (c + 3 < cols_here ? p1 >> 16 : 0u);
+                    s += r < rows_here ? t : 0u;
+                }
+                a.block_sums[(int64_t)sy * a.sums_pitch + sx] = s;
+            }
+        }
+    }
     for (int d = wave; d < ns; d += NW) {
         const int plane = CONSEC ? a.plane_of[g0 + d] : g0 + d;
+        if ((a.no_store >> plane) & 1u) continue;
         uint16_t* dst0 = a.disks + (int64_t)plane * a.plane_stride + ((int64_t)by * TY) * a.row_pitch + col;
         uint32_t lo = 0xffffffffu, hi = 0u;
         if (whole) {
@@ -527,6 +557,10 @@
     return status;
 }
 
+bool band_takes_sums(const shg::BlockSumsHint& want, int64_t n_frames, int64_t n_cols, int64_t k_offset, int n_shifts, int64_t ih) {
+    return want.sums && k_offset == 0 && n_frames == n_cols && want.plane >= 0 && want.plane < n_shifts && want.pitch >= (n_cols + 3) / 4 && ih > 0;
+}
+
 struct FoldMinmaxArgs {
     const uint32_t* slots;
     uint32_t* out;
@@ -581,6 +615,8 @@
                                           int64_t n_cols, int64_t k_offset, int flip_x, uint32_t* minmax_slots, shg_stream_t stream) {
     const bool slots_zeroed = shg::t_minmax_slots_zeroed;
     shg::t_minmax_slots_zeroed = false;
+    const shg::BlockSumsHint want = shg::t_block_sums;
+    shg::t_block_sums = shg::BlockSumsHint{};
     SHG_REQUIRE(stack && ind_l && lw && rw && disks, SHG_E_ARG, "shg_extract_columns: null pointer");
     SHG_REQUIRE(n_frames > 0 && height > 0 && width > 0 && n_shifts > 0, SHG_E_ARG, "shg_extract_columns: empty input");
     SHG_REQUIRE(bytes_per_px == 1 || bytes_per_px == 2, SHG_E_ARG, "shg_extract_columns: bytes_per_px must be 1 or 2");
@@ -626,9 +662,12 @@
     const bool general_only = [] { const char* e = getenv("SHG_EXT_GENERAL"); return e && atoi(e) != 0; }();
     if (rot && !general_only) {
         BandArgs ba{stack, n, height, width, fstride, ind_l, nullptr, lw, rw, n_shifts, disks, row_pitch, plane_stride, n_cols, k_offset, flip_x, vec_store,
-                    minmax_slots, (int)((n_cols + TK - 1) / TK), {}};
+                    minmax_slots, (int)((n_cols + TK - 1) / TK), {}, nullptr, 0, 0, 0u};
+        const bool sums = band_takes_sums(want, n_frames, n_cols, k_offset, n_shifts, ih);
+        if (sums) { ba.block_sums = want.sums; ba.sums_pitch = want.pitch; ba.sums_d = want.plane; ba.no_store = want.no_store ? 1u << want.plane : 0u; }
         launch_status = launch_band<false>(ba, bytes_per_px, ih, st);
         if (launch_status) return launch_status;
+        shg::t_block_sums.produced = sums;
         if (minmax_slots) return launch_fold(minmax_slots, n_shifts, st);
         return 0;
     }
@@ -665,6 +704,8 @@
                                          shg_stream_t stream) {
     const bool slots_zeroed = shg::t_minmax_slots_zeroed;
     shg::t_minmax_slots_zeroed = false;
+    const shg::BlockSumsHint want = shg::t_block_sums;
+    shg::t_block_sums = shg::BlockSumsHint{};
     SHG_REQUIRE(stack && ind_l && base_col && lw && rw && host_shifts && disks, SHG_E_ARG, "shg_extract_columns_dense: null pointer");
     SHG_REQUIRE(n_frames > 0 && height > 0 && width > 0, SHG_E_ARG, "shg_extract_columns_dense: empty input");
     SHG_REQUIRE(shg_extract_dense_fits(host_shifts, n_shifts), SHG_E_UNSUPPORTED, "shg_extract_columns_dense: the shifts are not 3..%d consecutive integers", DS_MAX);
@@ -692,10 +733,13 @@
     const int n = (int)n_frames;
     if (rot) {
         BandArgs ba{stack, n, height, width, fstride, ind_l, base_col, lw, rw, n_shifts, disks, row_pitch, plane_stride, n_cols, k_offset, flip_x, vec_store,
-                    minmax_slots, (int)((n_cols + TK - 1) / TK), {}};
+                    minmax_slots, (int)((n_cols + TK - 1) / TK), {}, nullptr, 0, 0, 0u};
         for (int i = 0; i < n_shifts; ++i) ba.plane_of[host_shifts[i] - lo] = (uint8_t)i;
+        const bool sums = band_takes_sums(want, n_frames, n_cols, k_offset, n_shifts, ih);
+        if (sums) { ba.block_sums = want.sums; ba.sums_pitch = want.pitch; ba.sums_d = host_shifts[want.plane] - lo; ba.no_store = want.no_store ? 1u << want.plane : 0u; }
         const int launch_status = launch_band<true>(ba, bytes_per_px, ih, st);
         if (launch_status) return launch_status;
+        shg::t_block_sums.produced = sums;
         if (minmax_slots) return launch_fold(minmax_slots, n_shifts, st);
         return 0;
     }
diff --git a/solex_ser_recon_en_amd/csrc/limb_fused.hip b/solex_ser_recon_en_amd/csrc/limb_fused.hip
--- a/solex_ser_recon_en_amd/csrc/limb_fused.hip
+++ b/solex_ser_recon_en_amd/csrc/limb_fused.hip
@@ -107,29 +107,49 @@
     int sh, sw, k, vec4;
     uint32_t *keysk, *keys5;
     unsigned long long* acc;
-};
-__global__ __launch_bounds__(256) void k_limb_blur(const LimbBlurArgs kargs) {
+    const uint32_t* sums;
+    int64_t sums_pitch;
+    int tiles_x, tiles;
+};
+template <bool SUMS> struct BlurTile { static constexpr int W = SUMS ? 64 : BT, H = SUMS ? 8 : BT, NT = W * H; };
+template <bool SUMS>
+__global__ __launch_bounds__(BlurTile<SUMS>::NT) void k_limb_blur(const LimbBlurArgs kargs) {
+    constexpr int BW = BlurTile<SUMS>::W, BH = BlurTile<SUMS>::H, NT = BlurTile<SUMS>::NT, NWV = NT / 64;
     const uint16_t* __restrict__ img = kargs.img;
     const int h = kargs.h, w = kargs.w, sh = kargs.sh, sw = kargs.sw, k = kargs.k, vec4 = kargs.vec4;
     const int64_t pitch = kargs.pitch;
     uint32_t* __restrict__ keysk = kargs.keysk;
     uint32_t* __restrict__ keys5 = kargs.keys5;
     unsigned long long* __restrict__ acc = kargs.acc;
-    __shared__ uint32_t S[(BT + KMAX) * (BT + KMAX)];
-    __shared__ uint32_t H[(BT + KMAX) * BT];
-    __shared__ unsigned long long wsum[4];
-    __shared__ uint32_t wmin[4];
+    __shared__ uint32_t S[(BH + KMAX) * (BW + KMAX)];
+    __shared__ uint32_t H[(BH + KMAX) * BW];
+    __shared__ unsigned long long wsum[NWV];
+    __shared__ uint32_t wmin[NWV];
     const int hl = max(k / 2, 2), hr = max(k - 1 - k / 2, 2);
-    const int RH = BT + hl + hr, RW = RH;
-    const int x0 = blockIdx.x * BT, y0 = blockIdx.y * BT;
+    const int RH = BH + hl + hr, RW = BW + hl + hr;
+    int tile_x, tile_y, tile;
+    if (SUMS) {
+        const int per = (kargs.tiles + 7) / 8;
+        tile = (int)(blockIdx.x & 7u) * per + (int)(blockIdx.x >> 3);
+        if ((int)(blockIdx.x >> 3) >= per || tile >= kargs.tiles) return;
+        tile_y = tile / kargs.tiles_x;
+        tile_x = tile - tile_y * kargs.tiles_x;
+    } else {
+        tile_x = blockIdx.x;
+        tile_y = blockIdx.y;
+        tile = blockIdx.y * gridDim.x + blockIdx.x;
+    }
+    const int x0 = tile_x * BW, y0 = tile_y * BH;
     const int tid = threadIdx.x;
     uint32_t my_min = 0xffffffffu;
     unsigned long long own = 0;
-    for (int e = tid; e < RH * RW; e += 256) {
+    for (int e = tid; e < RH * RW; e += NT) {
         const int r = e / RW, c = e - r * RW;
         const int sy = refl101(y0 - hl + r, sh), sx = refl101(x0 - hl + c, sw);
         uint32_t s = 0;
-        if (vec4 && sx * 4 + 4 <= w && sy * 4 + 4 <= h) {
+        if (SUMS) {
+            s = kargs.sums[(int64_t)sy * kargs.sums_pitch + sx];
+        } else if (vec4 && sx * 4 + 4 <= w && sy * 4 + 4 <= h) {
             uint2 q[4];
 #pragma unroll
             for (int j = 0; j < 4; ++j) q[j] = *reinterpret_cast<const uint2*>(img + (int64_t)(sy * 4 + j) * pitch + sx * 4);
@@ -147,7 +167,7 @@
         }
         S[e] = s;
         const int oy = y0 - hl + r, ox = x0 - hl + c;
-        if (r >= hl && r < hl + BT && c >= hl && c < hl + BT && oy < sh && ox < sw) own += s;
+        if (r >= hl && r < hl + BH && c >= hl && c < hl + BW && oy < sh && ox < sw) own += s;
     }
     own = shg::wave_sum((uint64_t)own);
     if ((tid & 63) == 0) wsum[tid >> 6] = own;
@@ -156,18 +176,18 @@
         const int kw = a == 0 ? k : 5;
         uint32_t* keys = a == 0 ? keysk : keys5;
         __syncthreads();
-        const int c_off = hl - kw / 2, r_lo = hl - kw / 2, r_n = BT + kw - 1;
-        for (int e = tid; e < r_n * BT; e += 256) {
-            const int r = r_lo + e / BT, x = e % BT;
+        const int c_off = hl - kw / 2, r_lo = hl - kw / 2, r_n = BH + kw - 1;
+        for (int e = tid; e < r_n * BW; e += NT) {
+            const int r = r_lo + e / BW, x = e % BW;
             uint32_t s = 0;
             for (int j = 0; j < kw; ++j) s += S[r * RW + x + c_off + j];
-            H[r * BT + x] = s;
+            H[r * BW + x] = s;
         }
         __syncthreads();
-        const int y = tid / BT, x = tid % BT;
+        const int y = tid / BW, x = tid % BW;
         if (y0 + y < sh && x0 + x < sw) {
             uint32_t s = 0;
-            for (int j = 0; j < kw; ++j) s += H[(r_lo + y + j) * BT + x];
+            for (int j = 0; j < kw; ++j) s += H[(r_lo + y + j) * BW + x];
             keys[(int64_t)(y0 + y) * sw + x0 + x] = s;
             if (a == 0) my_min = s;
         }
@@ -176,10 +196,11 @@
     if ((tid & 63) == 0) wmin[tid >> 6] = my_min;
     __syncthreads();
     if (tid == 0) {
-        const int slot = (blockIdx.y * gridDim.x + blockIdx.x) % FLOOD_SLOTS;
-        const unsigned long long t = wsum[0] + wsum[1] + wsum[2] + wsum[3];
+        const int slot = tile % FLOOD_SLOTS;
+        unsigned long long t = 0;
+        uint32_t m = 0xffffffffu;
+        for (int wv = 0; wv < NWV; ++wv) { t += wsum[wv]; m = min(m, wmin[wv]); }
         if (t) atomicAdd(&acc[acc_sum(slot)], t);
-        const uint32_t m = min(min(wmin[0], wmin[1]), min(wmin[2], wmin[3]));
         if (m != 0xffffffffu) atomicMax(&acc[ACC_SMALLEST + slot], ~f64_key(((double)m * kUnit) * (1.0 / ((double)k * (double)k))));
     }
 }
@@ -638,11 +659,11 @@
     return prep_layout(sh, sw, k).total_words * 4;
 }
 
-extern "C" int shg_limb_prepare(const uint16_t* img, int64_t h, int64_t w, int64_t pitch, int k, const int64_t* host_ranks4, double gamma99,
-                                double* packed, const uint32_t** keys_out, void* workspace, size_t workspace_bytes, shg_stream_t stream) {
-    SHG_REQUIRE(img && host_ranks4 && packed && keys_out && workspace, SHG_E_ARG, "shg_limb_prepare: null pointer");
-    SHG_REQUIRE(h > 0 && w > 0 && pitch >= w, SHG_E_ARG, "shg_limb_prepare: bad image size");
-    const int64_t sh = (h + 3) / 4, sw = (w + 3) / 4, n = sh * sw;
+namespace {
+int limb_prepare(const uint16_t* img, int64_t h, int64_t w, int64_t pitch, const uint32_t* sums, int64_t sums_pitch, int64_t sh, int64_t sw, int k,
+                 const int64_t* host_ranks4, double gamma99, double* packed, const uint32_t** keys_out, void* workspace, size_t workspace_bytes,
+                 shg_stream_t stream) {
+    const int64_t n = sh * sw;
     SHG_REQUIRE(shg_limb_fused_fits(sh, sw, k), SHG_E_UNSUPPORTED, "shg_limb_prepare: a %d x %d window on %lld x %lld is outside the fused path", k, k,
                 (long long)sh, (long long)sw);
     SHG_REQUIRE(gamma99 >= 0.0 && gamma99 <= 1.0, SHG_E_ARG, "shg_limb_prepare: gamma %g outside [0, 1]", gamma99);
@@ -666,9 +687,18 @@
     Ranks4 p;
     const double scale_k = 1.0 / ((double)k * (double)k), scale_5 = 1.0 / 25.0;
     for (int i = 0; i < 4; ++i) { p.rank[i] = host_ranks4[i]; p.array[i] = (i < 2 && k != 5) ? 1 : 0; p.scale[i] = (i < 2) ? scale_5 : scale_k; }
-    dim3 grid1((unsigned)((sw + BT - 1) / BT), (unsigned)((sh + BT - 1) / BT));
-    const int vec4 = (reinterpret_cast<uintptr_t>(img) & 7) == 0 && pitch % 4 == 0;
-    if (int e = shg::launch(k_limb_blur, grid1, dim3(256), 0, st, LimbBlurArgs{img, (int)h, (int)w, pitch, (int)sh, (int)sw, k, vec4, keysk, keys5, acc}, "k_limb_blur")) return e;
+    if (sums) {
+        const int tiles_x = (int)((sw + BlurTile<true>::W - 1) / BlurTile<true>::W), tiles = tiles_x * (int)((sh + BlurTile<true>::H - 1) / BlurTile<true>::H);
+        if (int e = shg::launch(k_limb_blur<true>, dim3((unsigned)((tiles + 7) / 8 * 8)), dim3(BlurTile<true>::NT), 0, st,
+                               LimbBlurArgs{nullptr, 0, 0, 0, (int)sh, (int)sw, k, 0, keysk, keys5, acc, sums, sums_pitch, tiles_x, tiles}, "k_limb_blur"))
+            return e;
+    } else {
+        dim3 grid1((unsigned)((sw + BT - 1) / BT), (unsigned)((sh + BT - 1) / BT));
+        const int vec4 = (reinterpret_cast<uintptr_t>(img) & 7) == 0 && pitch % 4 == 0;
+        if (int e = shg::launch(k_limb_blur<false>, grid1, dim3(256), 0, st,
+                               LimbBlurArgs{img, (int)h, (int)w, pitch, (int)sh, (int)sw, k, vec4, keysk, keys5, acc, nullptr, 0, 0, 0}, "k_limb_blur"))
+            return e;
+    }
     static const bool lds_ok = [] {
         return hipFuncSetAttribute(reinterpret_cast<const void*>(k_limb_select0), hipFuncAttributeMaxDynamicSharedMemorySize, 128 * 1024) == hipSuccess &&
                hipFuncSetAttribute(reinterpret_cast<const void*>(k_limb_select1), hipFuncAttributeMaxDynamicSharedMemorySize, 128 * 1024) == hipSuccess;
@@ -684,6 +714,21 @@
         return e;
     *keys_out = keysk;
     return shg::launch(k_limb_flood_hist, dim3((unsigned)blocks), dim3(256), 0, st, LimbFloodHistArgs{keysk, n, scale_k, acc, out4, counts, done + 1, packed, limb_fence()}, "k_limb_flood_hist");
+}
+}
+
+extern "C" int shg_limb_prepare(const uint16_t* img, int64_t h, int64_t w, int64_t pitch, int k, const int64_t* host_ranks4, double gamma99,
+                                double* packed, const uint32_t** keys_out, void* workspace, size_t workspace_bytes, shg_stream_t stream) {
+    SHG_REQUIRE(img && host_ranks4 && packed && keys_out && workspace, SHG_E_ARG, "shg_limb_prepare: null pointer");
+    SHG_REQUIRE(h > 0 && w > 0 && pitch >= w, SHG_E_ARG, "shg_limb_prepare: bad image size");
+    return limb_prepare(img, h, w, pitch, nullptr, 0, (h + 3) / 4, (w + 3) / 4, k, host_ranks4, gamma99, packed, keys_out, workspace, workspace_bytes, stream);
+}
+
+extern "C" int shg_limb_prepare_sums(const uint32_t* sums, int64_t sh, int64_t sw, int64_t sums_pitch, int k, const int64_t* host_ranks4, double gamma99,
+                                     double* packed, const uint32_t** keys_out, void* workspace, size_t workspace_bytes, shg_stream_t stream) {
+    SHG_REQUIRE(sums && host_ranks4 && packed && keys_out && workspace, SHG_E_ARG, "shg_limb_prepare_sums: null pointer");
+    SHG_REQUIRE(sh > 0 && sw > 0 && sums_pitch >= sw, SHG_E_ARG, "shg_limb_prepare_sums: bad image size");
+    return limb_prepare(nullptr, 0, 0, 0, sums, sums_pitch, sh, sw, k, host_ranks4, gamma99, packed, keys_out, workspace, workspace_bytes, stream);
 }
 
 extern "C" size_t shg_limb_edges_workspace_bytes(int64_t sh, int64_t sw) {
diff --git a/solex_ser_recon_en_amd/csrc/scan.hip b/solex_ser_recon_en_amd/csrc/scan.hip
--- a/solex_ser_recon_en_amd/csrc/scan.hip
+++ b/solex_ser_recon_en_amd/csrc/scan.hip
@@ -199,9 +199,14 @@
             shg::t_zero_with_fold = limb_ws;
             shg::t_zero_with_fold_words = shg::limb_prepare_zero_words(ih, n_cols);
         }
-        const int extract_status = shg_stage_extract(rq->stack, rq->n_frames, rq->height, rq->width, rq->bytes_per_px, rq->frame_stride_px, rq->host_fit,
-                                                     rq->host_shifts, S, rq->disks, rq->disk_pitch, rq->disk_plane_stride, n_cols, 0, rq->flip_x,
-                                                     rq->minmax_slots, extract_ws, rg.extract_ws, extract_pin, rg.extract_pin, stream);
+        const int64_t sums_pitch = (n_cols + 3) / 4;
+        uint32_t* const sums = limb ? shg::limb_sums_area(limb_ws, rg.limb_ws, ih, n_cols) : nullptr;
+        const bool fit_plane_unread = sums && rq->fit_disk_unread && !rq->host_requested[0] && !rq->want_fit_image;
+        int sums_written = 0;
+        const int extract_status = shg_stage_extract_sums(rq->stack, rq->n_frames, rq->height, rq->width, rq->bytes_per_px, rq->frame_stride_px, rq->host_fit,
+                                                          rq->host_shifts, S, rq->disks, rq->disk_pitch, rq->disk_plane_stride, n_cols, 0, rq->flip_x,
+                                                          rq->minmax_slots, sums, sums_pitch, 0, fit_plane_unread ? 1 : 0, &sums_written, extract_ws,
+                                                          rg.extract_ws, extract_pin, rg.extract_pin, stream);
         shg::t_zero_with_fold = nullptr;
         shg::t_zero_with_fold_words = 0;
         if (extract_status) { shg::t_prezeroed = nullptr; return extract_status; }
@@ -211,8 +216,9 @@
         double mat3[9], inv[4], origin[2], det;
         if (limb) {
             int64_t dims[2];
-            const int limb_status = shg_stage_limb_fit(rq->disks, ih, n_cols, rq->disk_pitch, rq->host_gauss_taps, rq->host_points, rq->host_flags, rq->points_cap,
-                                                       rs->counts3, rs->geom16, dims, rq->host_outline200, limb_ws, rg.limb_ws, limb_pin, rg.limb_pin, stream);
+            const int limb_status = shg_stage_limb_fit_sums(rq->disks, ih, n_cols, rq->disk_pitch, sums_written ? sums : nullptr, sums_pitch, rq->host_gauss_taps,
+                                                            rq->host_points, rq->host_flags, rq->points_cap, rs->counts3, rs->geom16, dims, rq->host_outline200,
+                                                            limb_ws, rg.limb_ws, limb_pin, rg.limb_pin, stream);
             shg::t_prezeroed = nullptr;
             if (limb_status) return limb_status;
             const double* g = rs->geom16;
diff --git a/solex_ser_recon_en_amd/csrc/shg_common.h b/solex_ser_recon_en_amd/csrc/shg_common.h
--- a/solex_ser_recon_en_amd/csrc/shg_common.h
+++ b/solex_ser_recon_en_amd/csrc/shg_common.h
@@ -105,9 +105,18 @@
 int on_frame_pass_lane(hipStream_t st, lane_launch_fn launch, void* arg);
 
 extern thread_local bool t_minmax_slots_zeroed;
+struct BlockSumsHint {
+    uint32_t* sums = nullptr;
+    int64_t pitch = 0;
+    int plane = 0;
+    bool no_store = false;
+    bool produced = false;
+};
+extern thread_local BlockSumsHint t_block_sums;
 extern thread_local void* t_zero_with_fold;
 extern thread_local size_t t_zero_with_fold_words;
 extern thread_local void* t_prezeroed;
+uint32_t* limb_sums_area(void* limb_workspace, size_t workspace_bytes, int64_t h, int64_t w);
 size_t limb_prepare_zero_words(int64_t h, int64_t w);
 int prelaunch_on_lane(hipStream_t after, lane_launch_fn launch, void* arg, hipEvent_t* done);
 
diff --git a/solex_ser_recon_en_amd/csrc/stages.hip b/solex_ser_recon_en_amd/csrc/stages.hip
--- a/solex_ser_recon_en_amd/csrc/stages.hip
+++ b/solex_ser_recon_en_amd/csrc/stages.hip
@@ -193,8 +193,22 @@
                                  uint16_t* disks, int64_t row_pitch, int64_t plane_stride, int64_t n_cols, int64_t k_offset,
                                  int flip_x, uint32_t* minmax_slots, void* workspace, size_t workspace_bytes, void* host_pinned,
                                  size_t host_pinned_bytes, shg_stream_t stream) {
+    return shg_stage_extract_sums(stack, n_frames, height, width, bytes_per_px, frame_stride_px, host_fit, host_shifts, n_shifts, disks, row_pitch,
+                                  plane_stride, n_cols, k_offset, flip_x, minmax_slots, nullptr, 0, 0, 0, nullptr, workspace, workspace_bytes, host_pinned,
+                                  host_pinned_bytes, stream);
+}
+
+extern "C" int shg_stage_extract_sums(const void* stack, int64_t n_frames, int64_t height, int64_t width, int bytes_per_px,
+                                      int64_t frame_stride_px, const double* host_fit, const int32_t* host_shifts, int n_shifts,
+                                      uint16_t* disks, int64_t row_pitch, int64_t plane_stride, int64_t n_cols, int64_t k_offset,
+                                      int flip_x, uint32_t* minmax_slots, uint32_t* block_sums, int64_t sums_pitch, int sums_plane,
+                                      int skip_plane_store, int* sums_written, void* workspace, size_t workspace_bytes, void* host_pinned,
+                                      size_t host_pinned_bytes, shg_stream_t stream) {
     SHG_HOST_TIME("stage extract");
+    if (sums_written) *sums_written = 0;
     SHG_REQUIRE(stack && host_fit && host_shifts && disks && workspace && host_pinned, SHG_E_ARG, "shg_stage_extract: null pointer");
+    SHG_REQUIRE(!block_sums || (sums_written && sums_plane >= 0 && sums_plane < n_shifts && sums_pitch >= (n_cols + 3) / 4), SHG_E_ARG,
+                "shg_stage_extract: block sums need sums_written, a plane below n_shifts and a pitch of at least ceil(n_cols / 4)");
     SHG_REQUIRE(height > 0 && width > 0 && n_shifts > 0, SHG_E_ARG, "shg_stage_extract: empty input");
     const int64_t ih = slit_rows(height, width), iw = spectral_cols(height, width);
     Arena dev(workspace, workspace_bytes), pin(host_pinned, host_pinned_bytes);
@@ -230,11 +244,21 @@
     } else {
         STAGE_TRY(move_words(ind_l, stg.on_device(h_ind), (size_t)(end - reinterpret_cast<const char*>(h_ind)), st));
     }
-    if (dense)
-        return shg_extract_columns_dense(stack, n_frames, height, width, bytes_per_px, frame_stride_px, ind_l, base, w2, w2 + ih, host_shifts, n_shifts,
-                                         disks, row_pitch, plane_stride, n_cols, k_offset, flip_x, minmax_slots, stream);
-    return shg_extract_columns_minmax(stack, n_frames, height, width, bytes_per_px, frame_stride_px, ind_l, w2, w2 + ih, n_shifts, disks,
-                                      row_pitch, plane_stride, n_cols, k_offset, flip_x, minmax_slots, stream);
+    if (block_sums) {
+        shg::t_block_sums = shg::BlockSumsHint{};
+        shg::t_block_sums.sums = block_sums;
+        shg::t_block_sums.pitch = sums_pitch;
+        shg::t_block_sums.plane = sums_plane;
+        shg::t_block_sums.no_store = skip_plane_store != 0;
+    }
+    const int status =
+        dense ? shg_extract_columns_dense(stack, n_frames, height, width, bytes_per_px, frame_stride_px, ind_l, base, w2, w2 + ih, host_shifts, n_shifts,
+                                          disks, row_pitch, plane_stride, n_cols, k_offset, flip_x, minmax_slots, stream)
+              : shg_extract_columns_minmax(stack, n_frames, height, width, bytes_per_px, frame_stride_px, ind_l, w2, w2 + ih, n_shifts, disks,
+                                           row_pitch, plane_stride, n_cols, k_offset, flip_x, minmax_slots, stream);
+    if (block_sums && status == 0) *sums_written = shg::t_block_sums.produced ? 1 : 0;
+    shg::t_block_sums = shg::BlockSumsHint{};
+    return status;
 }
 
 namespace {
@@ -259,20 +283,23 @@
     for (int64_t i = 0; i < kept; ++i) strong[(size_t)root[i]] = 0;
     return kept;
 }
-struct LimbImage { const uint16_t* disk; int64_t h, w, pitch, sh, sw, n; int k; };
+struct LimbImage { const uint16_t* disk; int64_t h, w, pitch, sh, sw, n; int k; const uint32_t* sums = nullptr; int64_t sums_pitch = 0; };
 
 struct FusedLimb {
-    size_t prep_bytes, edge_bytes;
+    size_t prep_bytes, edge_bytes, sums_bytes;
     char *prep_ws = nullptr, *edge_ws = nullptr;
     const uint32_t* keys = nullptr;
-    FusedLimb(const LimbImage& im) : prep_bytes(shg_limb_prepare_workspace_bytes(im.sh, im.sw, im.k)), edge_bytes(shg_limb_edges_workspace_bytes(im.sh, im.sw)) {}
-    size_t bytes() const { return up(prep_bytes) + up(edge_bytes) + kAlign; }
+    FusedLimb(const LimbImage& im)
+        : prep_bytes(shg_limb_prepare_workspace_bytes(im.sh, im.sw, im.k)), edge_bytes(shg_limb_edges_workspace_bytes(im.sh, im.sw)), sums_bytes((size_t)im.n * 4) {}
+    size_t sums_offset() const { return up(prep_bytes) + up(edge_bytes); }
+    size_t bytes() const { return sums_offset() + up(sums_bytes) + kAlign; }
     bool carve(Arena& dev) {
         prep_ws = dev.take<char>(prep_bytes);
         edge_ws = dev.take<char>(edge_bytes);
         return prep_ws && edge_ws;
     }
     int prepare(const LimbImage& im, const int64_t* ranks, double gamma99, double* packed_dev, shg_stream_t stream) {
+        if (im.sums) return shg_limb_prepare_sums(im.sums, im.sh, im.sw, im.sums_pitch, im.k, ranks, gamma99, packed_dev, &keys, prep_ws, prep_bytes, stream);
         return shg_limb_prepare(im.disk, im.h, im.w, im.pitch, im.k, ranks, gamma99, packed_dev, &keys, prep_ws, prep_bytes, stream);
     }
     int edges(const LimbImage& im, double thresh3, const double* taps, int radius, double low, double high, int32_t* comp_dev, shg_stream_t stream) {
@@ -347,7 +374,7 @@
 
 inline LimbImage limb_image(const uint16_t* disk, int64_t h, int64_t w, int64_t pitch) {
     const int64_t sh = small_dim(h), sw = small_dim(w);
-    return LimbImage{disk, h, w, pitch, sh, sw, sh * sw, (int)((double)sh * 0.01)};
+    return LimbImage{disk, h, w, pitch, sh, sw, sh * sw, (int)((double)sh * 0.01), nullptr, 0};
 }
 
 template <typename Chain>
@@ -406,6 +433,15 @@
 }
 }
 
+uint32_t* shg::limb_sums_area(void* limb_workspace, size_t workspace_bytes, int64_t h, int64_t w) {
+    if (!limb_workspace || h <= 0 || w <= 0) return nullptr;
+    const LimbImage im = limb_image(nullptr, h, w, w);
+    if (!limb_fused(im.sh, im.sw, im.k)) return nullptr;
+    const FusedLimb f(im);
+    if (f.sums_offset() + f.sums_bytes > workspace_bytes) return nullptr;
+    return reinterpret_cast<uint32_t*>(static_cast<char*>(limb_workspace) + f.sums_offset());
+}
+
 extern "C" size_t shg_stage_limb_points_workspace_bytes(int64_t h, int64_t w) {
     if (h <= 0 || w <= 0) return 0;
     const LimbImage im = limb_image(nullptr, h, w, w);
@@ -418,33 +454,54 @@
     return up(32 * 8) + up((2 * n + 1) * 4);
 }
 
+namespace {
+int limb_points(const uint16_t* disk, int64_t h, int64_t w, int64_t pitch, const uint32_t* sums, int64_t sums_pitch, const double* host_gauss_taps,
+                int32_t* host_points, uint8_t* host_flags, int64_t points_cap, int64_t* host_counts2, void* workspace, size_t workspace_bytes,
+                void* host_pinned, size_t host_pinned_bytes, shg_stream_t stream) {
+    SHG_REQUIRE(disk && host_gauss_taps && host_points && host_flags && host_counts2 && workspace && host_pinned, SHG_E_ARG,
+                "shg_stage_limb_points: null pointer");
+    SHG_REQUIRE(h > 0 && w > 0 && pitch >= w, SHG_E_ARG, "shg_stage_limb_points: bad image size");
+    LimbImage im = limb_image(disk, h, w, pitch);
+    if (im.k <= 0) {
+        shg::set_error("ellipse fit: the scan needs at least 400 slit rows (cv2.blur kernel int(0.01 * h/4) = 0)");
+        return SHG_E_RUNTIME;
+    }
+    if (limb_fused(im.sh, im.sw, im.k)) {
+        SHG_REQUIRE(!sums || sums_pitch >= im.sw, SHG_E_ARG, "shg_stage_limb_points: sums_pitch < ceil(w / 4)");
+        im.sums = sums;
+        im.sums_pitch = sums_pitch;
+        return limb_points_with(FusedLimb(im), im, host_gauss_taps, host_points, host_flags, points_cap, host_counts2, workspace, workspace_bytes,
+                                host_pinned, host_pinned_bytes, stream);
+    }
+    return limb_points_with(SeparateLimb(im), im, host_gauss_taps, host_points, host_flags, points_cap, host_counts2, workspace, workspace_bytes,
+                            host_pinned, host_pinned_bytes, stream);
+}
+}
+
 extern "C" int shg_stage_limb_points(const uint16_t* disk, int64_t h, int64_t w, int64_t pitch, const double* host_gauss_taps,
                                      int32_t* host_points, uint8_t* host_flags, int64_t points_cap, int64_t* host_counts2,
                                      void* workspace, size_t workspace_bytes, void* host_pinned, size_t host_pinned_bytes,
                                      shg_stream_t stream) {
-    SHG_REQUIRE(disk && host_gauss_taps && host_points && host_flags && host_counts2 && workspace && host_pinned, SHG_E_ARG,
-                "shg_stage_limb_points: null pointer");
-    SHG_REQUIRE(h > 0 && w > 0 && pitch >= w, SHG_E_ARG, "shg_stage_limb_points: bad image size");
-    const LimbImage im = limb_image(disk, h, w, pitch);
-    if (im.k <= 0) {
-        shg::set_error("ellipse fit: the scan needs at least 400 slit rows (cv2.blur kernel int(0.01 * h/4) = 0)");
-        return SHG_E_RUNTIME;
-    }
-    if (limb_fused(im.sh, im.sw, im.k))
-        return limb_points_with(FusedLimb(im), im, host_gauss_taps, host_points, host_flags, points_cap, host_counts2, workspace, workspace_bytes,
-                                host_pinned, host_pinned_bytes, stream);
-    return limb_points_with(SeparateLimb(im), im, host_gauss_taps, host_points, host_flags, points_cap, host_counts2, workspace, workspace_bytes,
-                            host_pinned, host_pinned_bytes, stream);
+    return limb_points(disk, h, w, pitch, nullptr, 0, host_gauss_taps, host_points, host_flags, points_cap, host_counts2, workspace, workspace_bytes,
+                       host_pinned, host_pinned_bytes, stream);
 }
 
 extern "C" int shg_stage_limb_fit(const uint16_t* disk, int64_t h, int64_t w, int64_t pitch, const double* host_gauss_taps,
                                   int32_t* host_points, uint8_t* host_flags, int64_t points_cap, int64_t* host_counts3,
                                   double* host_geom16, int64_t* host_dims2, double* host_outline200, void* workspace,
                                   size_t workspace_bytes, void* host_pinned, size_t host_pinned_bytes, shg_stream_t stream) {
+    return shg_stage_limb_fit_sums(disk, h, w, pitch, nullptr, 0, host_gauss_taps, host_points, host_flags, points_cap, host_counts3, host_geom16,
+                                   host_dims2, host_outline200, workspace, workspace_bytes, host_pinned, host_pinned_bytes, stream);
+}
+
+extern "C" int shg_stage_limb_fit_sums(const uint16_t* disk, int64_t h, int64_t w, int64_t pitch, const uint32_t* block_sums, int64_t sums_pitch,
+                                       const double* host_gauss_taps, int32_t* host_points, uint8_t* host_flags, int64_t points_cap,
+                                       int64_t* host_counts3, double* host_geom16, int64_t* host_dims2, double* host_outline200, void* workspace,
+                                       size_t workspace_bytes, void* host_pinned, size_t host_pinned_bytes, shg_stream_t stream) {
     SHG_HOST_TIME("stage limb_fit");
     SHG_REQUIRE(host_counts3 && host_geom16 && host_dims2, SHG_E_ARG, "shg_stage_limb_fit: null pointer");
-    STAGE_TRY(shg_stage_limb_points(disk, h, w, pitch, host_gauss_taps, host_points, host_flags, points_cap, host_counts3, workspace,
-                                    workspace_bytes, host_pinned, host_pinned_bytes, stream));
+    STAGE_TRY(limb_points(disk, h, w, pitch, block_sums, sums_pitch, host_gauss_taps, host_points, host_flags, points_cap, host_counts3, workspace,
+                          workspace_bytes, host_pinned, host_pinned_bytes, stream));
     const int64_t m = host_counts3[0], n_sel = host_counts3[1];
     std::vector<double> X((size_t)std::max<int64_t>(n_sel, 1) * 2);
     std::vector<uint8_t> kept((size_t)std::max<int64_t>(n_sel, 1));
diff --git a/solex_ser_recon_en_amd/stages.py b/solex_ser_recon_en_amd/stages.py
--- a/solex_ser_recon_en_amd/stages.py
+++ b/solex_ser_recon_en_amd/stages.py
@@ -323,7 +323,8 @@
 
 class ScanCall:
 
-    def __init__(self, stack, shifts, requested, options, taps_for, want_plot_data=False, want_fit_image=False, own_buffers=False):
+    def __init__(self, stack, shifts, requested, options, taps_for, want_plot_data=False, want_fit_image=False, own_buffers=False,
+                 fit_disk_unread=False):
         n, h, w, bpp = ops.stack_geometry(stack)
         dev = stack.device
         ih, iw = (w, h) if w > h else (h, w)
@@ -372,6 +373,7 @@
         rq.host_points, rq.host_flags, rq.points_cap = (_p(self.points), _p(self.flags), cap) if limb else (None, None, 0)
         rq.host_outline200 = _p(self.outline) if (limb and want_plot_data) else None
         rq.host_factors = _p(self.factors) if (trans and k) else None
+        rq.fit_disk_unread = int(bool(fit_disk_unread))
 
         self.key = key = (s, k, ih, n, bpp, bool(options['crop_width_square']), options['fixed_width'], keep_detrans, fit_image, limb)
         hint = _arena_hint.get(key)
```
